# Janspiry/Image-Super-Resolution-via-Iterative-Refinement

Hardware: AMD Instinct MI355X
Metric: SR3 16->128 images/sec (2000-step sample) (higher is better)
Workload: dtype f32 via 3xbf16 split MFMA; 1 GPU; SR3 16->128 UNet (reference config/sr_sr3_16_128.json; BASELINE.json configs[1]), batch 16 per GPU, 2000-step p_sample_loop via hipGraph replay; step = one reverse step of the batch; images/s = n_gpus*batch/(2000*t_step); batch_per_gpu=16, global_batch=16, image_size=128, params=97807491, parallelism=independent batches per rank (no collective), weights=random init (PyTorch default, seed 0), output_finite=True

## Files before the change

image-super-resolution-via-iterative-refinement_amd/csrc/abi_ops.hip:

```cpp
#include "plan_internal.h"
#include "tile_code.h"

namespace {

enum Derive { DERIVE_IGEMM_WSPLIT, DERIVE_WINO, DERIVE_WINO_SPLIT };
size_t derive_bytes(const ConvParams& c, Derive kind) {
  const int Cin = c.C0 + c.C1;
  return (kind == DERIVE_IGEMM_WSPLIT ? igemm_wsplit_floats(c.Cout, c.ksize * c.ksize, Cin) : wino_weight_floats(c.Cout, Cin, kind == DERIVE_WINO_SPLIT)) * sizeof(float);
}
int derive_behind_slabs(const ConvParams& c, int tile, int ksplit, Derive kind, void* scratch, size_t* scratch_bytes, hipStream_t st, float** out) {
  const size_t slab = conv_splitk_bytes(c, tile, ksplit);
  const size_t need = derive_bytes(c, kind);
  if (!scratch || *scratch_bytes < slab + need) {
    set_error("conv: %s (%zu < %zu)", kind == DERIVE_IGEMM_WSPLIT ? "scratch too small for the pre-split weights" : "Winograd scratch too small", *scratch_bytes, slab + need);
    return SR3_E_NOMEM;
  }
  *out = reinterpret_cast<float*>(static_cast<char*>(scratch) + slab);
  *scratch_bytes = slab;
  const int Cin = c.C0 + c.C1;
  return kind == DERIVE_IGEMM_WSPLIT ? igemm_split_weights(c.w, c.Cout, c.ksize * c.ksize, Cin, *out, st)
                                     : wino_transform_weights(c.w, c.Cout, Cin, *out, st, kind == DERIVE_WINO_SPLIT);
}

}

extern "C" {

int sr3_p_sample_step(float* x, const float* eps, const float* z, const float* ta, const float* tb, const float* tc1,
                      const float* tc2, const float* tsig, const int* step_dev, const int64_t* t_per_sample,
                      int step_host, int batch, int elems_per_image, void* stream) {
  if (!x || !eps || !ta || !tb || !tc1 || !tc2 || !tsig) { set_error("null argument"); return SR3_E_BADARG; }
  StepTables t{ta, tb, tc1, tc2, tsig};
  return p_sample_update(x, eps, z, t, step_dev, t_per_sample, step_host, batch, elems_per_image,
                         static_cast<hipStream_t>(stream));
}
int sr3_p_sample_step_ex(float* x, const float* eps, const float* z, const float* ta, const float* tb, const float* tc1,
                         const float* tc2, const float* tsig, const int* step_dev, const int64_t* t_per_sample,
                         int step_host, int batch, int elems_per_image, int clip_denoised, void* stream) {
  if (!x || !eps || !ta || !tb || !tc1 || !tc2 || !tsig) { set_error("null argument"); return SR3_E_BADARG; }
  StepTables t{ta, tb, tc1, tc2, tsig};
  return p_sample_update(x, eps, z, t, step_dev, t_per_sample, step_host, batch, elems_per_image,
                         static_cast<hipStream_t>(stream), clip_denoised != 0);
}
int sr3_p_sample_step_hist(float* x, const float* eps, const float* z, const float* ta, const float* tb, const float* tc1,
                           const float* tc2, const float* tsig, const int* step_dev, const int64_t* t_per_sample,
                           int step_host, int batch, int elems_per_image, int clip_denoised, const float* tc3, float* hist,
                           void* stream) {
  if (!x || !eps || !ta || !tb || !tc1 || !tc2 || !tsig) { set_error("null argument"); return SR3_E_BADARG; }
  if (batch <= 0 || elems_per_image <= 0) { set_error("p_sample_step_hist: sizes must be positive"); return SR3_E_BADARG; }
  StepTables t{ta, tb, tc1, tc2, tsig};
  return p_sample_update(x, eps, z, t, step_dev, t_per_sample, step_host, batch, elems_per_image,
                         static_cast<hipStream_t>(stream), clip_denoised != 0, tc3, hist);
}
int sr3_step_decrement(int* step_dev, void* stream) { return step_decrement(step_dev, static_cast<hipStream_t>(stream)); }
int sr3_q_sample(const float* x0, const float* z, const float* ca, const float* cb, int batch, int elems_per_image,
                 float* out, void* stream) {
  if (!x0 || !z || !ca || !cb || !out) { set_error("null argument"); return SR3_E_BADARG; }
  return q_sample(x0, z, ca, cb, batch, elems_per_image, out, static_cast<hipStream_t>(stream));
}

int sr3_conv_f32(const float* src0, int C0, const float* src1, int C1, int B, int Hs, int Ws, int ups, int stride,
                 int ksize, int Cout, const float* w, const float* bias, const float* ss, int act, const float* film,
                 int film_stride, const float* res0, int RC0, const float* res1, int RC1, float* out, double* out_stats,
                 int tile_cfg, int ksplit, void* scratch, size_t scratch_bytes, void* stream) {
  if (!src0 || !w || !out) { set_error("null argument"); return SR3_E_BADARG; }
  hipStream_t st = static_cast<hipStream_t>(stream);
  ConvParams c = conv_shape(B, Hs, Ws, ups, stride, ksize, C0, src1 ? C1 : 0, Cout);
  c.src0 = src0; c.src1 = src1; c.w = w; c.bias = bias; c.ss = ss; c.act = act; c.film = film; c.film_stride = film_stride;
  c.res0 = res0; c.res1 = res1; c.RC0 = res0 ? RC0 : 0; c.RC1 = res1 ? RC1 : 0;
  c.out = out; c.ostat = out_stats;
  const TileCode t = tile_decode(tile_cfg);
  c.wino_split = t.wino_split; c.wino_full = t.wino_full; c.igemm_split = t.igemm_split; tile_cfg = t.tile;
  if (t.wpre) {
    if (tile_cfg == 22 && !gemm1x1_fits(c, 2)) { set_error("conv: the 1x1 GEMM kernel (tile 22) does not fit this problem"); return SR3_E_UNSUPPORTED; }
    float* q = nullptr;
    if (const int rc = derive_behind_slabs(c, tile_cfg, ksplit, DERIVE_IGEMM_WSPLIT, scratch, &scratch_bytes, st, &q)) return rc;
    c.w_split = q;
  }
  if (tile_cfg == 11 && (ksize != 3 || stride != 1)) { set_error("conv: the Winograd kernel does not fit this problem (3x3 stride 1 only)"); return SR3_E_UNSUPPORTED; }
  if (tile_cfg == 11) {
    const Derive kind = t.wino_split ? DERIVE_WINO_SPLIT : DERIVE_WINO;
#ifdef SR3_WINO_ABLATIONS
    const size_t total = scratch_bytes;
#endif
    float* u = nullptr;
    if (const int rc = derive_behind_slabs(c, tile_cfg, ksplit, kind, scratch, &scratch_bytes, st, &u)) return rc;
    c.wino_u = u;
#ifdef SR3_WINO_ABLATIONS
    if (total >= scratch_bytes + derive_bytes(c, kind) + (1u << 20)) c.partial = reinterpret_cast<float*>(reinterpret_cast<char*>(u) + derive_bytes(c, kind));
#endif
  }
  return conv_forward(c, tile_cfg, ksplit, static_cast<float*>(scratch), scratch_bytes, st);
}
int sr3_block_conv_f32(const float* src0, int C0, const float* src1, int C1, int B, int H, int W, int Cout,
                       const float* w, const float* bias, const float* ss, int act, const float* film, int film_stride,
                       const float* x2_src0, int x2_C0, const float* x2_src1, int x2_C1, const float* x2_w,
                       const float* x2_bias, float* out, double* out_stats, int tile_cfg, int ksplit, void* scratch,
                       size_t scratch_bytes, void* stream) {
  if (!src0 || !w || !out || !x2_src0 || !x2_w) { set_error("null argument"); return SR3_E_BADARG; }
  ConvParams c = conv_shape(B, H, W, 0, 1, 3, C0, src1 ? C1 : 0, Cout);
  c.src0 = src0; c.src1 = src1; c.w = w; c.bias = bias; c.ss = ss; c.act = act; c.film = film; c.film_stride = film_stride;
  c.out = out; c.ostat = out_stats;
  c.x2_src0 = x2_src0; c.x2_src1 = x2_src1; c.x2_C0 = x2_C0; c.x2_C1 = x2_src1 ? x2_C1 : 0; c.x2_w = x2_w; c.x2_bias = x2_bias;
  return conv_forward(c, tile_cfg, ksplit, static_cast<float*>(scratch), scratch_bytes, static_cast<hipStream_t>(stream));
}
int sr3_conv_dropout_f32(const float* src0, int C0, int B, int H, int W, int Cout, const float* w, const float* bias,
                         const float* ss, int act, const float* film, int film_stride, const float* res0, int RC0,
                         const float* x2_src0, int x2_C0, const float* x2_src1, int x2_C1, const float* x2_w,
                         const float* x2_bias, float* out, double* out_stats, int tile_cfg, int ksplit, void* scratch,
                         size_t scratch_bytes, unsigned drop_seed, float drop_p, void* stream) {
  if (!src0 || !w || !out || !ss) { set_error("null argument"); return SR3_E_BADARG; }
  if (drop_p < 0.f || drop_p >= 1.f) { set_error("drop_p out of range"); return SR3_E_BADARG; }
  hipStream_t st = static_cast<hipStream_t>(stream);
  ConvParams c = conv_shape(B, H, W, 0, 1, 3, C0, 0, Cout);
  c.src0 = src0; c.w = w; c.bias = bias; c.ss = ss; c.act = act; c.film = film; c.film_stride = film_stride;
  c.res0 = res0; c.RC0 = res0 ? RC0 : 0;
  c.out = out; c.ostat = out_stats;
  if (x2_src0) {
    if (!x2_w) { set_error("x2_src0 needs x2_w"); return SR3_E_BADARG; }
    c.x2_src0 = x2_src0; c.x2_src1 = x2_src1; c.x2_C0 = x2_C0; c.x2_C1 = x2_src1 ? x2_C1 : 0; c.x2_w = x2_w; c.x2_bias = x2_bias;
  }
  c.drop_seed = drop_seed;
  dropout_consts(drop_p, &c.drop_thresh, &c.drop_scale);
  TileCode t = tile_decode(tile_cfg);
  if (tile_cfg != 12) t = TileCode{tile_cfg, 0, 0, false};
  c.wino_split = t.wino_split; tile_cfg = t.tile;
  if (tile_cfg == 11) {
    if (c.x2_w) { set_error("conv: the Winograd kernel has no fused 1x1 segment"); return SR3_E_UNSUPPORTED; }
    float* u = nullptr;
    if (const int rc = derive_behind_slabs(c, tile_cfg, ksplit, t.wino_split ? DERIVE_WINO_SPLIT : DERIVE_WINO, scratch, &scratch_bytes, st, &u)) return rc;
    c.wino_u = u;
  }
  return conv_forward(c, tile_cfg, ksplit, static_cast<float*>(scratch), scratch_bytes, st);
}
unsigned sr3_dropout_threshold(float drop_p, float* scale_out) {
  unsigned t = 0;
  float s = 1.f;
  if (drop_p > 0.f && drop_p < 1.f) dropout_consts(drop_p, &t, &s);
  if (scale_out) *scale_out = s;
  return t;
}
size_t sr3_conv_scratch_bytes(int B, int Ho, int Wo, int Cin, int Cout, int ksize, int tile_cfg, int ksplit) {
  const TileCode t = tile_decode(tile_cfg);
  ConvParams c = conv_shape(B, Ho, Wo, 0, 1, ksize, Cin, 0, Cout);
  c.igemm_split = t.igemm_split;
  if (t.tile == 11) {
    c.wino_split = t.wino_split == 3 ? 3 : 0;
    return conv_splitk_bytes(c, 11, ksplit) + derive_bytes(c, t.wino_split ? DERIVE_WINO_SPLIT : DERIVE_WINO);
  }
  if (t.tile == 22) {
    if (ksize == 3) { c = conv_shape(B, 2 * Ho, 2 * Wo, 0, 2, 3, Cin, 0, Cout); c.igemm_split = 1; }
    return conv_splitk_bytes(c, 22, ksplit) + derive_bytes(c, DERIVE_IGEMM_WSPLIT);
  }
  const size_t extra = t.wpre ? derive_bytes(c, DERIVE_IGEMM_WSPLIT) : 0;
  const size_t b = conv_splitk_bytes(c, t.tile, ksplit);
  c.Hs = c.Ws = c.stride = 0;
  const size_t a = conv_splitk_bytes(c, t.tile, ksplit);
  return (a > b ? a : b) + extra;
}
int sr3_groupnorm_stats_f32(const float* x, int B, int HW, int C, double* stat, void* stream) {
  if (!x || !stat) { set_error("null argument"); return SR3_E_BADARG; }
  return chan_stats(x, B, HW, C, stat, static_cast<hipStream_t>(stream));
}
int sr3_groupnorm_stats_slices(int B, int HW, int C) { return chan_stats_slices(B, HW, C); }
int sr3_conv_stats_slices(int B, int Hs, int Ws, int ups, int Cin, int Cout, int tile_cfg, int ksplit) {
  ConvParams c = conv_shape(B, Hs, Ws, ups, 1, 3, Cin, 0, Cout);
  const TileCode t = tile_decode(tile_cfg);
  c.wino_split = t.wino_split; c.igemm_split = t.igemm_split; tile_cfg = t.tile;
  if (tile_cfg == 22) c.igemm_split = 0;
  conv_pick(c, tile_cfg, ksplit);
  if (ksplit > 1) {
    const int rpb = splitk_rows_per_block(c, true);
    return rpb > 0 ? (c.Ho * c.Wo) / rpb : 0;
  }
  if (tile_cfg == 11) {
    WinoGeom wg;
    return wino_geometry(c, &wg) ? wino_stats_slices(wg) : 0;
  }
  HaloGeom g;
  if (tile_cfg < 5 || !halo_geometry(c, tile_cfg, &g)) return 0;
  return halo_stats_slices(g);
}
int sr3_groupnorm_fold_f32(const double* stat0, int C0, int T0, const double* stat1, int C1, int T1, int B, int HW,
                           int groups, const float* gamma, const float* beta, float eps, float* ss, void* stream) {
  if (!stat0 || !gamma || !beta || !ss) { set_error("null argument"); return SR3_E_BADARG; }
  return gn_finalize(stat0, C0, T0, stat1, stat1 ? C1 : 0, stat1 ? T1 : 0, B, HW, groups, gamma, beta, eps, ss,
                     static_cast<hipStream_t>(stream));
}
int sr3_attention_f32(const float* qkv, int B, int N, int C, float* out, void* stream) {
  if (!qkv || !out) { set_error("null argument"); return SR3_E_BADARG; }
  return attention_forward(qkv, B, N, C, out, static_cast<hipStream_t>(stream));
}
int sr3_attention_ex_f32(const float* qkv, int B, int N, int C, float* out, int split, void* stream) {
  if (!qkv || !out) { set_error("null argument"); return SR3_E_BADARG; }
  return attention_forward(qkv, B, N, C, out, static_cast<hipStream_t>(stream), split);
}
int sr3_film_embed_f32(int variant, int B, int inner, const float* level, const int64_t* timestep, const float* freq,
                       const float* w1, const float* b1, const float* w2, const float* b2, const float* wf,
                       const float* bf, int F, float* temb_scratch, float* film_out, void* stream) {
  EmbedParams e;
  memset(&e, 0, sizeof(e));
  e.variant = variant; e.B = B; e.inner = inner; e.level = level; e.tstep = timestep; e.freq = freq;
  e.w1 = w1; e.b1 = b1; e.w2 = w2; e.b2 = b2; e.wf = wf; e.bf = bf; e.F = F; e.temb = temb_scratch; e.film = film_out;
  return embed_forward(e, static_cast<hipStream_t>(stream));
}
int sr3_conv_in_f32(const float* a, int Ca, const float* b, int Cb, int B, int H, int W, const float* w,
                    const float* bias, int Cout, float* out, void* stream) {
  return conv_in_nchw(a, Ca, b, b ? Cb : 0, B, H, W, w, bias, Cout, out, nullptr, static_cast<hipStream_t>(stream));
}
int sr3_conv_out_f32(const float* x, const float* ss, int B, int H, int W, int C, const float* w, const float* bias,
                     int Cout, float* out, void* stream) {
  return conv_out_nchw(x, ss, B, H, W, C, w, bias, Cout, out, static_cast<hipStream_t>(stream));
}

}
```

image-super-resolution-via-iterative-refinement_amd/csrc/conv_igemm.hip:

```cpp
#include <stdlib.h>

#include <type_traits>

#include "sr3_common.h"

namespace sr3 {

__device__ __forceinline__ float silu_f(float v) {
  return SR3_SILU(v);
}

template <int BM, int BN, int TAPS, int SPLITM>
__global__ __launch_bounds__(256, 2) void k_conv_igemm(const ConvParams p) {
  constexpr bool SPLIT = SPLITM != 0, WPRE = SPLITM == 2;
  constexpr int BK = 32, LDK = 36, LDB = 32;
  constexpr int NST = (SPLIT && !WPRE && BM + BN > 192) ? 1 : 2;
  constexpr int AR = BM / 32, BR = BN / 32;
  constexpr int WM = BM / 2, WN = BN / 2;
  constexpr int MI = WM / 32, NI = WN / 32;
  constexpr int STAGE = SPLIT ? (BM + (WPRE ? 0 : BN)) * LDB * 3 / 2 : (BM + BN) * LDK;
  auto swz = [](int row, int seg) { return row * LDB + (((seg ^ (row >> 2)) & 3) << 3); };
  extern __shared__ f32x4 smem_v[];
  float* smem = reinterpret_cast<float*>(smem_v);

// ... 369 lines not shown
  const int nchunks = (Cin + 31) / 32;
  const long nfrag = (long)((Cout + 31) / 32) * nchunks * taps * 2 * 64;
  int blocks = (int)((nfrag + 255) / 256);
  if (blocks > 4096) blocks = 4096;
  if (blocks < 1) blocks = 1;
  hipLaunchKernelGGL(k_split_weights, dim3(blocks), dim3(256), 0, st, w, Cout, taps, Cin, nchunks, nfrag, reinterpret_cast<__bf16*>(out));
  SR3_LAUNCH_CHECK("k_split_weights");
  return SR3_OK;
}

namespace {
struct TileCfg { int bm, bn; };
const TileCfg kCfgs[5] = {{0, 0}, {128, 128}, {128, 64}, {64, 64}, {64, 128}};

inline int cdiv(int a, int b) { return (a + b - 1) / b; }

template <int BM, int BN, int TAPS, int SPLIT = 0>
int launch_conv(const ConvParams& p, hipStream_t st) {
  static std::atomic<uint64_t> attr_done{0};
  constexpr int smem = SPLIT == 2 ? 2 * BM * 192 : SPLIT ? ((BM + BN > 192) ? 1 : 2) * (BM + BN) * 192 : 2 * (BM + BN) * 36 * 4;
  auto kern = k_conv_igemm<BM, BN, TAPS, SPLIT>;
  if (int rc = ensure_max_lds(reinterpret_cast<const void*>(kern), smem, attr_done)) return rc;
  const int M = p.B * p.Ho * p.Wo;
  dim3 grid(cdiv(M, BM) * cdiv(p.Cout, BN), p.ksplit);
  hipLaunchKernelGGL(kern, grid, dim3(256), smem, st, p);
  SR3_LAUNCH_CHECK("k_conv_igemm");
  return SR3_OK;
}
}

static thread_local hipEvent_t g_mid_event = nullptr;
void conv_set_mid_event(hipEvent_t ev) { g_mid_event = ev; }

void conv_pick(const ConvParams& p, int& tile_cfg, int& ksplit) {
  const int M = p.B * p.Ho * p.Wo;
  const int Cin = p.C0 + p.C1;
  const int taps = p.ksize * p.ksize;
  const int nchunks = cdiv(Cin, 32);
  static const bool no_wide = getenv("SR3_NO_WIDE") != nullptr;
  if (tile_cfg == 0) {
    HaloGeom g;
    if (p.ksize == 3 && p.stride == 1) {
      if (p.Cout <= 64 && halo_geometry(p, 6, &g)) tile_cfg = 6;
      else if (p.Cout > 64 && !no_wide && halo_geometry(p, 9, &g) &&
               (long)cdiv(p.Cout, 128) * g.tiles_w * g.tiles_h * cdiv(p.B, g.NB) >= 256)
        tile_cfg = 9;
      else if (halo_geometry(p, 5, &g)) tile_cfg = 5;
    }
  }
  if (tile_cfg == 0 && p.igemm_split && (p.ksize == 1 || p.stride == 2)) tile_cfg = 3;
  if (tile_cfg == 0 && p.ksize == 1) tile_cfg = 3;
  if (tile_cfg == 0) {
    const int order_wide[3] = {1, 2, 3};
    const int order_narrow[2] = {2, 3};
    const int* order = p.Cout > 64 ? order_wide : order_narrow;
    const int norder = p.Cout > 64 ? 3 : 2;
    tile_cfg = order[norder - 1];
    for (int k = 0; k < norder; ++k) {
      const TileCfg c = kCfgs[order[k]];
      if ((long)cdiv(M, c.bm) * cdiv(p.Cout, c.bn) >= 448) { tile_cfg = order[k]; break; }
    }
  }
  if (tile_cfg == 22) {
    if (ksplit == 0) {
      const long tiles = (long)(M / gemm1x1_rows(p)) * (p.Cout / gemm1x1_cols(p));
      int ks = 1;
#ifndef SR3_G1_SPLIT_BELOW
#define SR3_G1_SPLIT_BELOW 128
#endif
#ifndef SR3_G1_S2_SPLIT_BELOW
#define SR3_G1_S2_SPLIT_BELOW 512
#endif
      const int ksteps = nchunks * taps;
      const int below = taps == 9 ? SR3_G1_S2_SPLIT_BELOW : SR3_G1_SPLIT_BELOW;
      if (tiles < below && tiles > 0) {
        ks = (int)((512 + tiles - 1) / tiles);
        const int cap = taps == 9 ? (ksteps / 8 > 1 ? ksteps / 8 : 1) : (nchunks / 4 > 1 ? nchunks / 4 : 1);
        if (ks > cap) ks = cap;
        if (ks > 16) ks = 16;
      }
      while (ks > 1 && (long)(ks - 1) * cdiv(ksteps, ks) >= ksteps) --ks;
      ksplit = ks;
    }
    return;
  }
  if (ksplit == 0 && tile_cfg == 11) {
    WinoGeom wg;
    if (!wino_geometry(p, &wg)) { ksplit = 1; return; }
    const long tiles = wino_workgroups(p, wg);
    const int units = wino_chunks(p);
    const int maxck = wino_max_chunks_per_split(wg);
    const long round = p.wino_split >= 2 ? 512 : 256;
    int ks = 1;
    if (tiles < round) {
      ks = (int)((round + tiles - 1) / tiles);
      const int cap = units / 4 > 1 ? units / 4 : 1;
      if (ks > cap) ks = cap;
      if (ks > 16) ks = 16;
    }
    if (wg.NB != 1 && ks < 2 && units >= 2) ks = 2;
    if (cdiv(units, ks) > maxck) ks = cdiv(units, maxck);
    while (ks > 1 && (long)(ks - 1) * cdiv(units, ks) >= units) --ks;
    ksplit = ks;
    return;
  }
  if (ksplit == 0) {
    long tiles;
    int units, min_units;
    if (tile_cfg >= 5) {
      HaloGeom g;
      if (!halo_geometry(p, tile_cfg, &g)) { ksplit = 1; return; }
      const int bn = halo_cfg_bn(tile_cfg);
      tiles = (long)cdiv(p.Cout, bn) * g.tiles_w * g.tiles_h * cdiv(p.B, g.NB);
      units = nchunks; min_units = 2;
    } else {
      const TileCfg c = kCfgs[tile_cfg];
      tiles = (long)cdiv(M, c.bm) * cdiv(p.Cout, c.bn);
      units = nchunks * taps; min_units = 6;
    }
    int ks = 1;
    static const long split_below_env = getenv("SR3_KSPLIT_TILES") ? atol(getenv("SR3_KSPLIT_TILES")) : 384;
    const bool wide = halo_cfg_one_wg_per_cu(tile_cfg);
    const long split_below = wide ? 256 : split_below_env;
    if (tiles < split_below) {
      ks = (int)(((wide ? 256 : 512) + tiles - 1) / tiles);
      const int cap = units / min_units > 1 ? units / min_units : 1;
      if (ks > cap) ks = cap;
      if (ks > 16) ks = 16;
    }
    while (ks > 1 && (long)(ks - 1) * cdiv(units, ks) >= units) --ks;
    ksplit = ks;
  }
}

int splitk_rows_per_block(const ConvParams& p, bool stats) {
  const long M = (long)p.B * p.Ho * p.Wo;
  const int HoWo = p.Ho * p.Wo;
  int rpb = 64;
  while (rpb > 4 && M / rpb < 1024) rpb >>= 1;
  if (stats) {
    while (rpb > 1 && HoWo % rpb) rpb >>= 1;
    if (HoWo % rpb || HoWo / rpb > 256) return 0;
  }
  return rpb;
}

size_t conv_splitk_bytes(const ConvParams& p, int tile_cfg, int ksplit) {
  conv_pick(p, tile_cfg, ksplit);
  if (ksplit <= 1) return 0;
  return (size_t)ksplit * p.B * p.Ho * p.Wo * p.Cout * sizeof(float);
}

int conv_forward(const ConvParams& pin, int tile_cfg, int ksplit, float* scratch, size_t scratch_bytes,
                 hipStream_t st) {
  ConvParams p = pin;
  const int Cin = p.C0 + p.C1;
  if ((p.C0 & 3) || (p.C1 & 3) || (p.Cout & 3)) { set_error("conv: channel counts must be multiples of 4 (C0=%d C1=%d Cout=%d)", p.C0, p.C1, p.Cout); return SR3_E_UNSUPPORTED; }
  if (p.ksize != 1 && p.ksize != 3) { set_error("conv: ksize %d unsupported", p.ksize); return SR3_E_UNSUPPORTED; }
  if (p.stride != 1 && p.stride != 2) { set_error("conv: stride %d unsupported", p.stride); return SR3_E_UNSUPPORTED; }
  if (p.act != 0 && !p.ss) { set_error("conv: act needs ss"); return SR3_E_BADARG; }
  if (p.drop_thresh != 0 && (p.C1 != 0 || p.ups != 0 || p.act == 0)) { set_error("conv: dropout needs a single-source, non-upsampled, activated input"); return SR3_E_UNSUPPORTED; }
  if (p.C1 > 0 && !p.src1) { set_error("conv: C1 > 0 needs src1"); return SR3_E_BADARG; }
  if (p.res0 && p.RC0 + p.RC1 != p.Cout) { set_error("conv: residual channels %d+%d != Cout %d", p.RC0, p.RC1, p.Cout); return SR3_E_BADARG; }
  const int pad = p.ksize / 2;
  const int Hi = p.Hs << p.ups, Wi = p.Ws << p.ups;
  if ((Hi + 2 * pad - p.ksize) / p.stride + 1 != p.Ho || (Wi + 2 * pad - p.ksize) / p.stride + 1 != p.Wo) {
    set_error("conv: output dims %dx%d inconsistent with input %dx%d k%d s%d", p.Ho, p.Wo, Hi, Wi, p.ksize, p.stride);
    return SR3_E_BADARG;
  }
  {
    const double lim = 2147483647.0;
    const double e_in = (double)p.B * p.Hs * p.Ws * (double)(p.C0 > p.C1 ? p.C0 : p.C1);
    const double e_w = (double)p.Cout * p.ksize * p.ksize * (double)Cin;
    const double e_ss = (double)p.B * Cin * 2.0;
    if (e_in >= lim || e_w >= lim || e_ss >= lim) { set_error("conv: tensor exceeds 2^31 elements (32-bit offsets)"); return SR3_E_UNSUPPORTED; }
  }
  conv_pick(p, tile_cfg, ksplit);
  p.ksplit = ksplit;
  if (p.ostat && ksplit == 1 && (tile_cfg < 5 || tile_cfg >= 22)) { set_error("conv: fused output statistics need the halo kernel or split-K"); return SR3_E_UNSUPPORTED; }
  if (p.ostat && ksplit > 1 && splitk_rows_per_block(p, true) == 0) { set_error("conv: Ho*Wo does not allow fused split-K statistics"); return SR3_E_UNSUPPORTED; }
  { static const char* e = getenv("SR3_CONV_DBG"); p.dbg = e ? atoi(e) : 0; }
  if (ksplit > 1) {
    const size_t need = (size_t)ksplit * p.B * p.Ho * p.Wo * p.Cout * sizeof(float);
    if (!scratch || scratch_bytes < need) { set_error("conv: split-K scratch too small (%zu < %zu)", scratch_bytes, need); return SR3_E_NOMEM; }
    p.partial = scratch;
  }
  int rc;
  const bool k3 = p.ksize == 3;
  if (p.x2_w && (tile_cfg < 5 || tile_cfg == 11 || tile_cfg >= 22 || p.ups)) { set_error("conv: the fused 1x1 segment needs the halo kernel without upsampling"); return SR3_E_UNSUPPORTED; }
  if (p.x2_w && ((p.x2_C0 & 3) || (p.x2_C1 & 3) || !p.x2_src0 || (p.x2_C1 > 0 && !p.x2_src1))) { set_error("conv: bad x2 segment"); return SR3_E_BADARG; }
  if (tile_cfg == 22) {
    rc = gemm1x1_forward(p, 2, st);
  } else if (tile_cfg == 11) {
    rc = conv3x3_wino_forward(p, p.wino_u, st);
  } else if (tile_cfg >= 5) {
    HaloGeom g;
    if (tile_cfg > 10 || !halo_geometry(p, tile_cfg, &g)) { set_error("conv: halo tile_cfg %d does not fit this problem", tile_cfg); return SR3_E_UNSUPPORTED; }
    const int nchunks = cdiv(Cin, 32);
    if ((long)(ksplit - 1) * cdiv(nchunks, ksplit) >= nchunks && ksplit > 1) { set_error("conv: ksplit %d leaves an empty split over %d chunks", ksplit, nchunks); return SR3_E_BADARG; }
    rc = conv3x3_halo_forward(p, tile_cfg, g, st);
  } else
  if (p.igemm_split && p.w_split) switch (tile_cfg) {
    case 1: rc = k3 ? launch_conv<128, 128, 9, 2>(p, st) : launch_conv<128, 128, 1, 2>(p, st); break;
    case 2: rc = k3 ? launch_conv<128, 64, 9, 2>(p, st) : launch_conv<128, 64, 1, 2>(p, st); break;
    case 3: rc = k3 ? launch_conv<64, 64, 9, 2>(p, st) : launch_conv<64, 64, 1, 2>(p, st); break;
    case 4: rc = k3 ? launch_conv<64, 128, 9, 2>(p, st) : launch_conv<64, 128, 1, 2>(p, st); break;
    default: set_error("conv: bad tile_cfg %d", tile_cfg); return SR3_E_BADARG;
  } else
  if (p.igemm_split) switch (tile_cfg) {
    case 1: rc = k3 ? launch_conv<128, 128, 9, 1>(p, st) : launch_conv<128, 128, 1, 1>(p, st); break;
    case 2: rc = k3 ? launch_conv<128, 64, 9, 1>(p, st) : launch_conv<128, 64, 1, 1>(p, st); break;
    case 3: rc = k3 ? launch_conv<64, 64, 9, 1>(p, st) : launch_conv<64, 64, 1, 1>(p, st); break;
    case 4: rc = k3 ? launch_conv<64, 128, 9, 1>(p, st) : launch_conv<64, 128, 1, 1>(p, st); break;
    default: set_error("conv: bad tile_cfg %d", tile_cfg); return SR3_E_BADARG;
  } else
  switch (tile_cfg) {
    case 1: rc = k3 ? launch_conv<128, 128, 9>(p, st) : launch_conv<128, 128, 1>(p, st); break;
    case 2: rc = k3 ? launch_conv<128, 64, 9>(p, st) : launch_conv<128, 64, 1>(p, st); break;
    case 3: rc = k3 ? launch_conv<64, 64, 9>(p, st) : launch_conv<64, 64, 1>(p, st); break;
    case 4: rc = k3 ? launch_conv<64, 128, 9>(p, st) : launch_conv<64, 128, 1>(p, st); break;
    default: set_error("conv: bad tile_cfg %d", tile_cfg); return SR3_E_BADARG;
  }
  if (rc) return rc;
  if (ksplit > 1) {
    if (g_mid_event) { SR3_HIP(hipEventRecord(g_mid_event, st)); g_mid_event = nullptr; }
    if (p.fold) return splitk_reduce_fold(p, *p.fold, st);
    const int rpb = splitk_rows_per_block(p, p.ostat != nullptr);
    const long M = (long)p.B * p.Ho * p.Wo;
    hipLaunchKernelGGL(k_splitk_reduce, dim3((unsigned)((M + rpb - 1) / rpb)), dim3(256), 0, st, p, rpb);
    SR3_LAUNCH_CHECK("k_splitk_reduce");
  }
  return SR3_OK;
}

}
```

image-super-resolution-via-iterative-refinement_amd/csrc/gemm1x1.hip:

```cpp
#include <stdlib.h>

#include "sr3_common.h"

#pragma clang diagnostic ignored "-Wpass-failed"

namespace sr3 {

namespace {

__device__ __forceinline__ float opaque(float v) { asm("" : "+v"(v)); return v; }
__device__ __forceinline__ void split3_plain(float x0, float x1, unsigned& h, unsigned& m, unsigned& l) {
  bf16x2 hh;
  hh[0] = (__bf16)x0; hh[1] = (__bf16)x1;
  h = __builtin_bit_cast(unsigned, hh);
  const float r0 = opaque(x0 - __builtin_bit_cast(float, h << 16)), r1 = opaque(x1 - __builtin_bit_cast(float, h & 0xFFFF0000u));
  bf16x2 mm;
  mm[0] = (__bf16)r0; mm[1] = (__bf16)r1;
  m = __builtin_bit_cast(unsigned, mm);
  const float q0 = opaque(r0 - __builtin_bit_cast(float, m << 16)), q1 = opaque(r1 - __builtin_bit_cast(float, m & 0xFFFF0000u));
  bf16x2 ll;
  ll[0] = (__bf16)q0; ll[1] = (__bf16)q1;
  l = __builtin_bit_cast(unsigned, ll);
}

typedef unsigned u32x2 __attribute__((ext_vector_type(2)));

}

template <int MI, bool ACT, bool S2 = false, int WM = 1>
__global__ __launch_bounds__(256, 2) void k_gemm1x1_split(const ConvParams p) {
  static_assert(!(ACT && S2), "the stride-2 form has no GroupNorm affine");
  static_assert(WM == 1 || WM == 2, "waves along M");
  constexpr int NWN = 4 / WM;
  constexpr int MQ = MI * WM;
  constexpr int BM = 32 * MQ;
  constexpr int FRAG = 64 * 16;
  constexpr int STAGE = 2 * MQ * 3 * FRAG;
  extern __shared__ f32x4 smem_v[];
  char* smem = reinterpret_cast<char*>(smem_v);

  const int tid = threadIdx.x, lane = tid & 63, wave = tid >> 6;
  const int wn = wave % NWN, wm = wave / NWN;
  const int Cin = p.C0 + p.C1;
  const int HoWo = p.Ho * p.Wo;
  const int M = p.B * HoWo;
  const int total = (Cin >> 5) * (S2 ? 9 : 1);
  const int per = (total + p.ksplit - 1) / p.ksplit;
  const int it0 = blockIdx.y * per;
  const int it1 = min(total, it0 + per);
  const int nsteps = it1 - it0;
  const int tiles_n = p.Cout / (32 * NWN);
  int tile_m, tile_n;
  {
    const int nwg = gridDim.x, w = blockIdx.x;
    const int q = nwg >> 3, r = nwg & 7, xcd = w & 7;
    const int lin = (xcd < r ? xcd * (q + 1) : r * (q + 1) + (xcd - r) * q) + (w >> 3);
    tile_m = lin / tiles_n;
    tile_n = lin - tile_m * tiles_n;
  }

  const int kq = tid & 7, lrow = tid >> 3;
  int aoff0[MQ], aoff1[MQ], ssoff[MQ];
  int edge[MQ];
#pragma unroll
  for (int i = 0; i < MQ; ++i) {
    const int m = tile_m * BM + lrow + 32 * i;
    if constexpr (S2) {
      const int b = m / HoWo, r = m - b * HoWo;
      const int oh = r / p.Wo, ow = r - oh * p.Wo;
      aoff0[i] = ((b * p.Hs + 2 * oh) * p.Ws + 2 * ow) * p.C0 + kq * 4;
      aoff1[i] = 0;
      edge[i] = (oh == 0 ? 1 : 0) | (ow == 0 ? 2 : 0);
    } else {
      aoff0[i] = m * p.C0 + kq * 4;
      aoff1[i] = m * p.C1 + kq * 4 - p.C0;
      edge[i] = 0;
    }
    ssoff[i] = ((m / HoWo) * Cin + kq * 4) * 2;
  }
  const bf16x8* bq = reinterpret_cast<const bf16x8*>(p.w_split) + ((size_t)(tile_n * NWN + wn) * total + it0) * (6 * 64) + lane;

  f32x4 ra[3][MQ];
  bf16x8 rb[3][6];
  f32x4 ssa[MQ], ssb[MQ];
  int pad[3] = {0, 0, 0};
  auto load_a = [&](int s, int it) {
    if constexpr (S2) {
      const int chunk = it / 9, tap = it - chunk * 9;
      const int ky = tap / 3, kx = tap - ky * 3;
      const int off = ((ky - 1) * p.Ws + (kx - 1)) * p.C0 + (chunk << 5);
      const int tapedge = (ky == 0 ? 1 : 0) | (kx == 0 ? 2 : 0);
      int pm = 0;
#pragma unroll
      for (int i = 0; i < MQ; ++i) {
        const bool out = (edge[i] & tapedge) != 0;
        ra[s][i] = *reinterpret_cast<const f32x4*>(p.src0 + aoff0[i] + (out ? (chunk << 5) : off));
        pm |= out ? (1 << i) : 0;
      }
      pad[s] = pm;
      return;
    }
    const int c = it << 5;
    const bool second = c >= p.C0;
    const float* sp = second ? p.src1 : p.src0;
#pragma unroll
    for (int i = 0; i < MQ; ++i) ra[s][i] = *reinterpret_cast<const f32x4*>(sp + (second ? aoff1[i] : aoff0[i]) + c);
  };
  auto load_b = [&](int s, int rel) {
    const bf16x8* q = bq + (size_t)rel * (6 * 64);
#pragma unroll
    for (int j = 0; j < 6; ++j) rb[s][j] = q[j * 64];
  };
  auto load_ss = [&](int it) {
    if constexpr (ACT) {
      const int c2 = it << 6;
#pragma unroll
      for (int i = 0; i < MQ; ++i) {
        const float* q = p.ss + ssoff[i] + c2;
        ssa[i] = *reinterpret_cast<const f32x4*>(q);
        ssb[i] = *reinterpret_cast<const f32x4*>(q + 4);
      }
    }
  };
  const int wbase = (kq >> 2) * (MQ * 3 * FRAG) + (lrow + 32 * ((kq >> 1) & 1)) * 16 + (kq & 1) * 8;
  auto stage_a = [&](int s, int stage) {
    char* A = smem + stage * STAGE + wbase;
#pragma unroll
    for (int i = 0; i < MQ; ++i) {
      f32x4 v = ra[s][i];
      if constexpr (S2) { if (pad[s] & (1 << i)) v = f32x4{0.f, 0.f, 0.f, 0.f}; }
      if constexpr (ACT) {
        v.x = opaque(fmaf(v.x, ssa[i].x, ssa[i].y));
        v.y = opaque(fmaf(v.y, ssa[i].z, ssa[i].w));
        v.z = opaque(fmaf(v.z, ssb[i].x, ssb[i].y));
        v.w = opaque(fmaf(v.w, ssb[i].z, ssb[i].w));
      }
      unsigned h0, m0, l0, h1, m1, l1;
      split3_plain(v.x, v.y, h0, m0, l0);
      split3_plain(v.z, v.w, h1, m1, l1);
      const u32x2 h = {h0, h1}, m = {m0, m1}, l = {l0, l1};
      *reinterpret_cast<u32x2*>(A + (i * 3 + 0) * FRAG) = h;
      *reinterpret_cast<u32x2*>(A + (i * 3 + 1) * FRAG) = m;
      *reinterpret_cast<u32x2*>(A + (i * 3 + 2) * FRAG) = l;
    }
  };

  f32x16 acc[MI];
#pragma unroll
  for (int i = 0; i < MI; ++i)
#pragma unroll
    for (int r = 0; r < 16; ++r) acc[i][r] = 0.f;

  constexpr int NSQ = 10, NSL = NSQ * MQ, NMF = 12 * MI, NBAR = 8 * MI;
  constexpr int PA[6] = {2, 0, 1, 1, 0, 0}, PB[6] = {0, 2, 1, 0, 1, 0};
  bf16x8 a0[MI][3];
  auto read_a0 = [&](int stage) {
    const char* Ar = smem + stage * STAGE + lane * 16 + wm * (MI * 3 * FRAG);
#pragma unroll
    for (int m = 0; m < MI; ++m)
#pragma unroll
      for (int pl = 0; pl < 3; ++pl) a0[m][pl] = *reinterpret_cast<const bf16x8*>(Ar + (m * 3 + pl) * FRAG);
  };
  auto step = [&](int s0, int s1, int s2, int i) {
    const int stage = i & 1;
    const int i2 = min(i + 2, nsteps - 1);
    const char* Ar = smem + stage * STAGE + lane * 16 + wm * (MI * 3 * FRAG);
    char* Aw = smem + (stage ^ 1) * STAGE + wbase;
    bf16x8 a1[MI][3];
#ifdef SR3_G1_ABL
    load_a(s2, (SR3_G1_ABL & 4) ? it0 : it0 + i2); load_b(s2, (SR3_G1_ABL & 1) ? 0 : i2);
#else
    load_a(s2, it0 + i2); load_b(s2, i2);
#endif
    __builtin_amdgcn_sched_barrier(0);
    f32x4 v[MQ];
    float r[MQ][4];
    unsigned hh[MQ][2], mm[MQ][2], ll[MQ][2];
    auto slice = [&](int sl) {
#ifdef SR3_G1_ABL
      if (SR3_G1_ABL & 2) return;
#endif
      const int j = sl / NSQ, ph = sl % NSQ;
      if (ph == 0) {
        v[j] = ra[s1][j];
        if constexpr (S2) { if (pad[s1] & (1 << j)) v[j] = f32x4{0.f, 0.f, 0.f, 0.f}; }
        if constexpr (ACT) {
          v[j].x = opaque(fmaf(v[j].x, ssa[j].x, ssa[j].y));
          v[j].y = opaque(fmaf(v[j].y, ssa[j].z, ssa[j].w));
          v[j].z = opaque(fmaf(v[j].z, ssb[j].x, ssb[j].y));
          v[j].w = opaque(fmaf(v[j].w, ssb[j].z, ssb[j].w));
        }
      } else if (ph == 9) {
        const u32x2 h = {hh[j][0], hh[j][1]}, m = {mm[j][0], mm[j][1]}, l = {ll[j][0], ll[j][1]};
        *reinterpret_cast<u32x2*>(Aw + (j * 3 + 0) * FRAG) = h;
        *reinterpret_cast<u32x2*>(Aw + (j * 3 + 1) * FRAG) = m;
        *reinterpret_cast<u32x2*>(Aw + (j * 3 + 2) * FRAG) = l;
      } else {
        const int e = (ph - 1) >> 2, sub = (ph - 1) & 3;
        if (sub == 0) {
          bf16x2 t;
          t[0] = (__bf16)v[j][2 * e]; t[1] = (__bf16)v[j][2 * e + 1];
          hh[j][e] = __builtin_bit_cast(unsigned, t);
        } else if (sub == 1) {
          r[j][2 * e] = opaque(v[j][2 * e] - __builtin_bit_cast(float, hh[j][e] << 16));
          r[j][2 * e + 1] = opaque(v[j][2 * e + 1] - __builtin_bit_cast(float, hh[j][e] & 0xFFFF0000u));
        } else if (sub == 2) {
          bf16x2 t;
          t[0] = (__bf16)r[j][2 * e]; t[1] = (__bf16)r[j][2 * e + 1];
          mm[j][e] = __builtin_bit_cast(unsigned, t);
        } else {
          const float q0 = opaque(r[j][2 * e] - __builtin_bit_cast(float, mm[j][e] << 16));
          const float q1 = opaque(r[j][2 * e + 1] - __builtin_bit_cast(float, mm[j][e] & 0xFFFF0000u));
          bf16x2 t;
          t[0] = (__bf16)q0; t[1] = (__bf16)q1;
          ll[j][e] = __builtin_bit_cast(unsigned, t);
        }
      }
    };
#pragma unroll
    for (int n = 0; n < NMF; ++n) {
      const int ks = n / (6 * MI), q = (n % (6 * MI)) / MI, m = n % MI;
#ifdef SR3_G1_ABL
      if (SR3_G1_ABL & 8) { if (q == 0) { acc[m][0] += (float)a0[m][0][0] + (float)a1[m][0][0] + (float)rb[s0][0][0] + (float)rb[s0][3][0]; } } else
#endif
      if (ks == 0) acc[m] = __builtin_amdgcn_mfma_f32_32x32x16_bf16(a0[m][PA[q]], rb[s0][PB[q]], acc[m], 0, 0, 0);
      else acc[m] = __builtin_amdgcn_mfma_f32_32x32x16_bf16(a1[m][PA[q]], rb[s0][3 + PB[q]], acc[m], 0, 0, 0);
      if (n == 2 * MI) {
#pragma unroll
        for (int mb = 0; mb < MI; ++mb)
#pragma unroll
          for (int pl = 0; pl < 3; ++pl) a1[mb][pl] = *reinterpret_cast<const bf16x8*>(Ar + ((MQ + mb) * 3 + pl) * FRAG);
      }
      if (n < NBAR - 1) {
#pragma unroll
        for (int sl = (n * NSL) / (NBAR - 1); sl < ((n + 1) * NSL) / (NBAR - 1); ++sl) slice(sl);
      }
      if (n == NBAR - 1) {
        __builtin_amdgcn_sched_barrier(0);
        __syncthreads();
        read_a0(stage ^ 1);
        load_ss(it0 + i2);
      }
      __builtin_amdgcn_sched_barrier(0);
    }
  };
  if (nsteps > 0) {
    load_a(0, it0); load_b(0, 0); load_ss(it0);
    if (nsteps > 1) { load_a(1, it0 + 1); load_b(1, 1); }
    stage_a(0, 0);
    if (nsteps > 1) load_ss(it0 + 1);
    __syncthreads();
    read_a0(0);
    int i = 0;
    for (; i + 2 < nsteps; i += 3) {
      step(0, 1, 2, i);
      step(1, 2, 0, i + 1);
      step(2, 0, 1, i + 2);
    }
    if (i < nsteps) step(0, 1, 2, i);
    if (i + 1 < nsteps) step(1, 2, 0, i + 1);
  }

  const bool direct = p.ksplit == 1;
  float* dst = direct ? p.out : p.partial + (size_t)blockIdx.y * M * p.Cout;
  const int n = tile_n * (32 * NWN) + wn * 32 + (lane & 31);
  float bn = 0.f;
  if (direct && p.bias) bn = p.bias[n];
#pragma unroll
  for (int i = 0; i < MI; ++i) {
#pragma unroll
    for (int g = 0; g < 4; ++g) {
      const int mbase = tile_m * BM + 32 * (wm * MI + i) + 8 * g;
      float fb = bn;
      if (direct && p.film) fb += p.film[(size_t)(mbase / HoWo) * p.film_stride + n];
#pragma unroll
      for (int e = 0; e < 4; ++e) {
        const int m = mbase + e + 4 * (lane >> 5);
        float v = acc[i][g * 4 + e];
        if (direct) {
          v += fb;
          if (p.res0) v += (n < p.RC0) ? p.res0[(size_t)m * p.RC0 + n] : p.res1[(size_t)m * p.RC1 + (n - p.RC0)];
        }
        dst[(size_t)m * p.Cout + n] = v;
      }
    }
  }
}

bool gemm1x1_s2(const ConvParams& p) {
  return p.ksize == 3 && p.stride == 2 && p.C1 == 0 && p.act == 0 && !(p.Hs & 1) && !(p.Ws & 1) && p.Ho * 2 == p.Hs && p.Wo * 2 == p.Ws;
}
bool gemm1x1_fits(const ConvParams& p, int mi) {
  const long M = (long)p.B * p.Ho * p.Wo;
  return ((p.ksize == 1 && p.stride == 1) || gemm1x1_s2(p)) && p.ups == 0 && (p.Cout & 63) == 0 && p.C0 > 0 && (p.C0 & 31) == 0 && (p.C1 & 31) == 0 &&
         M % (32 * mi) == 0 && ((p.Ho * p.Wo) & 31) == 0 && (p.act == 0 || p.act == 1) && p.drop_thresh == 0 && !p.x2_w;
}

int gemm1x1_cols(const ConvParams& p) { return (p.Cout & 127) ? 64 : 128; }
int gemm1x1_rows(const ConvParams& p) {
  if (p.Cout & 127) return 64;
#ifdef SR3_G1_NO32
  return 64;
#elif defined(SR3_G1_ALL32)
  return 32;
#else
  const long M = (long)p.B * p.Ho * p.Wo;
  if ((M / 64) * (p.Cout / 128) >= 384) return 64;
  if (p.ksize == 3) return 32;
  return (M <= 1024 || p.C0 + p.C1 <= 512) ? 32 : 64;
#endif
}

int gemm1x1_forward(const ConvParams& p, int mi, hipStream_t st) {
  if (!gemm1x1_fits(p, mi) || !p.w_split) { set_error("conv: the 1x1 GEMM kernel (tile 22) does not fit this problem"); return SR3_E_UNSUPPORTED; }
  if (p.act == 1 && !p.ss) { set_error("conv: act needs ss"); return SR3_E_BADARG; }
  const int M = p.B * p.Ho * p.Wo;
  const int rows = gemm1x1_rows(p), cols = gemm1x1_cols(p);
  mi = rows / 32;
  dim3 grid((M / rows) * (p.Cout / cols), p.ksplit);
  const int smem = 2 * 2 * mi * 3 * 1024;
  static std::atomic<uint64_t> done[9];
  auto go = [&](auto kern, std::atomic<uint64_t>& d) -> int {
    if (int rc = ensure_max_lds(reinterpret_cast<const void*>(kern), smem, d)) return rc;
    hipLaunchKernelGGL(kern, grid, dim3(256), smem, st, p);
    SR3_LAUNCH_CHECK("k_gemm1x1_split");
    return SR3_OK;
  };
  if (p.ksize == 3 && p.act) { set_error("conv: the stride-2 form of the GEMM kernel takes no activation"); return SR3_E_UNSUPPORTED; }
  if (cols == 64) {
    if (p.ksize == 3) return go(k_gemm1x1_split<1, false, true, 2>, done[6]);
    return p.act ? go(k_gemm1x1_split<1, true, false, 2>, done[7]) : go(k_gemm1x1_split<1, false, false, 2>, done[8]);
  }
  if (p.ksize == 3) {
    return mi == 2 ? go(k_gemm1x1_split<2, false, true>, done[4]) : go(k_gemm1x1_split<1, false, true>, done[5]);
  }
  if (mi == 2) return p.act ? go(k_gemm1x1_split<2, true>, done[0]) : go(k_gemm1x1_split<2, false>, done[1]);
  if (mi == 1) return p.act ? go(k_gemm1x1_split<1, true>, done[2]) : go(k_gemm1x1_split<1, false>, done[3]);
  set_error("conv: bad 1x1 GEMM tile");
  return SR3_E_BADARG;
}

}
```

image-super-resolution-via-iterative-refinement_amd/csrc/plan.hip:

```cpp
#include <stdarg.h>
#include <stdlib.h>
#include <stdio.h>
#include <string.h>

#include <algorithm>
#include <map>
#include <string>
#include <vector>

#include "plan_internal.h"
#include "tile_code.h"
#include "train.h"

namespace sr3 {

static thread_local char g_err[512] = "";
void set_error(const char* fmt, ...) {
  va_list ap;
  va_start(ap, fmt);
  vsnprintf(g_err, sizeof(g_err), fmt, ap);
  va_end(ap);
}
int hip_fail(hipError_t e, const char* what) {
  set_error("HIP error %d (%s) at %s", (int)e, hipGetErrorString(e), what);
  (void)hipGetLastError();
  return (int)e > 0 ? (int)e : 1;
}
const char* last_error() { return g_err; }

static size_t add_param(sr3_plan* P, const std::string& name, int ndim, const int* shape, int pack, size_t* cursor) {
  sr3_param_info pi;
  memset(&pi, 0, sizeof(pi));
  snprintf(pi.name, sizeof(pi.name), "%s", name.c_str());
  pi.ndim = ndim;
  size_t n = 1;
  for (int i = 0; i < ndim; ++i) { pi.shape[i] = shape[i]; n *= (size_t)shape[i]; }
  pi.pack = pack;
  pi.numel = n;
  *cursor = (*cursor + 3) & ~(size_t)3;
  pi.offset = *cursor;
  *cursor += n;
  P->pindex[name] = (int)P->params.size();
  P->params.push_back(pi);
  return pi.offset;
}
static size_t add_vec(sr3_plan* P, const std::string& name, int n, size_t* cur) {
  int s[1] = {n};
  return add_param(P, name, 1, s, 0, cur);
}
static size_t add_mat(sr3_plan* P, const std::string& name, int o, int i, size_t* cur) {
  int s[2] = {o, i};
  return add_param(P, name, 2, s, 0, cur);
}
static size_t add_conv(sr3_plan* P, const std::string& name, int o, int i, int k, size_t* cur) {
  int s[4] = {o, i, k, k};
  return add_param(P, name, 4, s, k == 1 ? 0 : 1, cur);
}

static bool in_list(const int* v, int n, int x) {
  for (int i = 0; i < n; ++i) if (v[i] == x) return true;
  return false;
}

static int build_structure(sr3_plan* P) {
  const sr3_unet_desc& d = P->d;
  const int inner = d.inner_channel;
  const bool ddpm = d.variant == SR3_VARIANT_DDPM;
  if (inner <= 0 || (inner & 3)) { set_error("inner_channel must be a positive multiple of 4 (got %d)", inner); return SR3_E_UNSUPPORTED; }
  if (d.n_mults < 1 || d.n_mults > 8 || d.n_attn_res < 0 || d.n_attn_res > 8) { set_error("bad n_mults/n_attn_res"); return SR3_E_BADARG; }
  if (d.norm_groups <= 0) { set_error("norm_groups must be > 0"); return SR3_E_BADARG; }
  if (d.in_channel <= 0 || d.in_channel > 16) { set_error("in_channel %d unsupported", d.in_channel); return SR3_E_UNSUPPORTED; }
  const int out_ch = d.out_channel > 0 ? d.out_channel : d.in_channel;
  if (out_ch > 4) { set_error("out_channel %d > 4 unsupported", out_ch); return SR3_E_UNSUPPORTED; }
  if ((d.image_size >> (d.n_mults - 1)) < 1 || (d.image_size & ((1 << (d.n_mults - 1)) - 1))) {
    set_error("image_size %d not divisible by 2^%d", d.image_size, d.n_mults - 1);
    return SR3_E_BADARG;
  }
  P->out_ch = out_ch;

  struct Proto { LayerKind kind; int cin, cout, skip; bool attn; };
  std::vector<Proto> pd, pm, pu;
  std::vector<int> feat;
  int pre = inner, now_res = d.image_size;
  feat.push_back(pre);
  pd.push_back({L_CONV_IN, d.in_channel, inner, 0, false});
  for (int ind = 0; ind < d.n_mults; ++ind) {
    const bool is_last = ind == d.n_mults - 1;
    const bool use_attn = in_list(d.attn_res, d.n_attn_res, now_res);
    const int cm = inner * d.channel_mults[ind];
    for (int r = 0; r < d.res_blocks; ++r) {
      pd.push_back({L_RES, pre, cm, 0, use_attn});
      feat.push_back(cm);
      pre = cm;
    }
    if (!is_last) {
      pd.push_back({L_DOWN, pre, pre, 0, false});
      feat.push_back(pre);
      now_res /= 2;
    }
  }
  pm.push_back({L_RES, pre, pre, 0, true});
  pm.push_back({L_RES, pre, pre, 0, false});
  for (int ind = d.n_mults - 1; ind >= 0; --ind) {
    const bool is_last = ind < 1;
    const bool use_attn = in_list(d.attn_res, d.n_attn_res, now_res);
    const int cm = inner * d.channel_mults[ind];
    for (int r = 0; r < d.res_blocks + 1; ++r) {
      const int skip = feat.back();
      feat.pop_back();
      pu.push_back({L_RES, pre + skip, cm, skip, use_attn});
      pre = cm;
    }
    if (!is_last) {
      pu.push_back({L_UP, pre, pre, 0, false});
      now_res *= 2;
    }
  }
  P->fin_cin = pre;

  size_t cur = 0;
  int F = 0;
  auto count_f = [&](const std::vector<Proto>& v) { for (auto& p : v) if (p.kind == L_RES) F += p.cout; };
  count_f(pd); count_f(pm); count_f(pu);
  P->F = F;
  P->film_w = cur; cur += (size_t)F * inner;
  cur = (cur + 3) & ~(size_t)3;
  P->film_b = cur; cur += (size_t)F;
  int frow = 0;

  const char* emb = ddpm ? "time_mlp" : "noise_level_mlp";
  P->emb_w1 = add_mat(P, std::string(emb) + ".1.weight", 4 * inner, inner, &cur);
  P->emb_b1 = add_vec(P, std::string(emb) + ".1.bias", 4 * inner, &cur);
  P->emb_w2 = add_mat(P, std::string(emb) + ".3.weight", inner, 4 * inner, &cur);
  P->emb_b2 = add_vec(P, std::string(emb) + ".3.bias", inner, &cur);

  auto emit = [&](const std::vector<Proto>& protos, const char* grp, std::vector<Layer>& out) {
    for (size_t i = 0; i < protos.size(); ++i) {
      const Proto& pr = protos[i];
      Layer L;
      L.kind = pr.kind;
      L.cin = pr.cin;
      L.cout = pr.cout;
      char nm[64];
      snprintf(nm, sizeof(nm), "%s.%zu", grp, i);
      L.name = nm;
      L.w = L.b = 0;
      std::string n = nm;
      if (pr.kind == L_CONV_IN) {
        L.w = add_conv(P, n + ".weight", pr.cout, pr.cin, 3, &cur);
        L.b = add_vec(P, n + ".bias", pr.cout, &cur);
      } else if (pr.kind == L_DOWN || pr.kind == L_UP) {
        L.w = add_conv(P, n + ".conv.weight", pr.cout, pr.cin, 3, &cur);
        L.b = add_vec(P, n + ".conv.bias", pr.cout, &cur);
      } else {
        ResLayer& R = L.res;
        R.name = n;
        R.cin = pr.cin; R.cout = pr.cout; R.skip = pr.skip; R.attn = pr.attn;
        R.film_off = frow;
        std::string rb = n + ".res_block";
        {
          sr3_param_info pi;
          memset(&pi, 0, sizeof(pi));
          std::string wn = rb + (ddpm ? ".mlp.1.weight" : ".noise_func.noise_func.0.weight");
// ... 375 lines not shown
  for (auto& L : P->downs) {
    if (L.kind == L_CONV_IN) {
      cur = bld.make(L.cout, IH, IW);
      Op o; o.kind = OP_CONV_IN;
      Op::ConvIn& v = o.conv_in;
      v.x_channels = d.in_channel - cond_channels; v.cond_channels = cond_channels; v.Cout = L.cout; v.H = IH; v.W = IW;
      v.w = L.w; v.bias = L.b; v.out = bld.T[cur].off;
      if (const int slices = P->fuse_stats ? conv_in_stat_slices(d.in_channel, IH, IW, L.cout) : 0) {
        bld.stat_slot(cur, slices);
        v.ostat = bld.T[cur].stat_off;
      }
      ops.push_back(o);
      if (bld.train) { Rec r; r.kind = R_CONV_IN; r.out = cur; r.s.w = L.w; r.s.bias = L.b; P->recs.push_back(r); }
      bld.flops += 2.0 * B * IH * IW * (double)L.cout * L.cin * 9;
    } else if (L.kind == L_RES) {
      cur = bld.res_block(cur, -1, L.res);
    } else {
      cur = bld.conv({.x0 = cur, .Cout = L.cout, .stride = 2, .w = L.w, .bias = L.b, .want_stats = true});
    }
    feats.push_back(cur);
    tap(L.name, cur);
  }
  bool cur_is_skip = true;
  for (auto& L : P->mid) {
    const int nxt = bld.res_block(cur, -1, L.res);
    if (!cur_is_skip) bld.drop(cur);
    cur = nxt;
    cur_is_skip = false;
    tap(L.name, cur);
  }
  for (auto& L : P->ups) {
    int nxt;
    if (L.kind == L_RES) {
      const int skip = feats.back();
      feats.pop_back();
      nxt = bld.res_block(cur, skip, L.res);
      bld.drop(cur);
      bld.drop(skip);
    } else {
      nxt = bld.conv({.x0 = cur, .Cout = L.cout, .ups = 1, .w = L.w, .bias = L.b, .want_stats = true});
      bld.drop(cur);
    }
    cur = nxt;
    tap(L.name, cur);
  }
  bld.fold(cur, -1, P->fin_gn_w, P->fin_gn_b);
  {
    Op o; o.kind = OP_CONV_OUT;
    o.conv_out = {bld.T[cur].off, P->fin_w, P->fin_b, bld.T[cur].C, P->out_ch, IH, IW};
    o.ss_rel = bld.cur_ss;
    ops.push_back(o);
    if (bld.train) {
      Rec r; r.kind = R_CONV_OUT; r.s.x0 = cur; r.s.w = P->fin_w; r.s.bias = P->fin_b; r.s.act = 2; r.gamma = P->fin_gn_w; r.beta = P->fin_gn_b;
      r.ss_off = bld.cur_ss; r.mr_off = bld.cur_mr;
      P->recs.push_back(r);
    }
    bld.flops += 2.0 * B * IH * IW * (double)P->out_ch * bld.T[cur].C * 9;
  }
}

void layout_derived(sr3_plan* P) {
  P->derived.clear();
  P->derived_of.clear();
  size_t dcur = 0;
  auto reg = [&](size_t w, int Cout, int Cin) {
    if (Cin & 3) return;
    P->derived.push_back({w, Cout, Cin, dcur});
    P->derived_of[w] = dcur;
    dcur += wino_weight_floats(Cout, Cin) + (P->wino_split ? wino_weight_floats(Cout, Cin, true) : 0);
  };
  for (auto* v : {&P->downs, &P->mid, &P->ups})
    for (auto& L : *v) {
      if (L.kind == L_RES) { reg(L.res.c1_w, L.res.cout, L.res.cin); reg(L.res.c2_w, L.res.cout, L.res.cout); }
      else if (L.kind == L_UP) reg(L.w, L.cout, L.cin);
    }
  P->wsplits.clear();
  P->wsplit_of.clear();
  if (P->gemm_split && (P->gemm_wpre || P->gemm2)) {
    auto regw = [&](size_t w, int Cout, int taps, int Cin) {
      if (Cin & 3) return;
      if (!P->gemm_wpre && ((taps != 1 && !(taps == 9 && P->gemm_s2)) || (Cout & (P->gemm_n64 ? 63 : 127)) || (Cin & 31))) return;
      P->wsplits.push_back({w, Cout, taps, Cin, dcur});
      P->wsplit_of[w] = dcur;
      dcur += igemm_wsplit_floats(Cout, taps, Cin);
    };
    for (auto* v : {&P->downs, &P->mid, &P->ups})
      for (auto& L : *v) {
        if (L.kind == L_RES) {
          if (L.res.has_rc) regw(L.res.rc_w, L.res.cout, 1, L.res.cin);
          if (L.res.attn) { regw(L.res.qkv_w, 3 * L.res.cout, 1, L.res.cout); regw(L.res.ao_w, L.res.cout, 1, L.res.cout); }
        } else if (L.kind == L_DOWN && (L.cout > 64 || (P->gemm2 && P->gemm_s2 && P->gemm_n64 && L.cout == 64))) {
          regw(L.w, L.cout, 9, L.cin);
        }
      }
  }
  P->derived_floats = dcur;
  P->derived_from = nullptr;
  if (P->derived_bound_bytes < dcur * sizeof(float)) { P->derived_ptr = nullptr; P->derived_bound_bytes = 0; }
}

static int build_forward(sr3_plan* P, int B, int cond_channels) {
  if (P->built_batch == B && P->built_cond == cond_channels && P->built_h == plan_height(P) && P->built_w == plan_width(P)) return SR3_OK;
  const sr3_unet_desc& d = P->d;
  if (B <= 0) { set_error("batch must be > 0"); return SR3_E_BADARG; }
  if (cond_channels < 0 || cond_channels >= d.in_channel) { set_error("cond_channels %d out of range (in_channel %d)", cond_channels, d.in_channel); return SR3_E_BADARG; }
  P->ops.clear();
  P->taps.clear();
  P->built_batch = -1;
  Builder bld(P, B);
  const int inner = d.inner_channel;
  walk_forward(P, bld, cond_channels);
  if (!bld.refused.empty()) {
    set_error("geometry %d x %d unsupported: %s", plan_height(P), plan_width(P), bld.refused.c_str());
    P->ops.clear();
    P->taps.clear();
    return SR3_E_UNSUPPORTED;
  }
  if (P->fork_side && !P->ops.empty() && P->ops[0].kind == OP_EMBED) {
    for (Op& o : P->ops)
      if (o.kind == OP_CONV && o.conv.film_row >= 0) {
        if (o.wait_id < 0) { o.wait_id = bld.n_side; P->ops[0].side_id = bld.n_side++; }
        break;
      }
  }
  size_t off = (bld.act.high + 255) & ~(size_t)255;
  Regions& R = P->regions;
  R.stats_off = off; off += (bld.stats_cursor + 255) & ~(size_t)255;
  R.ss_off = off; off += ((size_t)B * std::max(bld.max_cin, 4) * 2 * sizeof(float) + 255) & ~(size_t)255;
  R.temb_off = off; off += ((size_t)B * inner * sizeof(float) + 255) & ~(size_t)255;
  R.film_off = off; off += ((size_t)B * P->F * sizeof(float) + 255) & ~(size_t)255;
  R.scratch_off = off; R.scratch_bytes = bld.max_scratch; off += (bld.max_scratch + 255) & ~(size_t)255;
  P->ws_bytes = off;
  P->flops = bld.flops;
  P->built_batch = B;
  P->built_cond = cond_channels;
  P->built_h = plan_height(P); P->built_w = plan_width(P);
  return SR3_OK;
}

template <typename T> static T* bind(char* base, size_t off) { return off == NO_OFF ? nullptr : reinterpret_cast<T*>(base + off); }
static const float* bind(const float* params, size_t off) { return off == NO_OFF ? nullptr : params + off; }

static FoldTail make_fold_tail(const FoldSpec& s, int groups, const float* params, char* ws, const Regions& R) {
  FoldTail f;
  memset(&f, 0, sizeof(f));
  f.groups = groups; f.Ctot = s.Ctot; f.c_off = s.c_off;
  f.ostat = bind<const double>(ws + R.stats_off, s.ostat); f.oC = s.oC; f.oT = s.oT; f.o_off = s.o_off;
  f.gamma = params + s.gamma; f.beta = params + s.beta; f.eps = 1e-5f;
  f.ss = reinterpret_cast<float*>(ws + R.ss_off + s.ss_rel);
  f.mr = s.has_mr ? reinterpret_cast<float*>(ws + R.mr_off + s.mr_rel) : nullptr;
  return f;
}

int run_forward(sr3_plan* P, bool train, const float* x, const float* cond, int cond_channels, const float* level,
                const int64_t* tstep, const float* freq, const float* level_table, const int* step_dev,
                const float* params, char* ws, float* eps_out, int B, hipStream_t st,
                hipEvent_t* ev, hipEvent_t* mid, const DropCfg* drop, const StepFuse* fuse, const int* t_map) {
  const sr3_unet_desc& d = P->d;
  const Regions& R = train ? P->t_regions : P->regions;
  size_t op_index = 0;
  float* film = reinterpret_cast<float*>(ws + R.film_off);
  char* const stats = ws + R.stats_off;
  const bool forking = !ev && !train;
  hipStream_t const main_st = st;
  for (const Op& o : train ? P->tops : P->ops) {
    int rc = SR3_OK;
    st = main_st;
    if (ev) SR3_HIP(hipEventRecord(ev[op_index], st));
    ++op_index;
    if (forking && o.wait_id >= 0 && o.wait_id < (int)P->join_ev.size())
      SR3_HIP(hipStreamWaitEvent(main_st, P->join_ev[o.wait_id], 0));
    if (forking && o.side_id >= 0) {
      if (!P->side_stream) SR3_HIP(hipStreamCreateWithFlags(&P->side_stream, hipStreamNonBlocking));
      while ((int)P->fork_ev.size() <= o.side_id) {
        hipEvent_t a, b;
        SR3_HIP(hipEventCreateWithFlags(&a, hipEventDisableTiming));
        SR3_HIP(hipEventCreateWithFlags(&b, hipEventDisableTiming));
        P->fork_ev.push_back(a); P->join_ev.push_back(b);
      }
      SR3_HIP(hipEventRecord(P->fork_ev[o.side_id], main_st));
      SR3_HIP(hipStreamWaitEvent(P->side_stream, P->fork_ev[o.side_id], 0));
      st = P->side_stream;
    }
    switch (o.kind) {
      case OP_RESERVED:
        break;
      case OP_EMBED: {
        EmbedParams e;
        memset(&e, 0, sizeof(e));
        e.variant = d.variant; e.B = B; e.inner = d.inner_channel;
        e.level = level; e.tstep = tstep; e.level_table = level_table; e.step_dev = step_dev; e.t_map = t_map; e.freq = freq;
        e.step_out = fuse ? const_cast<int*>(fuse->step_cur) : nullptr;
        e.w1 = params + P->emb_w1; e.b1 = params + P->emb_b1; e.w2 = params + P->emb_w2; e.b2 = params + P->emb_b2;
        e.wf = params + P->film_w; e.bf = params + P->film_b; e.F = P->F;
        e.temb = reinterpret_cast<float*>(ws + R.temb_off); e.film = film;
        rc = embed_forward(e, st);
        break;
      }
      case OP_CONV_IN: {
        const Op::ConvIn& v = o.conv_in;
        const float* a = cond_channels > 0 ? cond : x;
        const int Ca = cond_channels > 0 ? cond_channels : v.x_channels;
        const float* b = cond_channels > 0 ? x : nullptr;
        const int Cb = cond_channels > 0 ? v.x_channels : 0;
        rc = conv_in_nchw(a, Ca, b, Cb, B, v.H, v.W, params + v.w, params + v.bias, v.Cout, bind<float>(ws, v.out),
                          bind<double>(stats, v.ostat), st);
        break;
      }
      case OP_STATS: {
        const Op::Stats& v = o.stats;
        if (o.fold_fused) {
          FoldTail ft = make_fold_tail(o.tail, d.norm_groups, params, ws, R);
          rc = chan_stats_fold(bind<const float>(ws, v.src), B, v.pixels, v.channels, bind<double>(stats, v.stat), ft, st);
          break;
        }
        rc = chan_stats(bind<const float>(ws, v.src), B, v.pixels, v.channels, bind<double>(stats, v.stat), st);
        break;
      }
      case OP_FOLD: {
        const Op::Fold& v = o.fold;
        rc = gn_finalize(bind<const double>(stats, v.stat0), v.C0, v.T0, bind<const double>(stats, v.stat1), v.C1, v.T1, B, v.pixels,
                         d.norm_groups, params + v.gamma, params + v.beta, 1e-5f, bind<float>(ws, R.ss_off + o.ss_rel), st,
                         v.has_mr ? bind<float>(ws, R.mr_off + o.mr_rel) : nullptr);
        break;
      }
      case OP_CONV: {
        const Op::Conv& v = o.conv;
        const ConvChoice& ch = v.ch;
        ConvParams c = v.cp;
        c.src0 = bind<const float>(ws, v.src0);
        c.src1 = bind<const float>(ws, v.src1);
        c.w = params + v.w;
        c.bias = bind(params, v.bias);
        c.ss = c.act ? bind<const float>(ws, R.ss_off + o.ss_rel) : nullptr;
        c.film = v.film_row >= 0 ? film + v.film_row : nullptr;
        c.res0 = bind<const float>(ws, v.res0);
        c.res1 = bind<const float>(ws, v.res1);
        c.out = bind<float>(ws, v.out);
        c.ostat = bind<double>(stats, v.ostat);
        if (drop && v.has_drop && drop->thresh != 0) {
          c.drop_seed = drop_layer_seed(drop->seed, v.drop_key); c.drop_thresh = drop->thresh; c.drop_scale = drop->scale;
        }
        if (v.x2_src0 != NO_OFF) {
          c.x2_src0 = bind<const float>(ws, v.x2_src0);
          c.x2_src1 = bind<const float>(ws, v.x2_src1);
          c.x2_w = params + v.x2_w;
          c.x2_bias = params + v.x2_bias;
        }
        if (ch.tile_cfg == 11) {
          if (!P->derived_ptr) { set_error("the plan's derived (Winograd) weights are not bound: call sr3_plan_bind_derived + sr3_plan_prepare_derived"); return SR3_E_BADARG; }
          if (P->derived_from != params) {
            set_error("the plan's derived (Winograd) weights are stale or were prepared from another arena: call sr3_plan_prepare_derived");
            return SR3_E_BADARG;
          }
          c.wino_u = P->derived_ptr + ch.wino_off;
        }
        if (ch.has_wsplit && ((ch.tile_cfg >= 1 && ch.tile_cfg <= 4) || ch.tile_cfg == 22) && c.igemm_split) {
          if (!P->derived_ptr || P->derived_from != params) {
            set_error("the plan's derived (pre-split 1x1 / stride-2) weights are not bound or stale: call sr3_plan_bind_derived + sr3_plan_prepare_derived");
            return SR3_E_BADARG;
          }
          c.w_split = P->derived_ptr + ch.wsplit_off;
        }
        if (mid && ch.ksplit > 1) conv_set_mid_event(mid[op_index - 1]);
        FoldTail ft;
        if (o.fold_fused) { ft = make_fold_tail(o.tail, d.norm_groups, params, ws, R); c.fold = &ft; }
        rc = conv_forward(c, ch.tile_cfg, ch.ksplit, bind<float>(ws, R.scratch_off), R.scratch_bytes, st);
        break;
      }
      case OP_ATTN: {
        const Op::Attn& v = o.attn;
        rc = attention_forward(bind<const float>(ws, v.qkv), B, v.tokens, v.channels, bind<float>(ws, v.out), st,
                               (P->attn_split ? 1 : 0) | (v.tile_cfg == 24 ? 2 : 0));
        break;
      }
      case OP_CONV_OUT: {
        const Op::ConvOut& v = o.conv_out;
        rc = conv_out_nchw(bind<const float>(ws, v.src), bind<const float>(ws, R.ss_off + o.ss_rel), B, v.H, v.W, v.channels,
                           params + v.w, params + v.bias, v.out_ch, eps_out, st, fuse);
        break;
      }
    }
    if (rc) return rc;
    if (forking && o.side_id >= 0) SR3_HIP(hipEventRecord(P->join_ev[o.side_id], st));
  }
  st = main_st;
  if (ev) SR3_HIP(hipEventRecord(ev[op_index], st));
  return SR3_OK;
}

TrainWalk walk_train(sr3_plan* P, int B, int cond_channels) {
  P->tops.clear();
  P->recs.clear();
  Builder bld(P, B, true);
  walk_forward(P, bld, cond_channels);
  P->ttens = bld.T;
  TrainWalk w;
  w.act_high = bld.act.high; w.stats_bytes = bld.stats_cursor; w.gn_bytes = bld.gn_cursor; w.mr_bytes = bld.mr_cursor;
  w.max_scratch = bld.max_scratch; w.refused = bld.refused;
  return w;
}

}

extern "C" {

int sr3_version(void) { return SR3_ABI_VERSION; }
const char* sr3_last_error(void) { return sr3::last_error(); }
int sr3_selftest_split3(int* scratch_dev, int* mismatches, void* stream) {
  if (!scratch_dev || !mismatches) { sr3::set_error("null argument"); return SR3_E_BADARG; }
  hipStream_t st = static_cast<hipStream_t>(stream);
  const int rc = sr3::split3_selftest(scratch_dev, st);
  if (rc) return rc;
  SR3_HIP(hipMemcpyAsync(mismatches, scratch_dev, sizeof(int), hipMemcpyDeviceToHost, st));
  SR3_HIP(hipStreamSynchronize(st));
  if (*mismatches != 0) { sr3::set_error("split3 self-test: %d of 2097152 elements do not satisfy x == h + m + l exactly (compiler / ISA change?)", *mismatches); return SR3_E_UNSUPPORTED; }
  return SR3_OK;
}

int sr3_plan_create(const sr3_unet_desc* desc, sr3_plan** out) {
  if (!desc || !out) { set_error("null argument"); return SR3_E_BADARG; }
  sr3_plan* P = new (std::nothrow) sr3_plan();
  if (!P) { set_error("out of host memory"); return SR3_E_NOMEM; }
#ifdef SR3_EXPERIMENTS
  { const char* e = getenv("SR3_WGRAD_SPLIT"); if (e) P->wgrad_split = atoi(e); }
  { const char* e = getenv("SR3_WINO2"); if (e) P->wino2 = atoi(e); }
#endif
  P->d = *desc;
  const int rc = build_structure(P);
  if (rc) { delete P; *out = nullptr; return rc; }
  *out = P;
  return SR3_OK;
}
void sr3_plan_destroy(sr3_plan* plan) { delete plan; }
int sr3_plan_num_params(const sr3_plan* plan) { return plan ? (int)plan->params.size() : 0; }
int sr3_plan_param_info(const sr3_plan* plan, int index, sr3_param_info* out) {
  if (!plan || !out || index < 0 || index >= (int)plan->params.size()) { set_error("bad param index"); return SR3_E_BADARG; }
  *out = plan->params[index];
  return SR3_OK;
}
size_t sr3_plan_param_floats(const sr3_plan* plan) { return plan ? plan->param_floats : 0; }
int sr3_plan_num_ops(sr3_plan* plan, int batch) {
  if (!plan) return 0;
  const int cond = plan->built_cond >= 0 ? plan->built_cond : 0;
  if (build_forward(plan, batch, cond)) return -1;
  return (int)plan->ops.size();
}
int sr3_plan_op_info(sr3_plan* plan, int batch, int index, sr3_op_info* out) {
  if (!plan || !out) { set_error("null argument"); return SR3_E_BADARG; }
  const int cond = plan->built_cond >= 0 ? plan->built_cond : 0;
  const int rc = build_forward(plan, batch, cond);
  if (rc) return rc;
  if (index < 0 || index >= (int)plan->ops.size()) { set_error("op index out of range"); return SR3_E_BADARG; }
  const Op& o = plan->ops[index];
  memset(out, 0, sizeof(*out));
  out->kind = (int)o.kind * 10;
  if (o.kind == OP_CONV) {
    const ConvParams& c = o.conv.cp;
    const ConvChoice& ch = o.conv.ch;
    out->tile_cfg = tile_encode(ch.tile_cfg, c.wino_split, c.igemm_split, ch.has_wsplit, c.wino_full);
    out->ksplit = ch.ksplit;
    out->ksize = c.ksize; out->stride = c.stride; out->upsample = c.ups;
    out->cin = c.C0 + c.C1; out->cout = c.Cout; out->h_out = c.Ho; out->w_out = c.Wo;
    out->fused_res_conv_cin = c.x2_C0 + c.x2_C1;
    out->fused_output_stats = o.conv.ostat != NO_OFF ? 1 : 0;
    out->flops = conv_flops(c);
  } else if (o.kind == OP_CONV_IN) {
    const Op::ConvIn& v = o.conv_in;
    out->ksize = 3; out->stride = 1; out->cin = v.x_channels + v.cond_channels; out->cout = v.Cout; out->h_out = v.H; out->w_out = v.W;
    out->fused_output_stats = v.ostat != NO_OFF ? 1 : 0;
  } else if (o.kind == OP_ATTN) {
    out->h_out = o.attn.tokens; out->cin = out->cout = o.attn.channels;
    out->tile_cfg = o.attn.tile_cfg;
    out->flops = attn_flops(batch, o.attn.tokens, o.attn.channels);
  }
  return SR3_OK;
}
int sr3_plan_op_side(sr3_plan* plan, int batch, int index, int* side_id, int* wait_id) {
  if (!plan) { set_error("null argument"); return SR3_E_BADARG; }
  const int cond = plan->built_cond >= 0 ? plan->built_cond : 0;
  const int rc = build_forward(plan, batch, cond);
  if (rc) return rc;
  if (index < 0 || index >= (int)plan->ops.size()) { set_error("op index out of range"); return SR3_E_BADARG; }
  if (side_id) *side_id = plan->ops[index].side_id;
  if (wait_id) *wait_id = plan->ops[index].wait_id;
  return SR3_OK;
}
double sr3_plan_forward_flops(sr3_plan* plan, int batch) {
  if (!plan) return 0;
  const int cond = plan->built_cond >= 0 ? plan->built_cond : 0;
  if (build_forward(plan, batch, cond)) return -1;
  return plan->flops;
}
int sr3_plan_set_option(sr3_plan* plan, const char* key, int value) {
  if (!plan || !key) return SR3_E_BADARG;
  int* slot = nullptr;
  if (!strcmp(key, "fuse_stats")) slot = &plan->fuse_stats;
  else if (!strcmp(key, "tile_cfg")) slot = &plan->tile_cfg;
  else if (!strcmp(key, "ksplit")) slot = &plan->ksplit;
  else if (!strcmp(key, "keep_all")) slot = &plan->keep_all;
  else if (!strcmp(key, "fuse_res")) slot = &plan->fuse_res;
  else if (!strcmp(key, "split_bf16")) slot = &plan->split_bf16;
  else if (!strcmp(key, "winograd")) slot = &plan->winograd;
  else if (!strcmp(key, "wino_split")) slot = &plan->wino_split;
  else if (!strcmp(key, "wino_split8")) slot = &plan->wino_split8;
  else if (!strcmp(key, "wgrad_split")) { const int prev = plan->wgrad_split; plan->wgrad_split = value; return prev; }
  else if (!strcmp(key, "attn_split")) { const int prev = plan->attn_split; plan->attn_split = value; return prev; }
  else if (!strcmp(key, "attn_long")) slot = &plan->attn_long;
  else if (!strcmp(key, "gemm_split")) slot = &plan->gemm_split;
  else if (!strcmp(key, "gemm_wpre")) slot = &plan->gemm_wpre;
  else if (!strcmp(key, "gemm2")) slot = &plan->gemm2;
  else if (!strcmp(key, "gemm_s2")) slot = &plan->gemm_s2;
  else if (!strcmp(key, "fork_side")) slot = &plan->fork_side;
  else if (!strcmp(key, "gemm_n64")) slot = &plan->gemm_n64;
  else if (!strcmp(key, "fold_fuse")) slot = &plan->fold_fuse;
  else if (!strcmp(key, "gemm_tile")) slot = &plan->gemm_tile;
  else if (!strcmp(key, "wino2")) slot = &plan->wino2;
  else if (!strcmp(key, "wino_ragged")) slot = &plan->wino_ragged;
  else if (!strcmp(key, "wino_up")) slot = &plan->wino_up;
  else if (!strcmp(key, "train_geom")) slot = &plan->train_geom;
  else if (!strcmp(key, "loss_l2")) { const int prev = plan->loss_l2; plan->loss_l2 = value; return prev; }
  if (!slot) { set_error("unknown option %s", key); return SR3_E_BADARG; }
#ifndef SR3_EXPERIMENTS
  if (slot == &plan->split_bf16 && value != 0) {
    set_error("option %s selects an experiment kernel that this library was built without (csrc/build.sh -DSR3_EXPERIMENTS)", key);
    return SR3_E_UNSUPPORTED;
  }
#endif
  const int prev = *slot;
  *slot = value;
  plan->built_batch = -1;
  plan->train_batch = -1;
  if (slot == &plan->winograd || slot == &plan->tile_cfg || slot == &plan->split_bf16) plan->derived_from = nullptr;
  if ((slot == &plan->wino_split || slot == &plan->gemm_split || slot == &plan->gemm_wpre || slot == &plan->gemm2 || slot == &plan->gemm_s2 || slot == &plan->gemm_n64) && prev != value) layout_derived(plan);
  return prev;
}
int sr3_plan_num_taps(sr3_plan* plan) { return plan ? (int)plan->taps.size() : 0; }
int sr3_plan_tap_info(sr3_plan* plan, int index, char* name, int name_len, size_t* offset, int* C, int* H, int* W) {
  if (!plan || index < 0 || index >= (int)plan->taps.size()) { set_error("bad tap index"); return SR3_E_BADARG; }
  const Tap& t = plan->taps[index];
  if (name && name_len > 0) snprintf(name, name_len, "%s", t.name.c_str());
  if (offset) *offset = t.off;
  if (C) *C = t.C;
  if (H) *H = t.H;
  if (W) *W = t.W;
  return SR3_OK;
}

size_t sr3_plan_derived_bytes(const sr3_plan* plan) { return plan ? plan->derived_floats * sizeof(float) : 0; }
int sr3_plan_bind_derived(sr3_plan* plan, void* buffer, size_t bytes) {
  if (!plan) { set_error("null plan"); return SR3_E_BADARG; }
  if (buffer && (bytes < plan->derived_floats * sizeof(float) || ((uintptr_t)buffer & 15))) {
    set_error("derived buffer too small or misaligned (%zu < %zu)", bytes, plan->derived_floats * sizeof(float));
    return SR3_E_NOMEM;
  }
  plan->derived_ptr = static_cast<float*>(buffer);
  plan->derived_bound_bytes = buffer ? bytes : 0;
  plan->derived_from = nullptr;
  return SR3_OK;
}
int sr3_plan_invalidate_derived(sr3_plan* plan) {
  if (!plan) { set_error("null plan"); return SR3_E_BADARG; }
  plan->derived_from = nullptr;
  return SR3_OK;
}
int sr3_plan_prepare_derived(sr3_plan* plan, const float* params, void* stream) {
  if (!plan || !params) { set_error("null argument"); return SR3_E_BADARG; }
  if (!plan->derived_ptr) { set_error("no derived buffer bound"); return SR3_E_BADARG; }
  for (const auto& d : plan->derived) {
    int rc = wino_transform_weights(params + d.w, d.Cout, d.Cin, plan->derived_ptr + d.off, static_cast<hipStream_t>(stream));
    if (rc) return rc;
    if (plan->wino_split) {
      rc = wino_transform_weights(params + d.w, d.Cout, d.Cin, plan->derived_ptr + d.off + wino_weight_floats(d.Cout, d.Cin),
                                  static_cast<hipStream_t>(stream), true);
      if (rc) return rc;
    }
  }
  for (const auto& d : plan->wsplits) {
    const int rc = igemm_split_weights(params + d.w, d.Cout, d.taps, d.Cin, plan->derived_ptr + d.off, static_cast<hipStream_t>(stream));
    if (rc) return rc;
  }
  plan->derived_from = params;
  return SR3_OK;
}

int sr3_plan_set_geometry(sr3_plan* plan, int height, int width) {
  if (!plan) { set_error("null plan"); return SR3_E_BADARG; }
  const int div = 1 << (plan->d.n_mults - 1);
  if (height == 0 && width == 0) {
    height = width = plan->d.image_size;
  } else if (height <= 0 || width <= 0 || (height % div) || (width % div)) {
    set_error("geometry %d x %d: height and width must be positive multiples of %d (2^(n_mults-1): the UNet halves the image %d times)",
              height, width, div, plan->d.n_mults - 1);
    return SR3_E_BADARG;
  }
  const bool native = height == plan->d.image_size && width == plan->d.image_size;
  const int h = native ? 0 : height, w = native ? 0 : width;
  if (h == plan->geo_h && w == plan->geo_w) return SR3_OK;
  plan->geo_h = h; plan->geo_w = w;
  plan->built_batch = -1;
  return SR3_OK;
}
int sr3_plan_get_geometry(const sr3_plan* plan, int* height, int* width) {
  if (!plan) { set_error("null plan"); return SR3_E_BADARG; }
  if (height) *height = plan_height(plan);
  if (width) *width = plan_width(plan);
  return SR3_OK;
}

size_t sr3_workspace_bytes(sr3_plan* plan, int batch) {
  if (!plan) return 0;
  const int cond = plan->built_cond >= 0 ? plan->built_cond : 0;
  if (build_forward(plan, batch, cond)) return 0;
  return plan->ws_bytes;
}

int sr3_unet_forward(sr3_plan* plan, const float* x_nchw, const float* cond_nchw, int cond_channels,
                     const float* noise_level, const int64_t* timestep, const float* freq, const float* level_table,
                     const int* step_dev, const float* params, void* workspace, size_t workspace_bytes,
                     float* eps_out_nchw, int batch, void* stream) {
  if (!plan || !x_nchw || !params || !workspace || !eps_out_nchw || !freq) { set_error("null argument"); return SR3_E_BADARG; }
  if (!cond_nchw) cond_channels = 0;
  const int rc = build_forward(plan, batch, cond_channels);
  if (rc) return rc;
  if (workspace_bytes < plan->ws_bytes) { set_error("workspace too small: %zu < %zu", workspace_bytes, plan->ws_bytes); return SR3_E_NOMEM; }
  if (((uintptr_t)workspace & 255) || ((uintptr_t)params & 15) || ((uintptr_t)x_nchw & 15) || ((uintptr_t)eps_out_nchw & 15)) {
    set_error("misaligned pointer (workspace 256 B, tensors 16 B)");
    return SR3_E_ALIGN;
  }
  if (plan->d.variant == SR3_VARIANT_SR3 && !noise_level && !step_dev) { set_error("SR3 variant needs noise_level or step_dev"); return SR3_E_BADARG; }
  if (plan->d.variant == SR3_VARIANT_DDPM && !timestep && !step_dev) { set_error("DDPM variant needs timestep or step_dev"); return SR3_E_BADARG; }
  return run_forward(plan, false, x_nchw, cond_nchw, cond_channels, noise_level, timestep, freq, level_table,
                     step_dev, params, static_cast<char*>(workspace), eps_out_nchw, batch, static_cast<hipStream_t>(stream),
                     nullptr, nullptr);
}

int sr3_reverse_step_hist(sr3_plan* plan, float* x_nchw, const float* cond_nchw, int cond_channels, const float* freq,
                          const float* level_table, int* step2_dev, const float* params, void* workspace, size_t workspace_bytes,
                          const float* z_nchw, const float* ta, const float* tb, const float* tc1, const float* tc2, const float* tsig,
                          int clip_denoised, float* eps_out_nchw, int batch, void* stream, const int* t_map, const float* tc3,
                          float* hist_nchw) {
  if (!plan || !x_nchw || !params || !workspace || !freq || !step2_dev || !ta || !tb || !tc1 || !tc2 || !tsig) { set_error("null argument"); return SR3_E_BADARG; }
  if (!cond_nchw) cond_channels = 0;
  const int rc = build_forward(plan, batch, cond_channels);
  if (rc) return rc;
  if (workspace_bytes < plan->ws_bytes) { set_error("workspace too small: %zu < %zu", workspace_bytes, plan->ws_bytes); return SR3_E_NOMEM; }
  if (((uintptr_t)workspace & 255) || ((uintptr_t)params & 15) || ((uintptr_t)x_nchw & 15) || ((uintptr_t)eps_out_nchw & 15) || ((uintptr_t)z_nchw & 15)) {
    set_error("misaligned pointer (workspace 256 B, tensors 16 B)");
    return SR3_E_ALIGN;
  }
  if (plan->d.variant == SR3_VARIANT_SR3 && !level_table) { set_error("SR3 variant needs level_table"); return SR3_E_BADARG; }
  const size_t image_bytes = (size_t)batch * plan->d.out_channel * plan_height(plan) * plan_width(plan) * sizeof(float);
  if (const int rc = check_step_history("reverse_step", tc3, hist_nchw, x_nchw, eps_out_nchw, image_bytes, true)) return rc;
  StepFuse f;
  f.x = x_nchw; f.z = z_nchw; f.tb = StepTables{ta, tb, tc1, tc2, tsig};
  f.step_cur = step2_dev; f.step_next = step2_dev + 1; f.clip = clip_denoised; f.c3 = tc3; f.hist = hist_nchw;
  return run_forward(plan, false, x_nchw, cond_nchw, cond_channels, nullptr, nullptr, freq, level_table,
                     step2_dev + 1, params, static_cast<char*>(workspace), eps_out_nchw, batch, static_cast<hipStream_t>(stream),
                     nullptr, nullptr, nullptr, &f, t_map);
}

int sr3_reverse_step_ex(sr3_plan* plan, float* x_nchw, const float* cond_nchw, int cond_channels, const float* freq,
                        const float* level_table, int* step2_dev, const float* params, void* workspace, size_t workspace_bytes,
                        const float* z_nchw, const float* ta, const float* tb, const float* tc1, const float* tc2, const float* tsig,
                        int clip_denoised, float* eps_out_nchw, int batch, void* stream, const int* t_map) {
  return sr3_reverse_step_hist(plan, x_nchw, cond_nchw, cond_channels, freq, level_table, step2_dev, params, workspace, workspace_bytes,
                               z_nchw, ta, tb, tc1, tc2, tsig, clip_denoised, eps_out_nchw, batch, stream, t_map, nullptr, nullptr);
}

int sr3_reverse_step(sr3_plan* plan, float* x_nchw, const float* cond_nchw, int cond_channels, const float* freq,
                     const float* level_table, int* step2_dev, const float* params, void* workspace, size_t workspace_bytes,
                     const float* z_nchw, const float* ta, const float* tb, const float* tc1, const float* tc2, const float* tsig,
// ... 73 lines not shown
```

image-super-resolution-via-iterative-refinement_amd/csrc/plan_internal.h:

```cpp
#pragma once
#include <map>
#include <string>
#include <vector>

#include "../../include/sr3_mi355x.h"
#include "sr3_common.h"

namespace sr3 {

struct Tensor {
  size_t off = 0;
  size_t bytes = 0;
  int C = 0, H = 0, W = 0;
  size_t stat_off = 0;
  int stat_T = 0;
  bool stats_done = false;
  bool valid = false;
};

struct ResLayer {
  std::string name;
  int cin, cout, skip;
  bool attn;
  int film_off;
  size_t gn1_w, gn1_b, c1_w, c1_b, gn2_w, gn2_b, c2_w, c2_b, rc_w, rc_b;
  bool has_rc;
  size_t an_w, an_b, qkv_w, ao_w, ao_b;
};

enum LayerKind { L_CONV_IN, L_RES, L_DOWN, L_UP };
struct Layer {
  LayerKind kind;
  std::string name;
  int cin, cout;
  size_t w, b;
  ResLayer res;
};

static constexpr size_t NO_OFF = ~(size_t)0;

struct ConvChoice {
  int tile_cfg, ksplit;
  int wino_split, igemm_split;
  int wino_mode;
  size_t wino_off;
  bool has_wsplit;
  size_t wsplit_off;
  int wino_full = 0;
};

struct FoldSpec {
  int Ctot = 0, c_off = 0;
  size_t ostat = NO_OFF;
  int oC = 0, oT = 0, o_off = 0;
  size_t gamma = 0, beta = 0;
  size_t ss_rel = 0, mr_rel = 0;
  bool has_mr = false;
};

enum OpKind { OP_RESERVED, OP_EMBED, OP_CONV_IN, OP_STATS, OP_FOLD, OP_CONV, OP_ATTN, OP_CONV_OUT };

struct Op {
  OpKind kind;
  struct ConvIn {
    int x_channels = 0, cond_channels = 0, Cout = 0, H = 0, W = 0;
    size_t w = 0, bias = 0, out = 0, ostat = NO_OFF;
  } conv_in;
  struct Stats { size_t src = 0, stat = 0; int pixels = 0, channels = 0; } stats;
  struct Fold {
    size_t stat0 = 0, stat1 = NO_OFF;
    int C0 = 0, C1 = 0, T0 = 0, T1 = 0, pixels = 0;
    size_t gamma = 0, beta = 0;
    bool has_mr = false;
  } fold;
  struct Conv {
    ConvParams cp = {};
    ConvChoice ch = {};
    size_t src0 = 0, src1 = NO_OFF, res0 = NO_OFF, res1 = NO_OFF, out = 0, ostat = NO_OFF;
    size_t w = 0, bias = NO_OFF;
    int film_row = -1;
    size_t x2_src0 = NO_OFF, x2_src1 = NO_OFF, x2_w = 0, x2_bias = 0;
    bool has_drop = false;
    unsigned drop_key = 0;
  } conv;
  struct Attn { size_t qkv = 0, out = 0; int tokens = 0, channels = 0, tile_cfg = 0; } attn;
  struct ConvOut { size_t src = 0, w = 0, bias = 0; int channels = 0, out_ch = 0, H = 0, W = 0; } conv_out;
  size_t ss_rel = 0, mr_rel = 0;
  bool fold_fused = false;
  FoldSpec tail;
  int side_id = -1, wait_id = -1;
};

inline double conv_flops(const ConvParams& c) {
  return 2.0 * c.B * c.Ho * c.Wo * (double)c.Cout * ((double)(c.C0 + c.C1) * c.ksize * c.ksize + (c.x2_C0 + c.x2_C1));
}
inline double attn_flops(int B, int tokens, int channels) { return 4.0 * B * (double)tokens * (double)tokens * channels; }

struct Tap { std::string name; size_t off; int C, H, W; };

struct Regions {
  size_t stats_off = 0, ss_off = 0, mr_off = 0, temb_off = 0, film_off = 0, scratch_off = 0, scratch_bytes = 0;
};

struct ConvSpec {
  int x0 = -1, x1 = -1;
  int Cout = 0, ksize = 3, stride = 1, ups = 0;
  int act = 0;
  size_t w = 0, bias = NO_OFF;
  int film_row = -1;
  int r0 = -1, r1 = -1;
  bool want_stats = false;
  int q0 = -1, q1 = -1; size_t qw = 0, qb = 0;
  int drop_key = -1;
};

enum WuKind { WU_NONE, WU_WINO, WU_WINO_SPLIT, WU_GEMM };
struct Dgrad {
  ConvParams c = {};
  int tile = 0, ksplit = 0;
  int wu = WU_NONE;
};

enum RecKind { R_CONV_IN, R_CONV, R_ATTN, R_CONV_OUT };
struct Rec {
  int kind = R_CONV;
  ConvSpec s;
  int out = -1;
  size_t gamma = 0, beta = 0;
  size_t ss_off = 0, mr_off = 0;
  int qkv = -1, o = -1;
  ConvParams dw = {}, dqw = {};
  Dgrad dx, dq;
  bool acc_x0 = true, acc_x1 = true, acc_r0 = true, acc_r1 = true, acc_q0 = true, acc_q1 = true;
  size_t param_end = 0;
};

struct DropCfg { unsigned seed, thresh; float scale; };
inline unsigned drop_layer_seed(unsigned seed, unsigned key) { return seed + (key + 1u) * 0x632BE5ABu; }

}

using namespace sr3;

struct sr3_plan {
  sr3_unet_desc d;
  std::vector<sr3_param_info> params;
  std::map<std::string, int> pindex;
  size_t param_floats = 0;
  int F = 0;
  size_t film_w = 0, film_b = 0;
  size_t emb_w1 = 0, emb_b1 = 0, emb_w2 = 0, emb_b2 = 0;
  std::vector<Layer> downs, mid, ups;
  size_t fin_gn_w = 0, fin_gn_b = 0, fin_w = 0, fin_b = 0;
  int fin_cin = 0, out_ch = 0;
  int fuse_stats = 1, fuse_res = 1, tile_cfg = 0, ksplit = 0, keep_all = 0, split_bf16 = 0;
  int winograd = 1;
  int wino2 = 1;
  int wino_split = 1;
  int wino_split8 = 1;
  int wgrad_split = 1;
  int attn_split = 1;
  int attn_long = 0;
  int gemm_tile = 0;
  int gemm_split = 1;
  int gemm_wpre = 0;
  int fold_fuse = 1;
  int gemm2 = 1;
  int gemm_s2 = 1;
  int gemm_n64 = 1;
  int wino_ragged = 1;
  int wino_up = 1;
  int train_geom = 0;
  int geo_h = 0, geo_w = 0;
  int fork_side = 0;
  hipStream_t side_stream = nullptr;
  std::vector<hipEvent_t> fork_ev, join_ev;
  ~sr3_plan() {
    for (hipEvent_t e : fork_ev) (void)hipEventDestroy(e);
    for (hipEvent_t e : join_ev) (void)hipEventDestroy(e);
    if (side_stream) (void)hipStreamDestroy(side_stream);
  }
  struct Derived { size_t w; int Cout, Cin; size_t off; };
  std::vector<Derived> derived;
  std::map<size_t, size_t> derived_of;
  struct WSplit { size_t w; int Cout, taps, Cin; size_t off; };
  std::vector<WSplit> wsplits;
  std::map<size_t, size_t> wsplit_of;
  size_t derived_floats = 0;
  float* derived_ptr = nullptr;
  size_t derived_bound_bytes = 0;
  const float* derived_from = nullptr;
  int loss_l2 = 0;
  int built_batch = -1;
  int built_cond = -1;
  int built_h = 0, built_w = 0;
  std::vector<Op> ops;
  std::vector<Tap> taps;
  size_t ws_bytes = 0;
  Regions regions;
  double flops = 0;
  int train_batch = -1, train_cond = -1;
  int train_h = 0, train_w = 0;
  std::vector<Op> tops;
  std::vector<sr3::Tensor> ttens;
  std::vector<sr3::Rec> recs;
  size_t t_act_bytes = 0;
  Regions t_regions;
  size_t t_dA_off = 0, t_z_off = 0, t_dq_off = 0, t_wt_off = 0, t_slab_off = 0, t_part_off = 0, t_gs_off = 0;
  size_t t_dfilm_off = 0, t_xnoisy_off = 0, t_eps_off = 0, t_geps_off = 0, t_inpad_off = 0, t_dwtmp_off = 0;
  size_t t_ws_bytes = 0, t_embscr_off = 0, t_a_off = 0;
  size_t t_wu_off = 0, t_wu_bytes = 0;
  std::vector<size_t> t_unproc_max;
  int t_final_x = -1;
  size_t t_final_ss = 0, t_final_mr = 0;
  int t_conv_in_out = -1;
};


namespace sr3 {
struct Builder;
inline int plan_height(const sr3_plan* P) { return P->geo_h > 0 ? P->geo_h : P->d.image_size; }
inline int plan_width(const sr3_plan* P) { return P->geo_w > 0 ? P->geo_w : P->d.image_size; }
inline bool plan_native_geometry(const sr3_plan* P) { return plan_height(P) == P->d.image_size && plan_width(P) == P->d.image_size; }
int run_forward(sr3_plan* P, bool train, const float* x, const float* cond, int cond_channels, const float* level,
                const int64_t* tstep, const float* freq, const float* level_table, const int* step_dev,
                const float* params, char* ws, float* eps_out, int B, hipStream_t st, hipEvent_t* ev, hipEvent_t* mid,
                const DropCfg* drop = nullptr, const StepFuse* fuse = nullptr, const int* t_map = nullptr);
struct TrainWalk {
  size_t act_high = 0;
  size_t stats_bytes = 0, gn_bytes = 0, mr_bytes = 0;
  size_t max_scratch = 0;
  std::string refused;
};
TrainWalk walk_train(sr3_plan* P, int B, int cond_channels);
int build_train(sr3_plan* P, int B, int cond_channels);
bool wino_ragged_wins(const ConvParams& c);
inline int igemm_split_rule(const sr3_plan* P, const ConvParams& c) { return (P->gemm_split && !(c.ksize == 3 && c.Cout <= 64)) ? 1 : 0; }
void layout_derived(sr3_plan* P);
}
```

image-super-resolution-via-iterative-refinement_amd/csrc/small_kernels.hip:

```cpp
#include <string.h>

#include "sr3_common.h"

namespace sr3 {

__device__ __forceinline__ float silu_s(float v) { return SR3_SILU(v); }

__global__ __launch_bounds__(256) void k_chan_stats(const float* __restrict__ x, int HW, int C, int LQ,
                                                     int pix_per_block, double* __restrict__ stat) {
  __shared__ double red[256 * 8];
  const int tid = threadIdx.x;
  const int nq = C >> 2;
  const int ql = tid % LQ, pl = tid / LQ, PP = 256 / LQ;
  const int q = blockIdx.y * LQ + ql;
  const int b = blockIdx.z;
  const int T = gridDim.x;
  const int p0 = blockIdx.x * pix_per_block;
  const int p1 = min(HW, p0 + pix_per_block);
  double s[4] = {0, 0, 0, 0}, s2[4] = {0, 0, 0, 0};
  if (q < nq) {
    const float* base = x + (size_t)b * HW * C + q * 4;
    for (int p = p0 + pl; p < p1; p += PP) {
      const f32x4 v = *reinterpret_cast<const f32x4*>(base + (size_t)p * C);
#pragma unroll
      for (int e = 0; e < 4; ++e) { const double d = (double)v[e]; s[e] += d; s2[e] += d * d; }
    }
  }
#pragma unroll
  for (int e = 0; e < 4; ++e) { red[tid * 8 + e] = s[e]; red[tid * 8 + 4 + e] = s2[e]; }
  __syncthreads();
  if (pl == 0 && q < nq) {
    for (int k = 1; k < PP; ++k) {
#pragma unroll
      for (int e = 0; e < 4; ++e) { s[e] += red[(k * LQ + ql) * 8 + e]; s2[e] += red[(k * LQ + ql) * 8 + 4 + e]; }
    }
    double* o = stat + (((size_t)b * T + blockIdx.x) * C + q * 4) * 2;
#pragma unroll
    for (int e = 0; e < 4; ++e) { o[2 * e] = s[e]; o[2 * e + 1] = s2[e]; }
  }
}

static void chan_stats_geometry(int B, int HW, int C, int* LQ_, int* cblocks_, int* ppb_, int* slices_) {
  const int nq = C >> 2;
  int LQ = 1;
  while (LQ < nq && LQ < 64) LQ <<= 1;
  const int cblocks = (nq + LQ - 1) / LQ;
  const int PP = 256 / LQ;
  long base_blocks = (long)cblocks * B;
  long want = 2048 / (base_blocks > 0 ? base_blocks : 1);
  if (want < 1) want = 1;
  if (want > 64) want = 64;
  long max_slices = (HW + PP - 1) / PP;
  if (want > max_slices) want = max_slices;
  int ppb = (int)((HW + want - 1) / want);
  ppb = ((ppb + PP - 1) / PP) * PP;
  *LQ_ = LQ; *cblocks_ = cblocks; *ppb_ = ppb; *slices_ = (HW + ppb - 1) / ppb;
}

int chan_stats_slices(int B, int HW, int C) {
  int LQ, cb, ppb, sl;
  chan_stats_geometry(B, HW, C, &LQ, &cb, &ppb, &sl);
  return sl;
}

int chan_stats(const float* x, int B, int HW, int C, double* stat, hipStream_t st) {
  if (C & 3) { set_error("chan_stats: C %% 4 != 0 (%d)", C); return SR3_E_UNSUPPORTED; }
  int LQ, cblocks, ppb, slices;
  chan_stats_geometry(B, HW, C, &LQ, &cblocks, &ppb, &slices);
  hipLaunchKernelGGL(k_chan_stats, dim3(slices, cblocks, B), dim3(256), 0, st, x, HW, C, LQ, ppb, stat);
  SR3_LAUNCH_CHECK("k_chan_stats");
  return SR3_OK;
}

__global__ __launch_bounds__(64) void k_gn_finalize(const double* __restrict__ st0, int C0, int T0,
                                                     const double* __restrict__ st1, int C1, int T1, int HW,
                                                     int groups, const float* __restrict__ gamma,
                                                     const float* __restrict__ beta, float eps,
                                                     float* __restrict__ ss, float* __restrict__ mr) {
  const int C = C0 + C1;
  const int b = blockIdx.x / groups, g = blockIdx.x - b * groups;
  const int cpg = C / groups;
  const int lane = threadIdx.x;
  double s = 0.0, s2 = 0.0;
  const int c_lo = g * cpg, c_hi = c_lo + cpg;
  const int n0 = max(0, min(c_hi, C0) - c_lo);
  typedef double d2 __attribute__((ext_vector_type(2)));
  auto walk = [&](const double* st, int Cs, int T, int c_first, int n) {
    const int total = n * T;
    auto at = [&](int idx) {
      const int k = idx / T, t = idx - k * T;
      return *reinterpret_cast<const d2*>(st + (((size_t)b * T + t) * Cs + (c_first + k)) * 2);
    };
    int idx = lane;
    for (; idx + 192 < total; idx += 256) {
      const d2 q0 = at(idx), q1 = at(idx + 64), q2 = at(idx + 128), q3 = at(idx + 192);
      s += q0[0]; s2 += q0[1]; s += q1[0]; s2 += q1[1]; s += q2[0]; s2 += q2[1]; s += q3[0]; s2 += q3[1];
    }
    for (; idx < total; idx += 64) { const d2 q = at(idx); s += q[0]; s2 += q[1]; }
  };
  walk(st0, C0, T0, c_lo, n0);
  const int n1 = cpg - n0;
  const int c1_lo = max(c_lo, C0) - C0;
  if (n1 > 0) walk(st1, C1, T1, c1_lo, n1);
#pragma unroll
  for (int m = 32; m >= 1; m >>= 1) { s += __shfl_xor(s, m); s2 += __shfl_xor(s2, m); }
  const double cnt = (double)HW * cpg;
  const double mean = s / cnt;
  double var = s2 / cnt - mean * mean;
  if (var < 0.0) var = 0.0;
  const float rstd = (float)(1.0 / sqrt(var + (double)eps));
  if (mr && lane == 0) { mr[((size_t)b * groups + g) * 2] = (float)mean; mr[((size_t)b * groups + g) * 2 + 1] = rstd; }
  for (int k = lane; k < cpg; k += 64) {
    const int c = g * cpg + k;
    const float sc = rstd * gamma[c];
    float* o = ss + ((size_t)b * C + c) * 2;
    o[0] = sc;
    o[1] = beta[c] - (float)mean * sc;
  }
}

int gn_finalize(const double* stat0, int C0, int T0, const double* stat1, int C1, int T1, int B, int HW, int groups,
                const float* gamma, const float* beta, float eps, float* ss, hipStream_t st, float* mr) {
  const int C = C0 + C1;
  if (groups <= 0 || C % groups) { set_error("gn_finalize: C=%d not divisible by groups=%d", C, groups); return SR3_E_BADARG; }
  hipLaunchKernelGGL(k_gn_finalize, dim3(B * groups), dim3(64), 0, st, stat0, C0, T0, stat1, C1, T1, HW, groups,
                     gamma, beta, eps, ss, mr);
  SR3_LAUNCH_CHECK("k_gn_finalize");
  return SR3_OK;
}

template <bool REDUCE>
__global__ __launch_bounds__(256) void k_rows_fold(const ConvParams p, const FoldTail f, const float* __restrict__ x, int C, int HW,
                                                    double* __restrict__ stat) {
  __shared__ double red[256 * 8];
  __shared__ double chs[2 * 128];
  __shared__ float mrs[2];
  const int tid = threadIdx.x;
#ifdef SR3_FOLD_NO_XCD
  const int lin = blockIdx.x;
#else
  int lin;
  {
    const int nwg = gridDim.x, w = blockIdx.x;
    const int q = nwg >> 3, r = nwg & 7, xcd = w & 7;
    lin = (xcd < r ? xcd * (q + 1) : r * (q + 1) + (xcd - r) * q) + (w >> 3);
  }
#endif
  const int b = lin / f.groups, g = lin - b * f.groups;
  const int cpg = f.Ctot / f.groups;
  const int glo = g * cpg, ghi = glo + cpg;
  const int a_lo = max(glo, f.c_off) - f.c_off, a_hi = min(ghi, f.c_off + C) - f.c_off;
  const int na = a_hi > a_lo ? a_hi - a_lo : 0;
  const int nq = na >> 2;
  int nqp = 1;
  while (nqp < nq) nqp <<= 1;
  const int R = 256 / nqp, tq = tid % nqp, tr = tid / nqp;
  double s1[4] = {0, 0, 0, 0}, s2[4] = {0, 0, 0, 0};
  if (tq < nq) {
    const int n = a_lo + 4 * tq;
    const size_t M = (size_t)p.B * HW;
    f32x4 cb = {0.f, 0.f, 0.f, 0.f};
    if constexpr (REDUCE) {
      if (p.bias) cb += *reinterpret_cast<const f32x4*>(p.bias + n);
      if (p.x2_w && p.x2_bias) cb += *reinterpret_cast<const f32x4*>(p.x2_bias + n);
    }
    for (int r = tr; r < HW; r += R) {
      const size_t m = (size_t)b * HW + r;
      f32x4 v;
      if constexpr (REDUCE) {
        v = cb;
        auto slab = [&](int s) { return *reinterpret_cast<const f32x4*>(p.partial + ((size_t)s * M + m) * p.Cout + n); };
        int s = 0;
        for (; s + 4 <= p.ksplit; s += 4) {
          const f32x4 q0 = slab(s), q1 = slab(s + 1), q2 = slab(s + 2), q3 = slab(s + 3);
          v += q0; v += q1; v += q2; v += q3;
        }
        for (; s < p.ksplit; ++s) v += slab(s);
        if (p.film) v += *reinterpret_cast<const f32x4*>(p.film + (size_t)b * p.film_stride + n);
        if (p.res0) {
          if (n < p.RC0) v += *reinterpret_cast<const f32x4*>(p.res0 + m * p.RC0 + n);
          else v += *reinterpret_cast<const f32x4*>(p.res1 + m * p.RC1 + (n - p.RC0));
        }
        *reinterpret_cast<f32x4*>(p.out + m * p.Cout + n) = v;
      } else {
        v = *reinterpret_cast<const f32x4*>(x + m * C + n);
      }
#pragma unroll
      for (int e = 0; e < 4; ++e) { const double dv = (double)v[e]; s1[e] += dv; s2[e] += dv * dv; }
    }
  }
#pragma unroll
  for (int e = 0; e < 4; ++e) { red[tid * 8 + e] = s1[e]; red[tid * 8 + 4 + e] = s2[e]; }
  __syncthreads();
  if (tid < na) {
    const int q = tid >> 2, e = tid & 3;
    double a1 = 0.0, a2 = 0.0;
    for (int k = 0; k < R; ++k) { a1 += red[(k * nqp + q) * 8 + e]; a2 += red[(k * nqp + q) * 8 + 4 + e]; }
    double* o = stat + ((size_t)b * C + a_lo + tid) * 2;
    o[0] = a1; o[1] = a2;
    const int cc = f.c_off + a_lo + tid - glo;
    chs[2 * cc] = a1; chs[2 * cc + 1] = a2;
  }
  if (f.ostat) {
    const int o_lo = max(glo, f.o_off) - f.o_off, o_hi = min(ghi, f.o_off + f.oC) - f.o_off;
    const int no = o_hi > o_lo ? o_hi - o_lo : 0;
    const int t2 = tid - 128;
    if (t2 >= 0 && t2 < no) {
      typedef double d2 __attribute__((ext_vector_type(2)));
      double a1 = 0.0, a2 = 0.0;
      const double* q = f.ostat + ((size_t)b * f.oT * f.oC + o_lo + t2) * 2;
      int t = 0;
      for (; t + 4 <= f.oT; t += 4) {
        const d2 q0 = *reinterpret_cast<const d2*>(q + (size_t)t * f.oC * 2), q1 = *reinterpret_cast<const d2*>(q + (size_t)(t + 1) * f.oC * 2),
                 q2 = *reinterpret_cast<const d2*>(q + (size_t)(t + 2) * f.oC * 2), q3 = *reinterpret_cast<const d2*>(q + (size_t)(t + 3) * f.oC * 2);
        a1 += q0[0]; a2 += q0[1]; a1 += q1[0]; a2 += q1[1]; a1 += q2[0]; a2 += q2[1]; a1 += q3[0]; a2 += q3[1];
      }
      for (; t < f.oT; ++t) { const d2 q0 = *reinterpret_cast<const d2*>(q + (size_t)t * f.oC * 2); a1 += q0[0]; a2 += q0[1]; }
      const int cc = f.o_off + o_lo + t2 - glo;
      chs[2 * cc] = a1; chs[2 * cc + 1] = a2;
    }
  }
  __syncthreads();
  if (tid == 0) {
    double s = 0.0, sq = 0.0;
    for (int k = 0; k < cpg; ++k) { s += chs[2 * k]; sq += chs[2 * k + 1]; }
    const double cnt = (double)HW * cpg;
    const double mean = s / cnt;
    double var = sq / cnt - mean * mean;
    if (var < 0.0) var = 0.0;
    const float rstd = (float)(1.0 / sqrt(var + (double)f.eps));
    mrs[0] = (float)mean; mrs[1] = rstd;
    if (f.mr) { f.mr[((size_t)b * f.groups + g) * 2] = (float)mean; f.mr[((size_t)b * f.groups + g) * 2 + 1] = rstd; }
  }
  __syncthreads();
  if (tid < cpg) {
    const int c = glo + tid;
    const float sc = mrs[1] * f.gamma[c];
    float* o = f.ss + ((size_t)b * f.Ctot + c) * 2;
    o[0] = sc;
    o[1] = f.beta[c] - mrs[0] * sc;
  }
}

bool fold_tail_fits(int C, int Ctot, int c_off, int groups) {
  if (groups <= 0 || Ctot % groups) return false;
  const int cpg = Ctot / groups;
  return (cpg & 3) == 0 && cpg <= 64 && (c_off & 3) == 0 && (C & 3) == 0;
}

int chan_stats_fold(const float* x, int B, int HW, int C, double* stat, const FoldTail& f, hipStream_t st) {
  if (!fold_tail_fits(C, f.Ctot, f.c_off, f.groups)) { set_error("chan_stats_fold: grouping does not fit"); return SR3_E_UNSUPPORTED; }
  ConvParams p;
  memset(&p, 0, sizeof(p));
  p.B = B;
  hipLaunchKernelGGL(k_rows_fold<false>, dim3(B * f.groups), dim3(256), 0, st, p, f, x, C, HW, stat);
  SR3_LAUNCH_CHECK("k_rows_fold");
  return SR3_OK;
}

int splitk_reduce_fold(const ConvParams& p, const FoldTail& f, hipStream_t st) {
  if (!fold_tail_fits(p.Cout, f.Ctot, f.c_off, f.groups) || !p.ostat) { set_error("splitk_reduce_fold: grouping does not fit"); return SR3_E_UNSUPPORTED; }
  hipLaunchKernelGGL(k_rows_fold<true>, dim3(p.B * f.groups), dim3(256), 0, st, p, f, static_cast<const float*>(nullptr), p.Cout,
                     p.Ho * p.Wo, p.ostat);
  SR3_LAUNCH_CHECK("k_rows_fold");
  return SR3_OK;
}

__global__ __launch_bounds__(256) void k_split3_selftest(int n, unsigned seed, int* __restrict__ bad) {
  int nbad = 0;
  for (int i = blockIdx.x * blockDim.x + threadIdx.x; i < n; i += gridDim.x * blockDim.x) {
    float x[2];
#pragma unroll
    for (int e = 0; e < 2; ++e) {
      const unsigned r = hash32((unsigned)(2 * i + e) * 0x9E3779B9u + seed);
      unsigned bits;
      switch (i & 7) {
        case 0: bits = (r & 0x807fffffu) | (((r >> 23) % 200u + 27u) << 23); break;
        case 1: bits = ((r >> 23) % 200u + 27u) << 23; break;
        case 2: bits = (r & 0xffff0000u & 0x807fffffu) | (100u << 23) | 0x00007fffu; break;
        case 3: bits = (r & 0xffff0000u & 0x807fffffu) | (140u << 23) | 0x00008001u; break;
        case 4: bits = (r & 0x80000000u) | (127u << 23) | 0x007fffffu; break;
        case 5: bits = r & 0x80000000u; break;
        case 6: bits = (r & 0x807fffffu) | (127u << 23); break;
        default: bits = (r & 0xffff8000u & 0x807fffffu) | (90u << 23) | 0x00008000u; break;
      }
      x[e] = __builtin_bit_cast(float, bits);
    }
    bf16x2 h, m, l;
    split3_pair(x[0], x[1], h, m, l);
#pragma unroll
    for (int e = 0; e < 2; ++e) {
      const float back = ((float)h[e] + (float)m[e]) + (float)l[e];
      if (__builtin_bit_cast(unsigned, back) != __builtin_bit_cast(unsigned, x[e]) && !(back == 0.f && x[e] == 0.f)) ++nbad;
    }
  }
  if (nbad) atomicAdd(bad, nbad);
}

int split3_selftest(int* bad_dev, hipStream_t st) {
  SR3_HIP(hipMemsetAsync(bad_dev, 0, sizeof(int), st));
  hipLaunchKernelGGL(k_split3_selftest, dim3(64), dim3(256), 0, st, 1 << 20, 0x5eedu, bad_dev);
  SR3_LAUNCH_CHECK("k_split3_selftest");
  return SR3_OK;
}

__global__ __launch_bounds__(256) void k_conv_in_nchw(const float* __restrict__ a, int Ca,
                                                       const float* __restrict__ bsrc, int Cb, int B, int H,
                                                       int W, const float* __restrict__ w,
                                                       const float* __restrict__ bias, int Cout,
                                                       float* __restrict__ out) {
  extern __shared__ f32x4 smem_v[];
  float* wl = reinterpret_cast<float*>(smem_v);
  const int Cin = Ca + Cb;
  const int K = 9 * Cin;
  const int CoutP = (Cout + 63) & ~63;
  const int tid = threadIdx.x;
  for (int i = tid; i < K * CoutP; i += 256) {
    const int k = i / CoutP, n = i - k * CoutP;
    const int tap = k / Cin, c = k - tap * Cin;
    wl[i] = (n < Cout) ? w[((size_t)n * 9 + tap) * Cin + c] : 0.f;
  }
  __syncthreads();
  const int HWp = H * W;
  const long M = (long)B * HWp;
  const long m = (long)blockIdx.x * 64 + (tid & 63);
  const int cog = tid >> 6;
  if (m >= M) return;
  const int b = (int)(m / HWp);
  const int rem = (int)(m - (long)b * HWp);
  const int oh = rem / W, ow = rem - oh * W;
  for (int cobase = 0; cobase < Cout; cobase += 64) {
    float acc[16];
#pragma unroll
    for (int e = 0; e < 16; ++e) acc[e] = 0.f;
    for (int tap = 0; tap < 9; ++tap) {
      const int ih = oh + tap / 3 - 1, iw = ow + tap % 3 - 1;
      const bool ok = (unsigned)ih < (unsigned)H && (unsigned)iw < (unsigned)W;
      for (int c = 0; c < Cin; ++c) {
        float v = 0.f;
        if (ok) {
          v = (c < Ca) ? a[((size_t)b * Ca + c) * HWp + (size_t)ih * W + iw]
                       : bsrc[((size_t)b * Cb + (c - Ca)) * HWp + (size_t)ih * W + iw];
        }
        const float* wr = wl + (size_t)(tap * Cin + c) * CoutP + cobase + cog * 16;
#pragma unroll
        for (int e4 = 0; e4 < 4; ++e4) {
          const f32x4 ww = *reinterpret_cast<const f32x4*>(wr + e4 * 4);
#pragma unroll
          for (int e = 0; e < 4; ++e) acc[e4 * 4 + e] = fmaf(v, ww[e], acc[e4 * 4 + e]);
        }
      }
    }
    const int co0 = cobase + cog * 16;
#pragma unroll
    for (int e4 = 0; e4 < 4; ++e4) {
      const int co = co0 + e4 * 4;
      if (co < Cout) {
        f32x4 o;
#pragma unroll
        for (int e = 0; e < 4; ++e) o[e] = acc[e4 * 4 + e] + (bias ? bias[co + e] : 0.f);
        *reinterpret_cast<f32x4*>(out + (size_t)m * Cout + co) = o;
      }
    }
  }
}

template <int CIN, int NB>
__global__ __launch_bounds__(256) void k_conv_in_mfma(const float* __restrict__ a, int Ca, const float* __restrict__ bsrc,
                                                       int Cb, int B, int H, int W, const float* __restrict__ w,
                                                       const float* __restrict__ bias, float* __restrict__ out,
                                                       double* __restrict__ ostat, int bpw, int T) {
  constexpr int K = 9 * CIN, KS = (K + 1) / 2, Cout = 32 * NB;
  const int lane = threadIdx.x & 63, wave = threadIdx.x >> 6;
  const int ln = lane & 31, h = lane >> 5;
  const int HW = H * W, bpi = HW >> 5;
  const int task = blockIdx.x * 4 + wave;
  if (task >= B * (bpi / bpw)) return;
  const int blk0 = task * bpw;
  const int b = blk0 / bpi;
  const int slice = (blk0 - b * bpi) / bpw;

  float bw[KS][NB], bn[NB];
#pragma unroll
  for (int s = 0; s < KS; ++s)
#pragma unroll
    for (int nb = 0; nb < NB; ++nb) {
      const int k = 2 * s + h;
      bw[s][nb] = k < K ? w[(size_t)(nb * 32 + ln) * K + k] : 0.f;
    }
#pragma unroll
  for (int nb = 0; nb < NB; ++nb) bn[nb] = bias ? bias[nb * 32 + ln] : 0.f;

  const float* plane[CIN];
#pragma unroll
  for (int c = 0; c < CIN; ++c)
    plane[c] = c < Ca ? a + ((size_t)b * Ca + c) * HW : bsrc + ((size_t)b * Cb + (c - Ca)) * HW;

  auto load_block = [&](int blk, float (&av)[KS]) {
    const int p0 = (blk - b * bpi) * 32;
    const int oh = p0 / W, ow = p0 - oh * W + ln;
    const int pixoff = oh * W + ow;
    const bool up = oh > 0, down = oh < H - 1, left = ow > 0, right = ow < W - 1;
#pragma unroll
    for (int s = 0; s < KS; ++s) {
      constexpr int dummy = 0; (void)dummy;
      const int k0 = 2 * s, k1 = 2 * s + 1;
      const int t0 = k0 / CIN, c0 = k0 - t0 * CIN, t1 = k1 / CIN, c1 = (k1 < K) ? k1 - t1 * CIN : 0;
      const int dy0 = t0 / 3 - 1, dx0 = t0 % 3 - 1, dy1 = (k1 < K) ? t1 / 3 - 1 : 0, dx1 = (k1 < K) ? t1 % 3 - 1 : 0;
      const bool v0 = (dy0 < 0 ? up : (dy0 > 0 ? down : true)) && (dx0 < 0 ? left : (dx0 > 0 ? right : true));
      const bool v1 = (k1 < K) && (dy1 < 0 ? up : (dy1 > 0 ? down : true)) && (dx1 < 0 ? left : (dx1 > 0 ? right : true));
      const bool valid = h ? v1 : v0;
      const float* pl = h ? plane[c1] : plane[c0];
      const int d = h ? dy1 * W + dx1 : dy0 * W + dx0;
      const float v = pl[pixoff + (valid ? d : 0)];
      av[s] = valid ? v : 0.f;
    }
  };

// ... 352 lines not shown
```

image-super-resolution-via-iterative-refinement_amd/csrc/sr3_common.h:

```cpp
#pragma once
#include <hip/hip_runtime.h>
#include <stdint.h>
#include <stddef.h>

#include <atomic>

#include "../../include/sr3_mi355x.h"

namespace sr3 {

typedef float f32x4 __attribute__((ext_vector_type(4)));
typedef float f32x16 __attribute__((ext_vector_type(16)));

typedef __bf16 bf16x8 __attribute__((ext_vector_type(8)));
typedef __bf16 bf16x4 __attribute__((ext_vector_type(4)));

typedef __bf16 bf16x2 __attribute__((ext_vector_type(2)));

__device__ __forceinline__ void split3_pair(float x0, float x1, bf16x2& h, bf16x2& m, bf16x2& l) {
#ifdef SR3_SPLIT_NO_DOT2
  h[0] = (__bf16)x0; h[1] = (__bf16)x1;
  const float r0 = x0 - (float)h[0], r1 = x1 - (float)h[1];
  m[0] = (__bf16)r0; m[1] = (__bf16)r1;
  const float q0 = r0 - (float)m[0], q1 = r1 - (float)m[1];
  l[0] = (__bf16)q0; l[1] = (__bf16)q1;
#else
  unsigned s_lo = 0x0000BF80u, s_hi = 0xBF800000u;
  asm("" : "+v"(s_lo), "+v"(s_hi));
  const bf16x2 sel_lo = __builtin_bit_cast(bf16x2, s_lo), sel_hi = __builtin_bit_cast(bf16x2, s_hi);
  h[0] = (__bf16)x0; h[1] = (__bf16)x1;
  const float r0 = __builtin_amdgcn_fdot2_f32_bf16(h, sel_lo, x0, false);
  const float r1 = __builtin_amdgcn_fdot2_f32_bf16(h, sel_hi, x1, false);
  m[0] = (__bf16)r0; m[1] = (__bf16)r1;
  const float q0 = __builtin_amdgcn_fdot2_f32_bf16(m, sel_lo, r0, false);
  const float q1 = __builtin_amdgcn_fdot2_f32_bf16(m, sel_hi, r1, false);
  l[0] = (__bf16)q0; l[1] = (__bf16)q1;
#endif
}
__device__ __forceinline__ void split3(const f32x4 v, bf16x4& h, bf16x4& m, bf16x4& l) {
#pragma unroll
  for (int e = 0; e < 4; e += 2) {
    bf16x2 hh, mm, ll;
    split3_pair(v[e], v[e + 1], hh, mm, ll);
    h[e] = hh[0]; h[e + 1] = hh[1]; m[e] = mm[0]; m[e + 1] = mm[1]; l[e] = ll[0]; l[e + 1] = ll[1];
  }
}

__device__ __forceinline__ void split3x8(const f32x4& lo, const f32x4& hi, bf16x8& h, bf16x8& m, bf16x8& l) {
#pragma unroll
  for (int e = 0; e < 8; e += 2) {
    bf16x2 hh, mm, ll;
    split3_pair(e < 4 ? lo[e] : hi[e - 4], e < 4 ? lo[e + 1] : hi[e - 3], hh, mm, ll);
    h[e] = hh[0]; h[e + 1] = hh[1]; m[e] = mm[0]; m[e + 1] = mm[1]; l[e] = ll[0]; l[e + 1] = ll[1];
  }
}
__device__ __forceinline__ void mfma_split6(const bf16x8 (&a)[3], const bf16x8 (&b)[3], f32x16& acc) {
  constexpr int PA[6] = {2, 0, 1, 1, 0, 0}, PB[6] = {0, 2, 1, 0, 1, 0};
#pragma unroll
  for (int q = 0; q < 6; ++q) acc = __builtin_amdgcn_mfma_f32_32x32x16_bf16(a[PA[q]], b[PB[q]], acc, 0, 0, 0);
}

#ifdef SR3_EXACT_ACT
#define SR3_SIGMOID(v) (1.0f / (1.0f + expf(-(v))))
#define SR3_SILU(v) ((v) / (1.0f + expf(-(v))))
#else
#define SR3_SIGMOID(v) __builtin_amdgcn_rcpf(1.0f + expf(-(v)))
#define SR3_SILU(v) ((v) * __builtin_amdgcn_rcpf(1.0f + expf(-(v))))
#endif

enum { SR3_OK = 0 };
void set_error(const char* fmt, ...);
int hip_fail(hipError_t e, const char* what);
#define SR3_HIP(call)                                   \
  do {                                                  \
    hipError_t _e = (call);                             \
    if (_e != hipSuccess) return sr3::hip_fail(_e, #call); \
  } while (0)
#define SR3_LAUNCH_CHECK(name)                          \
  do {                                                  \
    hipError_t _e = hipGetLastError();                  \
    if (_e != hipSuccess) return sr3::hip_fail(_e, name); \
  } while (0)

inline int ensure_max_lds(const void* kern, int bytes, std::atomic<uint64_t>& done) {
  int dev = 0;
  SR3_HIP(hipGetDevice(&dev));
  const uint64_t bit = 1ull << (dev & 63);
  if (done.load(std::memory_order_acquire) & bit) return SR3_OK;
  SR3_HIP(hipFuncSetAttribute(kern, hipFuncAttributeMaxDynamicSharedMemorySize, bytes));
  done.fetch_or(bit, std::memory_order_release);
  return SR3_OK;
}

double meant_double(float f);
inline void dropout_consts(float p, unsigned* thresh, float* scale) {
  const double pd = meant_double(p);
  *thresh = p > 0.f ? (unsigned)(pd * 4294967296.0) : 0u;
  *scale = p > 0.f ? (float)(1.0 / (1.0 - pd)) : 1.0f;
}

struct FoldTail {
  int groups, Ctot, c_off;
  const double* ostat;
  int oC, oT, o_off;
  const float* gamma;
  const float* beta;
  float eps;
  float* ss;
  float* mr;
};
bool fold_tail_fits(int C, int Ctot, int c_off, int groups);
int chan_stats_fold(const float* x, int B, int HW, int C, double* stat, const FoldTail& f, hipStream_t st);
struct ConvParams;
int splitk_reduce_fold(const ConvParams& p, const FoldTail& f, hipStream_t st);

struct ConvParams {
  const float* src0;
  const float* src1;
  int C0, C1;
  int B, Hs, Ws;
  int ups;
  int stride;
  int ksize;
  int Ho, Wo;
  int Cout;
  const float* w;
  const float* bias;
  const float* ss;
  int act;
  const float* film;
  int film_stride;
  const float* res0;
  const float* res1;
  int RC0, RC1;
  float* out;
  float* partial;
  int ksplit;
  double* ostat;
  int dbg;
  const float* x2_src0;
  const float* x2_src1;
  int x2_C0, x2_C1;
  const float* x2_w;
  const float* x2_bias;
  unsigned drop_seed, drop_thresh;
  float drop_scale;
  const float* wino_u;
  int wino_split;
  int igemm_split;
  int wgrad_split;
  const FoldTail* fold;
  const void* w_split;
  int wino_full;
};

__device__ __forceinline__ unsigned hash32(unsigned x) {
  x ^= x >> 16; x *= 0x7feb352dU; x ^= x >> 15; x *= 0x846ca68bU; x ^= x >> 16;
  return x;
}
__device__ __forceinline__ float drop_mask(unsigned seed, unsigned idx, unsigned thresh, float scale) {
  return hash32(idx * 0x9E3779B9U + seed) >= thresh ? scale : 0.f;
}

int conv_forward(const ConvParams& p, int tile_cfg, int ksplit, float* splitk_scratch,
                 size_t splitk_scratch_bytes, hipStream_t st);
size_t conv_splitk_bytes(const ConvParams& p, int tile_cfg, int ksplit);
void conv_pick(const ConvParams& p, int& tile_cfg, int& ksplit);
int splitk_rows_per_block(const ConvParams& p, bool stats);
size_t igemm_wsplit_floats(int Cout, int taps, int Cin);
int igemm_split_weights(const float* w, int Cout, int taps, int Cin, float* out, hipStream_t st);
bool gemm1x1_fits(const ConvParams& p, int mi);
int gemm1x1_cols(const ConvParams& p);
int gemm1x1_forward(const ConvParams& p, int mi, hipStream_t st);
int gemm1x1_rows(const ConvParams& p);
void conv_set_mid_event(hipEvent_t ev);
struct HaloGeom {
  int TH, TW, NB;
  int log_tw, log_thw;
  int tiles_w, tiles_h;
  int HPI, HP;
};
inline bool halo_cfg_one_wg_per_cu(int cfg) { return cfg >= 8; }
inline int halo_cfg_bm(int cfg) { return (cfg == 5 || cfg == 7) ? 128 : 256; }
inline int halo_cfg_bn(int cfg) { return (cfg == 6 || cfg == 8) ? 64 : 128; }
inline bool halo_cfg_split(int cfg) { return cfg == 7 || cfg == 8 || cfg == 10; }
bool halo_geometry(const ConvParams& p, int cfg, HaloGeom* g);
int conv3x3_halo_forward(const ConvParams& p, int cfg, const HaloGeom& g, hipStream_t st);

struct WinoGeom {
  int TH, TW, NB;
  int twt, log_twt;
  int tpi, log_tpi;
  int tiles_w, tiles_h;
  int nbt;
  int HPI, HP;
  int log_tw, log_th, pow2;
  unsigned sp_magic;
};
bool wino_geometry(const ConvParams& p, WinoGeom* g);
int wino_stats_slices(const WinoGeom& g);
int wino_max_chunks_per_split(const WinoGeom& g);
long wino_workgroups(const ConvParams& p, const WinoGeom& g);
int wino_chunks(const ConvParams& p);
size_t wino_weight_floats(int Cout, int Cin, bool split = false);
int wino_transform_weights(const float* w_ohwi, int Cout, int Cin, float* ufrag, hipStream_t st, bool split = false);
int conv3x3_wino_forward(const ConvParams& p, const float* ufrag, hipStream_t st);
bool wino2_fits(const ConvParams& p);
bool wino2_ragged_fits(const ConvParams& p);
int conv3x3_wino2_forward(const ConvParams& p, const WinoGeom& g, const float* ufrag, hipStream_t st);

int chan_stats_slices(int B, int HW, int C);
int chan_stats(const float* x, int B, int HW, int C, double* stat, hipStream_t st);
int gn_finalize(const double* stat0, int C0, int T0, const double* stat1, int C1, int T1, int B, int HW, int groups,
                const float* gamma, const float* beta, float eps, float* ss, hipStream_t st, float* mr = nullptr);
int halo_stats_slices(const HaloGeom& g);
int conv_in_stat_slices(int Cin, int H, int W, int Cout);
int conv_in_nchw(const float* a, int Ca, const float* b, int Cb, int B, int H, int W, const float* w,
                 const float* bias, int Cout, float* out, double* ostat, hipStream_t st);
struct StepTables { const float* a; const float* b; const float* c1; const float* c2; const float* sigma; };

__device__ __forceinline__ float mul_rn(float a, float b) { float r = a * b; asm volatile("" : "+v"(r)); return r; }
__device__ __forceinline__ float add_rn(float a, float b) { float r = a + b; asm volatile("" : "+v"(r)); return r; }
__device__ __forceinline__ float sub_rn(float a, float b) { float r = a - b; asm volatile("" : "+v"(r)); return r; }
struct StepCoef { float a, b, c1, c2, c3, sigma; };
template <bool HIST>
__device__ __forceinline__ StepCoef load_step_coef(const StepTables& tb, const float* c3, int t) {
  return StepCoef{tb.a[t], tb.b[t], tb.c1[t], tb.c2[t], HIST ? c3[t] : 0.f, tb.sigma[t]};
}
__device__ __forceinline__ float step_x0(const StepCoef& k, bool clip, float x, float eps) {
  float x0 = sub_rn(mul_rn(k.a, x), mul_rn(k.b, eps));
  if (clip) x0 = fminf(fmaxf(x0, -1.f), 1.f);
  return x0;
}
template <bool HIST>
__device__ __forceinline__ float step_mix(const StepCoef& k, float x0, float x, float z, float& hist) {
  float mean = add_rn(mul_rn(k.c1, x0), mul_rn(k.c2, x));
  if (HIST) { mean = add_rn(mean, mul_rn(k.c3, hist)); hist = x0; }
  return add_rn(mean, mul_rn(z, k.sigma));
}
template <bool HIST>
__device__ __forceinline__ float step_tail(const StepCoef& k, bool clip, float x, float eps, float z, float& hist) {
  return step_mix<HIST>(k, step_x0(k, clip, x, eps), x, z, hist);
}
inline bool overlaps(const void* a, size_t abytes, const void* b, size_t bbytes) {
  const uintptr_t a0 = (uintptr_t)a, b0 = (uintptr_t)b;
  return a0 < b0 + bbytes && b0 < a0 + abytes;
}
inline int check_step_history(const char* who, const float* c3, const float* hist, const float* x, const float* eps, size_t bytes,
                              bool align16 = false) {
  if ((c3 != nullptr) != (hist != nullptr)) { set_error("%s: the c3 table and the history go together (both or neither)", who); return SR3_E_BADARG; }
  if (!hist) return SR3_OK;
  const uintptr_t h0 = (uintptr_t)hist;
  if (align16 && (h0 & 15)) { set_error("misaligned pointer (hist: 16 B)"); return SR3_E_ALIGN; }
  for (const float* p : {x, eps}) {
    const uintptr_t p0 = (uintptr_t)p;
    if (p && p0 < h0 + bytes && h0 < p0 + bytes) { set_error("%s: the history overlaps x or eps", who); return SR3_E_BADARG; }
  }
  return SR3_OK;
}

struct StepFuse {
  float* x;
  const float* z;
  StepTables tb;
  const int* step_cur;
  int* step_next;
  int clip;
  const float* c3;
  float* hist;
};
int conv_out_nchw(const float* x, const float* ss, int B, int H, int W, int C, const float* w,
                  const float* bias, int Cout, float* out_nchw, hipStream_t st, const StepFuse* fuse = nullptr);
struct EmbedParams {
  int variant;
  int B, inner;
  const float* level;
  const int64_t* tstep;
  const float* level_table;
  const int* step_dev;
  const int* t_map;
  int* step_out;
  const float* freq;
  const float* w1; const float* b1;
  const float* w2; const float* b2;
  const float* wf; const float* bf;
  int F;
  float* temb;
  float* film;
};
int embed_forward(const EmbedParams& p, hipStream_t st);
int attention_forward(const float* qkv, int B, int N, int C, float* out, hipStream_t st, int mode = 0);
bool attention_fits(int N, int C);
int attention_long_forward(const float* qkv, int B, int N, int C, float* out, hipStream_t st, bool split);
int p_sample_update(float* x, const float* eps, const float* z, StepTables tb, const int* step_dev,
                    const int64_t* t_per_sample, int step_host, int B, int per_image, hipStream_t st, bool clip = true,
                    const float* c3 = nullptr, float* hist = nullptr);
int step_decrement(int* step_dev, hipStream_t st);
int step_copy(int* step2, hipStream_t st);
int split3_selftest(int* bad_dev, hipStream_t st);
int q_sample(const float* x0, const float* z, const float* ca, const float* cb, int B, int per_image,
             float* out, hipStream_t st);

}
```

image-super-resolution-via-iterative-refinement_amd/sr3_hip/engine.py:

```python
import ctypes as C
import math

import torch

from . import lib as L


def make_desc(variant, in_channel, out_channel, inner_channel, norm_groups, channel_mults, attn_res,
              res_blocks, image_size):
    d = L.UnetDesc()
    d.variant = {'sr3': 0, 'ddpm': 1}[variant]
    d.in_channel = int(in_channel)
    d.out_channel = int(out_channel if out_channel is not None else in_channel)
    d.inner_channel = int(inner_channel)
    d.norm_groups = int(norm_groups)
    mults = list(channel_mults)
    attn = [attn_res] if isinstance(attn_res, int) else list(attn_res)
    if len(mults) > 8 or len(attn) > 8:
        raise L.Sr3Error('at most 8 channel multipliers / attention resolutions')
    d.n_mults = len(mults)
    for i, m in enumerate(mults):
        d.channel_mults[i] = int(m)
    d.n_attn_res = len(attn)
    for i, a in enumerate(attn):
        d.attn_res[i] = int(a)
    d.res_blocks = int(res_blocks)
    d.image_size = int(image_size)
    return d


class Plan(object):

    def __init__(self, variant, in_channel, out_channel, inner_channel, norm_groups, channel_mults, attn_res,
                 res_blocks, image_size):
        self.lib = L.load()
        self.variant = variant
        self.inner = int(inner_channel)
        self.in_channel = int(in_channel)
        self.out_channel = int(out_channel if out_channel is not None else in_channel)
        self.image_size = int(image_size)
        self.desc = make_desc(variant, in_channel, out_channel, inner_channel, norm_groups, channel_mults,
                              attn_res, res_blocks, image_size)
        h = C.c_void_p()
        L.check(self.lib.sr3_plan_create(C.byref(self.desc), C.byref(h)))
        self.handle = h
        self.options = {}
        self.generation = 0
        self.options_epoch = 0
        self.divisor = 1 << (len(list(channel_mults)) - 1)
        self.geometry = (self.image_size, self.image_size)
        self._next_generation = 1
        self._geometry_generation = {self.geometry: 0}
        self.param_floats = int(self.lib.sr3_plan_param_floats(h))
        self.table = []
        pi = L.ParamInfo()
        for i in range(self.lib.sr3_plan_num_params(h)):
            L.check(self.lib.sr3_plan_param_info(h, i, C.byref(pi)))
            self.table.append(dict(name=pi.name.decode(), shape=tuple(pi.shape[:pi.ndim]), pack=int(pi.pack),
                                   offset=int(pi.offset), numel=int(pi.numel)))

    def __del__(self):
        try:
            if getattr(self, 'handle', None):
                self.lib.sr3_plan_destroy(self.handle)
                self.handle = None
        except Exception:
            pass

    def set_option(self, key, value):
        rc = self.lib.sr3_plan_set_option(self.handle, key.encode(), int(value))
        if rc < 0:
            L.check(rc)
        self.options[key] = int(value)
        self.generation = self._next_generation
        self._next_generation += 1
        self._geometry_generation = {self.geometry: self.generation}
        self.options_epoch += 1
        return rc

    def set_geometry(self, height, width):
        height, width = int(height), int(width)
        if (height, width) == (0, 0):
            height = width = self.image_size
        if (height, width) == self.geometry:
            return
        if height <= 0 or width <= 0 or height % self.divisor or width % self.divisor:
            raise L.Sr3Error('image size %d x %d: height and width must be positive multiples of %d (the UNet halves the image %d times)'
                             % (height, width, self.divisor, self.desc.n_mults - 1))
        L.check(self.lib.sr3_plan_set_geometry(self.handle, height, width))
        self.geometry = (height, width)
        gen = self._geometry_generation.get(self.geometry)
        if gen is None:
            gen = self._geometry_generation[self.geometry] = self._next_generation
            self._next_generation += 1
        self.generation = gen

    def workspace_bytes(self, batch):
        n = int(self.lib.sr3_workspace_bytes(self.handle, int(batch)))
        if n == 0:
            raise L.Sr3Error('sr3_workspace_bytes failed: %s' % L.hint((self.lib.sr3_last_error() or b'').decode()))
        return n

    def forward_flops(self, batch):
        return float(self.lib.sr3_plan_forward_flops(self.handle, int(batch)))

    def num_ops(self, batch):
        return int(self.lib.sr3_plan_num_ops(self.handle, int(batch)))

    def op_list(self, batch):
        info = L.OpInfo()
        side, wait = C.c_int(), C.c_int()
        out = []
        for i in range(self.num_ops(batch)):
            L.check(self.lib.sr3_plan_op_info(self.handle, int(batch), i, C.byref(info)))
            o = {k: getattr(info, k) for k, _ in L.OpInfo._fields_}
            L.check(self.lib.sr3_plan_op_side(self.handle, int(batch), i, C.byref(side), C.byref(wait)))
            if side.value >= 0 or wait.value >= 0:
                o['side_id'], o['wait_id'] = side.value, wait.value
            out.append(o)
        return out

    def taps(self):
        out = []
        name = C.create_string_buffer(64)
        off = C.c_size_t()
        c, h, w = C.c_int(), C.c_int(), C.c_int()
        for i in range(self.lib.sr3_plan_num_taps(self.handle)):
            L.check(self.lib.sr3_plan_tap_info(self.handle, i, name, 64, C.byref(off), C.byref(c), C.byref(h), C.byref(w)))
            out.append((name.value.decode(), int(off.value), c.value, h.value, w.value))
        return out

    def view(self, arena, entry):
        flat = arena[entry['offset']:entry['offset'] + entry['numel']]
        shape = entry['shape']
        if entry['pack'] == 1:
            o, i, kh, kw = shape
            return flat.view(o, kh, kw, i).permute(0, 3, 1, 2)
        return flat.view(*shape)

    def default_freq(self):
        dim = self.inner
        if self.variant == 'sr3':
            count = dim // 2
            step = torch.arange(count, dtype=torch.float32) / count
            return torch.exp(-math.log(1e4) * step)
        return torch.exp(torch.arange(0, dim, 2, dtype=torch.float32) * (-math.log(10000) / dim))


class Workspace(object):

    def __init__(self):
        self.buf = None
        self.batch = None

    def get(self, plan, batch, device):
        need = plan.workspace_bytes(batch)
        if self.buf is None or self.buf.numel() < need or self.buf.device != device:
            self.buf = torch.empty(need + 256, dtype=torch.uint8, device=device)
        self.batch = batch
        off = (-self.buf.data_ptr()) % 256
        return self.buf[off:off + need], need


def _check_same_size(x, cond):
    if cond is not None and (cond.dim() != 4 or cond.shape[0] != x.shape[0] or tuple(cond.shape[2:]) != tuple(x.shape[2:])):
        raise L.Sr3Error('conditioning image %s and input %s differ in batch or size' % (tuple(cond.shape), tuple(x.shape)))


def reverse_step(plan, arena, freq, ws, x, z, tables, step2, cond=None, level_table=None, clip_denoised=True, eps_out=None,
                 t_map=None, c3=None, hist=None):
    if not x.is_cuda or not x.is_contiguous() or x.dtype != torch.float32:
        raise L.Sr3Error('reverse_step needs a contiguous fp32 GPU tensor (got %s, %s); there is no CPU fallback' % (x.device, x.dtype))
    B = x.shape[0]
    cc = 0
    if cond is not None:
        cond = cond.contiguous()
        cc = cond.shape[1]
    if x.dim() != 4 or x.shape[1] + cc != plan.in_channel or x.shape[1] != plan.out_channel:
        raise L.Sr3Error('input shape %s (+%d cond channels) does not match the plan (in_channel %d, out_channel %d)'
                         % (tuple(x.shape), cc, plan.in_channel, plan.out_channel))
    _check_same_size(x, cond)
    plan.set_geometry(x.shape[2], x.shape[3])
    if step2.dtype != torch.int32 or step2.numel() != 2 or step2.device != x.device:
        raise L.Sr3Error('step2 must be two int32 on the device of x')
    wsbuf, need = ws.get(plan, B, x.device)
    stream = torch.cuda.current_stream(x.device).cuda_stream
    a, b, c1, c2, sg = tables
    if t_map is not None and (t_map.dtype != torch.int32 or not t_map.is_contiguous() or t_map.device != x.device):
        raise L.Sr3Error('t_map must be a contiguous int32 tensor on the device of x')
    if hist is not None and (hist.dtype != torch.float32 or not hist.is_contiguous() or hist.device != x.device or hist.shape != x.shape):
        raise L.Sr3Error('hist must be a contiguous fp32 tensor of the shape and on the device of x')
    L.check(plan.lib.sr3_reverse_step_hist(plan.handle, L.ptr(x), L.ptr(cond), cc, L.ptr(freq), L.ptr(level_table), L.ptr(step2),
                                           L.ptr(arena), L.ptr(wsbuf), need, L.ptr(z), L.ptr(a), L.ptr(b), L.ptr(c1), L.ptr(c2), L.ptr(sg),
                                           1 if clip_denoised else 0, L.ptr(eps_out), B, C.c_void_p(stream), L.ptr(t_map), L.ptr(c3),
                                           L.ptr(hist)))
    return x


def unet_forward(plan, arena, freq, ws, x, cond=None, noise_level=None, timestep=None, level_table=None,
                 step_dev=None, out=None):
    if not x.is_cuda:
        raise L.Sr3Error('the MI355X engine only runs on a GPU tensor (got %s); there is no CPU fallback' % x.device)
    B = x.shape[0]
    x = x.contiguous()
    cc = 0
    if cond is not None:
        cond = cond.contiguous()
        cc = cond.shape[1]
    if x.dtype != torch.float32 or (cond is not None and cond.dtype != torch.float32):
        raise L.Sr3Error('fp32 tensors expected')
    if x.dim() != 4 or x.shape[1] + cc != plan.in_channel:
        raise L.Sr3Error('input shape %s (+%d cond channels) does not match the plan (in_channel %d)'
                         % (tuple(x.shape), cc, plan.in_channel))
    _check_same_size(x, cond)
    plan.set_geometry(x.shape[2], x.shape[3])
    if noise_level is not None:
        noise_level = noise_level.reshape(-1).contiguous().float()
        if noise_level.numel() != B:
            raise L.Sr3Error('noise_level must have one value per sample')
    if timestep is not None:
        timestep = timestep.reshape(-1).contiguous().long()
        if timestep.numel() != B:
            raise L.Sr3Error('timestep must have one value per sample')
    wsbuf, need = ws.get(plan, B, x.device)
    if out is None:
        out = torch.empty(B, plan.out_channel, x.shape[2], x.shape[3], device=x.device, dtype=torch.float32)
    elif tuple(out.shape) != (B, plan.out_channel, x.shape[2], x.shape[3]) or not out.is_contiguous():
        raise L.Sr3Error('out must be a contiguous %s tensor (got %s)' % ((B, plan.out_channel, x.shape[2], x.shape[3]), tuple(out.shape)))
    stream = torch.cuda.current_stream(x.device).cuda_stream
    L.check(plan.lib.sr3_unet_forward(plan.handle, L.ptr(x), L.ptr(cond), cc, L.ptr(noise_level), L.ptr(timestep),
                                      L.ptr(freq), L.ptr(level_table), L.ptr(step_dev), L.ptr(arena), L.ptr(wsbuf),
                                      need, L.ptr(out), B, C.c_void_p(stream)))
    return out
```

image-super-resolution-via-iterative-refinement_amd/sr3_hip/lib.py:

```python
import ctypes as C
import os

_HERE = os.path.dirname(os.path.abspath(__file__))
LIB_PATH = os.environ.get('SR3_LIBRARY') or os.path.join(_HERE, 'libsr3_mi355x.so')


class Sr3Error(RuntimeError):
    pass


class UnetDesc(C.Structure):
    _fields_ = [('variant', C.c_int), ('in_channel', C.c_int), ('out_channel', C.c_int),
                ('inner_channel', C.c_int), ('norm_groups', C.c_int), ('n_mults', C.c_int),
                ('channel_mults', C.c_int * 8), ('n_attn_res', C.c_int), ('attn_res', C.c_int * 8),
                ('res_blocks', C.c_int), ('image_size', C.c_int)]


class ParamInfo(C.Structure):
    _fields_ = [('name', C.c_char * 128), ('ndim', C.c_int), ('shape', C.c_int * 4), ('pack', C.c_int),
                ('offset', C.c_size_t), ('numel', C.c_size_t)]


class OpInfo(C.Structure):
    _fields_ = [('kind', C.c_int), ('tile_cfg', C.c_int), ('ksplit', C.c_int), ('ksize', C.c_int), ('stride', C.c_int),
                ('upsample', C.c_int), ('cin', C.c_int), ('cout', C.c_int), ('h_out', C.c_int), ('w_out', C.c_int),
                ('fused_res_conv_cin', C.c_int), ('fused_output_stats', C.c_int), ('flops', C.c_double)]


_P = C.c_void_p
_I = C.c_int
_Z = C.c_size_t

_F = C.c_float
_PI = C.POINTER(C.c_int)
SIGNATURES = {
    'sr3_tensor2img': (_I, [_P, _I, _I, _I, _I, _F, _F, _I, _I, _I, _P, _PI, _PI, _PI, _P]),
    'sr3_sse_u8': (_I, [_P, _P, _I, _Z, _P, _P]),
    'sr3_ssim_scratch_bytes': (_Z, [_I, _I, _I, _I]),
    'sr3_ssim_u8': (_I, [_P, _P, _I, _I, _I, _I, _P, _Z, _P, _P]),
    'sr3_eval_scratch_bytes': (_Z, [_I, _I, _I, _I]),
    'sr3_eval_psnr_ssim_f32': (_I, [_P, _P, _I, _I, _I, _I, _F, _F, _P, _Z, _P, _P, _P]),
    'sr3_attention_bwd_f32': (_I, [_P, _P, _P, _I, _I, _I, _P, _P]),
    'sr3_conv_wgrad_scratch_bytes': (_Z, [_I, _I, _I, _I, _I, _I, _I, _I, _I, _I]),
    'sr3_conv_wgrad_f32': (_I, [_P, _I, _P, _I, _I, _I, _I, _I, _I, _I, _I, _P, _I, _P, _P, _I, _P, _Z, _P]),
    'sr3_attention_bwd_scratch_bytes': (_Z, [_I, _I, _I]),
    'sr3_attention_bwd_ex_f32': (_I, [_P, _P, _P, _I, _I, _I, _P, _P, _Z, _P]),
    'sr3_resize_scratch_bytes': (_Z, [_I, _I, _I, _I, _I, _I]),
    'sr3_resize_u8': (_I, [_P, _I, _I, _I, _I, _I, _I, _I, _P, _Z, _P, _P]),
    'sr3_images_u8_to_f32': (_I, [_P, _I, _I, _I, _I, _P, _F, _F, _P, _P]),
    'sr3_blur_u8': (_I, [_P, _I, _I, _I, _I, _P, _I, _P, _P]),
    'sr3_noise_u8': (_I, [_P, _I, _Z, _P, _P, _P, _P]),
    'sr3_version': (_I, []),
    'sr3_selftest_split3': (_I, [_P, C.POINTER(C.c_int), _P]),
    'sr3_last_error': (C.c_char_p, []),
    'sr3_plan_create': (_I, [C.POINTER(UnetDesc), C.POINTER(_P)]),
    'sr3_plan_destroy': (None, [_P]),
    'sr3_plan_num_params': (_I, [_P]),
    'sr3_plan_param_info': (_I, [_P, _I, C.POINTER(ParamInfo)]),
    'sr3_plan_param_floats': (_Z, [_P]),
    'sr3_plan_op_info': (C.c_int, [C.c_void_p, C.c_int, C.c_int, C.POINTER(OpInfo)]),
    'sr3_plan_op_side': (C.c_int, [C.c_void_p, C.c_int, C.c_int, C.POINTER(C.c_int), C.POINTER(C.c_int)]),
    'sr3_plan_num_ops': (_I, [_P, _I]),
    'sr3_plan_forward_flops': (C.c_double, [_P, _I]),
    'sr3_plan_set_option': (_I, [_P, C.c_char_p, _I]),
    'sr3_plan_num_taps': (_I, [_P]),
    'sr3_plan_tap_info': (_I, [_P, _I, C.c_char_p, _I, C.POINTER(_Z), C.POINTER(_I), C.POINTER(_I), C.POINTER(_I)]),
    'sr3_workspace_bytes': (_Z, [_P, _I]),
    'sr3_plan_set_geometry': (_I, [_P, _I, _I]),
    'sr3_plan_get_geometry': (_I, [_P, _PI, _PI]),
    'sr3_plan_derived_bytes': (_Z, [_P]),
    'sr3_plan_bind_derived': (_I, [_P, _P, _Z]),
    'sr3_plan_prepare_derived': (_I, [_P, _P, _P]),
    'sr3_plan_invalidate_derived': (_I, [_P]),
    'sr3_unet_forward': (_I, [_P, _P, _P, _I, _P, _P, _P, _P, _P, _P, _P, _Z, _P, _I, _P]),
    'sr3_unet_forward_profile': (_I, [_P, _P, _P, _I, _P, _P, _P, _P, _P, _Z, _P, _I, _P, _I, _P, _P, _P, _P]),
    'sr3_p_sample_step': (_I, [_P, _P, _P, _P, _P, _P, _P, _P, _P, _P, _I, _I, _I, _P]),
    'sr3_p_sample_step_ex': (_I, [_P, _P, _P, _P, _P, _P, _P, _P, _P, _P, _I, _I, _I, _I, _P]),
    'sr3_p_sample_step_hist': (_I, [_P, _P, _P, _P, _P, _P, _P, _P, _P, _P, _I, _I, _I, _I, _P, _P, _P]),
    'sr3_step_decrement': (_I, [_P, _P]),
    'sr3_reverse_step': (_I, [_P, _P, _P, _I, _P, _P, _P, _P, _P, _Z, _P, _P, _P, _P, _P, _P, _I, _P, _I, _P]),
    'sr3_reverse_step_ex': (_I, [_P, _P, _P, _I, _P, _P, _P, _P, _P, _Z, _P, _P, _P, _P, _P, _P, _I, _P, _I, _P, _P]),
    'sr3_reverse_step_hist': (_I, [_P, _P, _P, _I, _P, _P, _P, _P, _P, _Z, _P, _P, _P, _P, _P, _P, _I, _P, _I, _P, _P, _P, _P]),
    'sr3_tile_gather': (_I, [_P, _I, _I, _I, _I, _P, _I, _P, _I, _I, _I, _I, _I, _P, _P]),
    'sr3_tiled_step': (_I, [_P, _P, _I, _I, _I, _I, _P, _I, _P, _I, _P, _P, _I, _I, _P, _P, _P, _P, _P, _P, _P, _P, _P, _I, _P, _P]),
    'sr3_tiled_step_hist': (_I, [_P, _P, _I, _I, _I, _I, _P, _I, _P, _I, _P, _P, _I, _I, _P, _P, _P, _P, _P, _P, _P, _P, _P, _I, _P, _P, _P, _P]),
    'sr3_block_mean_f32': (_I, [_P, _I, _I, _I, _I, _I, _P, _P]),
    'sr3_consistent_step': (_I, [_P, _P, _P, _P, _I, _I, _I, _I, _I, _F, _P, _P, _P, _P, _P, _P, _I, _P, _P, _P]),
    'sr3_resample_f32': (_I, [_P, _I, _I, _I, _P, _I, _I, _P, _P, _I, _P, _P, _I, _P, _P, _P, _P]),
    'sr3_backproject_scratch_bytes': (_Z, [_I, _I, _I, _I, _I]),
    'sr3_backproject_step': (_I, [_P, _P, _P, _P, _I, _I, _I, _I, _I, _I, _F, _P, _P, _I, _P, _P, _I, _P, _P, _I, _P, _P, _I,
                                  _P, _P, _P, _P, _P, _P, _I, _P, _P, _P, _Z, _P]),
    'sr3_cond_drop_f32': (_I, [_P, _P, _I, _I, _P, _P]),
    'sr3_abs_quantile_scratch_bytes': (_Z, [_I, _I]),
    'sr3_abs_quantile_f32': (_I, [_P, _I, _I, _I, C.c_double, _P, _P, _Z, _P]),
    'sr3_guided_step': (_I, [_P, _P, _P, _F, _P, _I, _I, _I, _I, _P, _P, _P, _P, _P, _P, _P, _P, _I, _I, C.c_double, _P, _P, _Z, _P, _P]),
    'sr3_teacher_step_f32': (_I, [_P, _P, _P, _F, _P, _P, _P, _P, _I, _I, _I, _P, _P, _P]),
    'sr3_distill_target_f32': (_I, [_P, _P, _P, _P, _F, _P, _P, _P, _P, _P, _P, _P, _I, _I, _I, _P, _P, _P]),
    'sr3_q_sample': (_I, [_P, _P, _P, _P, _I, _I, _P, _P]),
    'sr3_train_workspace_bytes': (_Z, [_P, _I, _I]),
    'sr3_train_step': (_I, [_P, _P, _P, _I, _P, _P, _P, _P, _P, _P, _P, _P, _P, _Z, _P, C.c_float, C.c_float, C.c_uint,
                            _I, _P, _P, _I, _P]),
    'sr3_train_step_ex': (_I, [_P, _P, _P, _I, _P, _P, _P, _P, _P, _P, _P, _P, _P, _Z, _P, C.c_float, C.c_float, C.c_uint,
                               _I, _P, _P, _I, _P, _P, _P, _I, C.c_float, _P]),
    'sr3_loss_grad_scratch_bytes': (_Z, []),
    'sr3_loss_grad_f32': (_I, [_P, _P, _P, _P, _P, _P, _I, _I, _I, _I, C.c_float, C.c_float, _P, _P, _P, _P]),
    'sr3_adam_step': (_I, [_P, _P, _P, _P, _Z, C.c_float, C.c_float, C.c_float, C.c_float, _I, _P]),
    'sr3_adam_ema_step': (_I, [_P, _P, _P, _P, _P, _Z, C.c_float, C.c_float, C.c_float, C.c_float, _I, C.c_float, _I, _P]),
    'sr3_adam_ema_step_scaled': (_I, [_P, _P, _P, _P, _P, _Z, C.c_float, C.c_float, C.c_float, C.c_float, _I, C.c_float, _I, _P, _P]),
    'sr3_grad_norm_scratch_bytes': (_Z, [_Z]),
    'sr3_grad_norm': (_I, [_P, _Z, C.c_float, _P, _Z, _P, _P]),
    'sr3_grad_accumulate': (_I, [_P, _P, _Z, _I, C.c_float, _P, _Z, _P, _P]),
    'sr3_conv_f32': (_I, [_P, _I, _P, _I, _I, _I, _I, _I, _I, _I, _I, _P, _P, _P, _I, _P, _I, _P, _I, _P, _I, _P, _P,
                          _I, _I, _P, _Z, _P]),
    'sr3_block_conv_f32': (_I, [_P, _I, _P, _I, _I, _I, _I, _I, _P, _P, _P, _I, _P, _I, _P, _I, _P, _I, _P, _P, _P, _P, _I,
                                _I, _P, _Z, _P]),
    'sr3_conv_dropout_f32': (_I, [_P, _I, _I, _I, _I, _I, _P, _P, _P, _I, _P, _I, _P, _I, _P, _I, _P, _I, _P, _P, _P, _P,
                                  _I, _I, _P, _Z, C.c_uint, C.c_float, _P]),
    'sr3_dropout_threshold': (C.c_uint, [C.c_float, C.POINTER(C.c_float)]),
    'sr3_conv_scratch_bytes': (_Z, [_I, _I, _I, _I, _I, _I, _I, _I]),
    'sr3_groupnorm_stats_f32': (_I, [_P, _I, _I, _I, _P, _P]),
    'sr3_groupnorm_stats_slices': (_I, [_I, _I, _I]),
    'sr3_conv_stats_slices': (_I, [_I, _I, _I, _I, _I, _I, _I, _I]),
    'sr3_groupnorm_fold_f32': (_I, [_P, _I, _I, _P, _I, _I, _I, _I, _I, _P, _P, C.c_float, _P, _P]),
    'sr3_attention_f32': (_I, [_P, _I, _I, _I, _P, _P]),
    'sr3_attention_ex_f32': (_I, [_P, _I, _I, _I, _P, _I, _P]),
    'sr3_film_embed_f32': (_I, [_I, _I, _I, _P, _P, _P, _P, _P, _P, _P, _P, _P, _I, _P, _P, _P]),
    'sr3_conv_in_f32': (_I, [_P, _I, _P, _I, _I, _I, _I, _P, _P, _I, _P, _P]),
    'sr3_conv_out_f32': (_I, [_P, _P, _I, _I, _I, _I, _P, _P, _I, _P, _P]),
}

_lib = None


def load():
    global _lib
    if _lib is not None:
        return _lib
    if not os.path.exists(LIB_PATH):
        raise Sr3Error('libsr3_mi355x.so is not built (%s); run `python __graft_entry__.py build` '
                       'or csrc/build.sh -- there is no CPU / eager fallback' % LIB_PATH)
    lib = C.CDLL(LIB_PATH)
    for name, (res, args) in SIGNATURES.items():
        fn = getattr(lib, name)
        fn.restype = res
        fn.argtypes = args
    if lib.sr3_version() != 1:
        raise Sr3Error('ABI version mismatch: %d' % lib.sr3_version())
    _lib = lib
    return lib


def hint(msg):
    if 'more than the attention kernel holds in LDS' in msg:
        msg += ('; set "long_attention": true in the config\'s model.unet section (EngineUNet(long_attention=True), plan option '
                'attn_long) to run such levels on the key-blocked attention kernel')
    return msg


def check(rc):
    if rc != 0:
        msg = load().sr3_last_error()
        raise Sr3Error('libsr3_mi355x error %d: %s' % (rc, hint((msg or b'').decode())))


def ptr(t):
    return None if t is None else C.c_void_p(t.data_ptr())
```

include/sr3_mi355x.h:

```cpp
#ifndef SR3_MI355X_H
#define SR3_MI355X_H

#include <stddef.h>
#include <stdint.h>

#ifdef __cplusplus
extern "C" {
#endif

#define SR3_ABI_VERSION 1

#define SR3_E_BADARG (-1)
#define SR3_E_UNSUPPORTED (-2)
#define SR3_E_ALIGN (-3)
#define SR3_E_NOMEM (-4)
#define SR3_E_STATE (-5)

#define SR3_VARIANT_SR3 0
#define SR3_VARIANT_DDPM 1

typedef struct sr3_unet_desc {
  int variant;
  int in_channel, out_channel, inner_channel, norm_groups;
  int n_mults;
  int channel_mults[8];
  int n_attn_res;
  int attn_res[8];
  int res_blocks;
  int image_size;
} sr3_unet_desc;

typedef struct sr3_param_info {
  char name[128];
  int ndim;
  int shape[4];
  int pack;
  size_t offset;
  size_t numel;
} sr3_param_info;

typedef struct sr3_plan sr3_plan;

int sr3_version(void);
const char* sr3_last_error(void);
int sr3_selftest_split3(int* scratch_dev, int* mismatches, void* stream);

int sr3_plan_create(const sr3_unet_desc* desc, sr3_plan** out);
void sr3_plan_destroy(sr3_plan* plan);
int sr3_plan_num_params(const sr3_plan* plan);
int sr3_plan_param_info(const sr3_plan* plan, int index, sr3_param_info* out);
size_t sr3_plan_param_floats(const sr3_plan* plan);
int sr3_plan_num_ops(sr3_plan* plan, int batch);
typedef struct sr3_op_info {
  int kind, tile_cfg, ksplit;
  int ksize, stride, upsample;
  int cin, cout, h_out, w_out;
  int fused_res_conv_cin;
  int fused_output_stats;
  double flops;
} sr3_op_info;
int sr3_plan_op_info(sr3_plan* plan, int batch, int index, sr3_op_info* out);
int sr3_plan_op_side(sr3_plan* plan, int batch, int index, int* side_id, int* wait_id);
double sr3_plan_forward_flops(sr3_plan* plan, int batch);
int sr3_plan_set_option(sr3_plan* plan, const char* key, int value);

int sr3_plan_num_taps(sr3_plan* plan);
int sr3_plan_tap_info(sr3_plan* plan, int index, char* name, int name_len, size_t* offset, int* C, int* H, int* W);

int sr3_plan_set_geometry(sr3_plan* plan, int height, int width);
int sr3_plan_get_geometry(const sr3_plan* plan, int* height, int* width);

size_t sr3_plan_derived_bytes(const sr3_plan* plan);
int sr3_plan_bind_derived(sr3_plan* plan, void* buffer, size_t bytes);
int sr3_plan_prepare_derived(sr3_plan* plan, const float* params, void* stream);
int sr3_plan_invalidate_derived(sr3_plan* plan);
size_t sr3_workspace_bytes(sr3_plan* plan, int batch);

int sr3_unet_forward(sr3_plan* plan, const float* x_nchw, const float* cond_nchw, int cond_channels,
                     const float* noise_level, const int64_t* timestep, const float* freq,
                     const float* level_table, const int* step_dev, const float* params,
                     void* workspace, size_t workspace_bytes, float* eps_out_nchw, int batch,
                     void* stream);

int sr3_unet_forward_profile(sr3_plan* plan, const float* x_nchw, const float* cond_nchw, int cond_channels,
                             const float* noise_level, const int64_t* timestep, const float* freq,
                             const float* params, void* workspace, size_t workspace_bytes, float* eps_out_nchw,
                             int batch, void* stream, int max_ops, float* op_ms, int* op_kind, double* op_flops,
                             int* n_ops);

int sr3_p_sample_step(float* x_nchw, const float* eps_nchw, const float* z_nchw, const float* tab_a,
                      const float* tab_b, const float* tab_c1, const float* tab_c2, const float* tab_sigma,
                      const int* step_dev, const int64_t* t_per_sample, int step_host, int batch,
                      int elems_per_image, void* stream);
int sr3_p_sample_step_ex(float* x_nchw, const float* eps_nchw, const float* z_nchw, const float* tab_a,
                         const float* tab_b, const float* tab_c1, const float* tab_c2, const float* tab_sigma,
                         const int* step_dev, const int64_t* t_per_sample, int step_host, int batch,
                         int elems_per_image, int clip_denoised, void* stream);
int sr3_p_sample_step_hist(float* x_nchw, const float* eps_nchw, const float* z_nchw, const float* tab_a,
                           const float* tab_b, const float* tab_c1, const float* tab_c2, const float* tab_sigma,
                           const int* step_dev, const int64_t* t_per_sample, int step_host, int batch,
                           int elems_per_image, int clip_denoised, const float* tab_c3, float* hist_nchw, void* stream);
int sr3_step_decrement(int* step_dev, void* stream);

int sr3_reverse_step(sr3_plan* plan, float* x_nchw, const float* cond_nchw, int cond_channels, const float* freq,
                     const float* level_table, int* step2_dev, const float* params, void* workspace, size_t workspace_bytes,
                     const float* z_nchw, const float* tab_a, const float* tab_b, const float* tab_c1, const float* tab_c2,
                     const float* tab_sigma, int clip_denoised, float* eps_out_nchw, int batch, void* stream);
int sr3_reverse_step_ex(sr3_plan* plan, float* x_nchw, const float* cond_nchw, int cond_channels, const float* freq,
                        const float* level_table, int* step2_dev, const float* params, void* workspace, size_t workspace_bytes,
                        const float* z_nchw, const float* tab_a, const float* tab_b, const float* tab_c1, const float* tab_c2,
                        const float* tab_sigma, int clip_denoised, float* eps_out_nchw, int batch, void* stream, const int* t_map);
int sr3_reverse_step_hist(sr3_plan* plan, float* x_nchw, const float* cond_nchw, int cond_channels, const float* freq,
                          const float* level_table, int* step2_dev, const float* params, void* workspace, size_t workspace_bytes,
                          const float* z_nchw, const float* tab_a, const float* tab_b, const float* tab_c1, const float* tab_c2,
                          const float* tab_sigma, int clip_denoised, float* eps_out_nchw, int batch, void* stream, const int* t_map,
                          const float* tab_c3, float* hist_nchw);


int sr3_tile_gather(const float* src_nchw, int batch, int channels, int height, int width, const int* oy_dev, int ny,
                    const int* ox_dev, int nx, int first_tile, int n_tiles, int th, int tw, float* dst_tiles, void* stream);

int sr3_tiled_step(float* x_nchw, const float* eps_tiles, int batch, int channels, int height, int width, const int* oy_dev, int ny,
                   const int* ox_dev, int nx, const float* wy_dev, const float* wx_dev, int th, int tw, const int* oy_host,
                   const int* ox_host, const float* z_nchw, const float* tab_a, const float* tab_b, const float* tab_c1,
                   const float* tab_c2, const float* tab_sigma, int* step2_dev, int clip_denoised, float* eps_out_nchw, void* stream);
int sr3_tiled_step_hist(float* x_nchw, const float* eps_tiles, int batch, int channels, int height, int width, const int* oy_dev, int ny,
                        const int* ox_dev, int nx, const float* wy_dev, const float* wx_dev, int th, int tw, const int* oy_host,
                        const int* ox_host, const float* z_nchw, const float* tab_a, const float* tab_b, const float* tab_c1,
                        const float* tab_c2, const float* tab_sigma, int* step2_dev, int clip_denoised, float* eps_out_nchw, void* stream,
                        const float* tab_c3, float* hist_nchw);


int sr3_block_mean_f32(const float* src_nchw, int batch, int channels, int height, int width, int block, float* dst_means, void* stream);

int sr3_consistent_step(float* x_nchw, const float* eps_nchw, const float* z_nchw, const float* target_means, int batch, int channels,
                        int height, int width, int block, float strength, const float* tab_a, const float* tab_b, const float* tab_c1,
                        const float* tab_c2, const float* tab_sigma, int* step2_dev, int clip_denoised, const float* tab_c3,
                        float* hist_nchw, void* stream);


int sr3_resample_f32(const float* src, int planes, int height, int width, float* dst, int out_height, int out_width,
                     const int* bounds_h_dev, const float* weights_h_dev, int ksize_h, const int* bounds_v_dev,
                     const float* weights_v_dev, int ksize_v, float* tmp, const int* bounds_h_host, const int* bounds_v_host,
                     void* stream);

size_t sr3_backproject_scratch_bytes(int batch, int channels, int height, int width, int scale);

int sr3_backproject_step(float* x_nchw, const float* eps_nchw, const float* z_nchw, const float* y_lr, int batch, int channels, int height,
                         int width, int scale, int iterations, float strength, const int* down_bounds_h, const float* down_weights_h,
                         int down_ksize_h, const int* down_bounds_v, const float* down_weights_v, int down_ksize_v,
                         const int* up_bounds_h, const float* up_weights_h, int up_ksize_h, const int* up_bounds_v,
                         const float* up_weights_v, int up_ksize_v, const float* tab_a, const float* tab_b, const float* tab_c1,
                         const float* tab_c2, const float* tab_sigma, int* step2_dev, int clip_denoised, const float* tab_c3,
                         float* hist_nchw, void* scratch, size_t scratch_bytes, void* stream);


int sr3_cond_drop_f32(const float* src, const int* keep_dev, int batch, int elems_per_image, float* dst, void* stream);

size_t sr3_abs_quantile_scratch_bytes(int batch, int n);
int sr3_abs_quantile_f32(const float* src, int batch, int n, int rank_lo, double frac, float* out_dev, void* scratch, size_t scratch_bytes,
                         void* stream);

int sr3_guided_step(float* x_nchw, const float* out_c, const float* out_u, float scale, const float* z_nchw, int batch, int channels,
                    int height, int width, const float* tab_a, const float* tab_b, const float* tab_c1, const float* tab_c2,
                    const float* tab_sigma, const float* tab_c3, float* hist_nchw, int* step2_dev, int mode, int rank_lo, double frac,
                    float* x0_scratch, void* q_scratch, size_t q_scratch_bytes, float* thr_out_dev, void* stream);


int sr3_teacher_step_f32(const float* x, const float* out_c, const float* out_u, float scale, const float* a, const float* b,
                         const float* c1, const float* c2, int batch, int elems_per_image, int clip_denoised, float* x_next,
                         float* x0_out, void* stream);

int sr3_distill_target_f32(const float* z_t, const float* x_mid, const float* out_c, const float* out_u, float scale,
                           const float* x0_first, const float* a, const float* b, const float* w1, const float* w2, const float* s1,
                           const float* s2, int batch, int elems_per_image, int clip_denoised, float* x_tgt, float* eps_tgt,
                           void* stream);

int sr3_q_sample(const float* x0, const float* z, const float* ca, const float* cb, int batch,
                 int elems_per_image, float* out, void* stream);


size_t sr3_train_workspace_bytes(sr3_plan* plan, int batch, int cond_channels);

int sr3_train_step(sr3_plan* plan, const float* hr_nchw, const float* cond_nchw, int cond_channels,
                   const float* z_nchw, const float* q_ca, const float* q_cb, const float* noise_level,
                   const int64_t* timestep, const float* freq, const float* params, float* grads,
                   void* workspace, size_t workspace_bytes, float* loss_sum_out, float grad_scale, float dropout_p,
                   unsigned dropout_seed, int n_marks, const size_t* mark_offsets, void* const* mark_events,
                   int batch, void* stream);

int sr3_train_step_ex(sr3_plan* plan, const float* hr_nchw, const float* cond_nchw, int cond_channels,
                      const float* z_nchw, const float* q_ca, const float* q_cb, const float* noise_level,
                      const int64_t* timestep, const float* freq, const float* params, float* grads,
                      void* workspace, size_t workspace_bytes, float* loss_sum_out, float grad_scale, float dropout_p,
                      unsigned dropout_seed, int n_marks, const size_t* mark_offsets, void* const* mark_events,
                      int batch, const float* tgt_z, const float* tgt_x0, const float* weight, int loss_kind,
                      float huber_delta, void* stream);

size_t sr3_loss_grad_scratch_bytes(void);
int sr3_loss_grad_f32(const float* z_nchw, const float* out_nchw, const float* hr_nchw, const float* tgt_z,
                      const float* tgt_x0, const float* weight, int batch, int channels , int pixels,
                      int loss_kind, float huber_delta, float scale, float* g_nhwc4, float* loss_sum_out,
                      void* scratch , void* stream);

int sr3_adam_step(float* params, const float* grads, float* exp_avg, float* exp_avg_sq, size_t n, float lr,
                  float beta1, float beta2, float eps, int step, void* stream);

int sr3_adam_ema_step(float* params, const float* grads, float* exp_avg, float* exp_avg_sq, float* ema, size_t n,
                      float lr, float beta1, float beta2, float eps, int step, float ema_decay, int ema_mode,
                      void* stream);

size_t sr3_grad_norm_scratch_bytes(size_t n);
int sr3_grad_norm(const float* grads, size_t n, float max_norm, void* scratch, size_t scratch_bytes, float* out4_dev,
                  void* stream);

int sr3_grad_accumulate(float* acc, const float* g, size_t n, int first, float max_norm, void* scratch,
                        size_t scratch_bytes, float* out4_dev, void* stream);

int sr3_adam_ema_step_scaled(float* params, const float* grads, float* exp_avg, float* exp_avg_sq, float* ema, size_t n,
                             float lr, float beta1, float beta2, float eps, int step, float ema_decay, int ema_mode,
                             const float* scale4_dev, void* stream);


int sr3_conv_f32(const float* src0, int C0, const float* src1, int C1, int B, int Hs, int Ws, int ups,
                 int stride, int ksize, int Cout, const float* w_ohwi, const float* bias, const float* ss,
                 int act, const float* film, int film_stride, const float* res0, int RC0, const float* res1,
                 int RC1, float* out, double* out_stats, int tile_cfg, int ksplit, void* scratch,
                 size_t scratch_bytes, void* stream);
int sr3_block_conv_f32(const float* src0, int C0, const float* src1, int C1, int B, int H, int W, int Cout,
                       const float* w_ohwi, const float* bias, const float* ss, int act, const float* film,
                       int film_stride, const float* x2_src0, int x2_C0, const float* x2_src1, int x2_C1,
                       const float* x2_w, const float* x2_bias, float* out, double* out_stats, int tile_cfg,
                       int ksplit, void* scratch, size_t scratch_bytes, void* stream);
int sr3_conv_dropout_f32(const float* src0, int C0, int B, int H, int W, int Cout, const float* w_ohwi,
                         const float* bias, const float* ss, int act, const float* film, int film_stride,
                         const float* res0, int RC0, const float* x2_src0, int x2_C0, const float* x2_src1, int x2_C1,
                         const float* x2_w, const float* x2_bias, float* out, double* out_stats, int tile_cfg,
                         int ksplit, void* scratch, size_t scratch_bytes, unsigned drop_seed, float drop_p,
                         void* stream);
unsigned sr3_dropout_threshold(float drop_p, float* scale_out);
size_t sr3_conv_scratch_bytes(int B, int Ho, int Wo, int Cin, int Cout, int ksize, int tile_cfg, int ksplit);
int sr3_groupnorm_stats_slices(int B, int HW, int C);
int sr3_groupnorm_stats_f32(const float* x_nhwc, int B, int HW, int C, double* stat, void* stream);
int sr3_conv_stats_slices(int B, int Hs, int Ws, int ups, int Cin, int Cout, int tile_cfg, int ksplit);
int sr3_groupnorm_fold_f32(const double* stat0, int C0, int T0, const double* stat1, int C1, int T1, int B, int HW,
                           int groups, const float* gamma, const float* beta, float eps, float* ss, void* stream);
int sr3_attention_f32(const float* qkv, int B, int N, int C, float* out, void* stream);
int sr3_attention_ex_f32(const float* qkv, int B, int N, int C, float* out, int split, void* stream);
int sr3_attention_bwd_f32(const float* qkv, const float* dout, const float* out_fwd, int B, int N, int C, float* dqkv,
                          void* stream);
size_t sr3_attention_bwd_scratch_bytes(int B, int N, int C);
int sr3_attention_bwd_ex_f32(const float* qkv, const float* dout, const float* out_fwd, int B, int N, int C, float* dqkv,
                             void* scratch, size_t scratch_bytes, void* stream);
size_t sr3_conv_wgrad_scratch_bytes(int B, int Hs, int Ws, int ups, int stride, int ksize, int C0, int C1, int Cout, int split);
int sr3_conv_wgrad_f32(const float* src0, int C0, const float* src1, int C1, int B, int Hs, int Ws, int ups, int stride, int ksize,
                       int Cout, const float* ss, int act, const float* dy, float* dw_ohwi, int split, void* scratch,
                       size_t scratch_bytes, void* stream);
int sr3_film_embed_f32(int variant, int B, int inner, const float* level, const int64_t* timestep,
                       const float* freq, const float* w1, const float* b1, const float* w2, const float* b2,
                       const float* wf, const float* bf, int F, float* temb_scratch, float* film_out,
                       void* stream);
int sr3_conv_in_f32(const float* a_nchw, int Ca, const float* b_nchw, int Cb, int B, int H, int W,
                    const float* w_ohwi, const float* bias, int Cout, float* out_nhwc, void* stream);
int sr3_conv_out_f32(const float* x_nhwc, const float* ss, int B, int H, int W, int C, const float* w_ohwi,
                     const float* bias, int Cout, float* out_nchw, void* stream);

#ifdef __cplusplus
}
#endif
#endif
```

Measured before the change: 1.190 images/s.

## Pair GroupNorm fold launches with independent following 1x1 GEMM kernels

Adds a paired kernel in which the first workgroups run the GroupNorm finalize (fold) as a rider and the rest run the 1x1 GEMM, so a small fold launch shares a grid with the next independent 1x1 conv. The planner checks memory-span overlap between the fold and the conv to confirm independence. The goal is to remove one small kernel launch and its serialization gap per pairing in the graph. The cost is extra grid blocks on the GEMM and more complex plan logic.

After: 1.191 images/s (median of 2 runs). No clear change (+0.1%).

```diff
diff --git a/image-super-resolution-via-iterative-refinement_amd/csrc/abi_ops.hip b/image-super-resolution-via-iterative-refinement_amd/csrc/abi_ops.hip
--- a/image-super-resolution-via-iterative-refinement_amd/csrc/abi_ops.hip
+++ b/image-super-resolution-via-iterative-refinement_amd/csrc/abi_ops.hip
@@ -1,4 +1,5 @@
 #include "plan_internal.h"
+#include "rider.h"
 #include "tile_code.h"
 
 namespace {
@@ -187,6 +188,29 @@
   return gn_finalize(stat0, C0, T0, stat1, stat1 ? C1 : 0, stat1 ? T1 : 0, B, HW, groups, gamma, beta, eps, ss,
                      static_cast<hipStream_t>(stream));
 }
+int sr3_gemm1x1_rider_f32(const sr3_rider_desc* rd, int paired, const float* src0, int C0, const float* src1, int C1, int B, int H, int W,
+                          int Cout, const float* w, const float* bias, const float* res0, int RC0, float* out, void* scratch,
+                          size_t scratch_bytes, void* stream) {
+  if (!rd || !src0 || !w || !out || !rd->stat0 || !rd->gamma || !rd->beta || !rd->ss) { set_error("null argument"); return SR3_E_BADARG; }
+  if (rd->B <= 0 || rd->HW <= 0 || rd->groups <= 0) { set_error("rider: sizes must be positive"); return SR3_E_BADARG; }
+  hipStream_t st = static_cast<hipStream_t>(stream);
+  RiderArgs r;
+  if (const int rc = gn_fold_rider(rd->stat0, rd->C0, rd->T0, rd->stat1, rd->stat1 ? rd->C1 : 0, rd->stat1 ? rd->T1 : 0, rd->B, rd->HW, rd->groups,
+                                   rd->gamma, rd->beta, rd->eps, rd->ss, nullptr, &r))
+    return rc;
+  ConvParams c = conv_shape(B, H, W, 0, 1, 1, C0, src1 ? C1 : 0, Cout);
+  c.src0 = src0; c.src1 = src1; c.w = w; c.bias = bias; c.res0 = res0; c.RC0 = res0 ? RC0 : 0; c.out = out;
+  c.igemm_split = 1;
+  if (!gemm1x1_fits(c, 2)) { set_error("conv: the 1x1 GEMM kernel (tile 22) does not fit this problem"); return SR3_E_UNSUPPORTED; }
+  float* q = nullptr;
+  if (const int rc = derive_behind_slabs(c, 22, 1, DERIVE_IGEMM_WSPLIT, scratch, &scratch_bytes, st, &q)) return rc;
+  c.w_split = q;
+  if (!paired) {
+    if (const int rc = rider_launch_alone(r, st)) return rc;
+    return conv_forward(c, 22, 1, static_cast<float*>(scratch), scratch_bytes, st);
+  }
+  return conv_forward(c, 22, 1, static_cast<float*>(scratch), scratch_bytes, st, &r);
+}
 int sr3_attention_f32(const float* qkv, int B, int N, int C, float* out, void* stream) {
   if (!qkv || !out) { set_error("null argument"); return SR3_E_BADARG; }
   return attention_forward(qkv, B, N, C, out, static_cast<hipStream_t>(stream));
diff --git a/image-super-resolution-via-iterative-refinement_amd/csrc/conv_igemm.hip b/image-super-resolution-via-iterative-refinement_amd/csrc/conv_igemm.hip
--- a/image-super-resolution-via-iterative-refinement_amd/csrc/conv_igemm.hip
+++ b/image-super-resolution-via-iterative-refinement_amd/csrc/conv_igemm.hip
@@ -545,7 +545,7 @@
 }
 
 int conv_forward(const ConvParams& pin, int tile_cfg, int ksplit, float* scratch, size_t scratch_bytes,
-                 hipStream_t st) {
+                 hipStream_t st, const RiderArgs* rider) {
   ConvParams p = pin;
   const int Cin = p.C0 + p.C1;
   if ((p.C0 & 3) || (p.C1 & 3) || (p.Cout & 3)) { set_error("conv: channel counts must be multiples of 4 (C0=%d C1=%d Cout=%d)", p.C0, p.C1, p.Cout); return SR3_E_UNSUPPORTED; }
@@ -582,8 +582,9 @@
   const bool k3 = p.ksize == 3;
   if (p.x2_w && (tile_cfg < 5 || tile_cfg == 11 || tile_cfg >= 22 || p.ups)) { set_error("conv: the fused 1x1 segment needs the halo kernel without upsampling"); return SR3_E_UNSUPPORTED; }
   if (p.x2_w && ((p.x2_C0 & 3) || (p.x2_C1 & 3) || !p.x2_src0 || (p.x2_C1 > 0 && !p.x2_src1))) { set_error("conv: bad x2 segment"); return SR3_E_BADARG; }
+  if (rider && tile_cfg != 22) { set_error("conv: only the 1x1 GEMM kernel (tile 22) takes a rider"); return SR3_E_UNSUPPORTED; }
   if (tile_cfg == 22) {
-    rc = gemm1x1_forward(p, 2, st);
+    rc = gemm1x1_forward(p, 2, st, rider);
   } else if (tile_cfg == 11) {
     rc = conv3x3_wino_forward(p, p.wino_u, st);
   } else if (tile_cfg >= 5) {
diff --git a/image-super-resolution-via-iterative-refinement_amd/csrc/gemm1x1.hip b/image-super-resolution-via-iterative-refinement_amd/csrc/gemm1x1.hip
--- a/image-super-resolution-via-iterative-refinement_amd/csrc/gemm1x1.hip
+++ b/image-super-resolution-via-iterative-refinement_amd/csrc/gemm1x1.hip
@@ -1,6 +1,7 @@
 #include <stdlib.h>
 
 #include "sr3_common.h"
+#include "rider.h"
 
 #pragma clang diagnostic ignored "-Wpass-failed"
 
@@ -27,8 +28,8 @@
 
 }
 
-template <int MI, bool ACT, bool S2 = false, int WM = 1>
-__global__ __launch_bounds__(256, 2) void k_gemm1x1_split(const ConvParams p) {
+template <int MI, bool ACT, bool S2, int WM>
+__device__ __forceinline__ void gemm1x1_body(const ConvParams p, const int wg_x, const int nwg_x) {
   static_assert(!(ACT && S2), "the stride-2 form has no GroupNorm affine");
   static_assert(WM == 1 || WM == 2, "waves along M");
   constexpr int NWN = 4 / WM;
@@ -52,7 +53,7 @@
   const int tiles_n = p.Cout / (32 * NWN);
   int tile_m, tile_n;
   {
-    const int nwg = gridDim.x, w = blockIdx.x;
+    const int nwg = nwg_x, w = wg_x;
     const int q = nwg >> 3, r = nwg & 7, xcd = w & 7;
     const int lin = (xcd < r ? xcd * (q + 1) : r * (q + 1) + (xcd - r) * q) + (w >> 3);
     tile_m = lin / tiles_n;
@@ -287,6 +288,22 @@
   }
 }
 
+template <int MI, bool ACT, bool S2 = false, int WM = 1>
+__global__ __launch_bounds__(256, 2) void k_gemm1x1_split(const ConvParams p) {
+  gemm1x1_body<MI, ACT, S2, WM>(p, blockIdx.x, gridDim.x);
+}
+
+template <int MI, int WM>
+__global__ __launch_bounds__(256, 2) void k_gemm1x1_paired(const ConvParams p, const RiderArgs r) {
+  const int nr = r.n_wg;
+  if ((int)blockIdx.x < nr) {
+    const int idx = blockIdx.x * 4 + (threadIdx.x >> 6);
+    if (idx < r.g.B * r.g.groups) gn_fold_body(r.g, idx, threadIdx.x & 63);
+    return;
+  }
+  gemm1x1_body<MI, false, false, WM>(p, blockIdx.x - nr, gridDim.x - nr);
+}
+
 bool gemm1x1_s2(const ConvParams& p) {
   return p.ksize == 3 && p.stride == 2 && p.C1 == 0 && p.act == 0 && !(p.Hs & 1) && !(p.Ws & 1) && p.Ho * 2 == p.Hs && p.Wo * 2 == p.Ws;
 }
@@ -311,7 +328,11 @@
 #endif
 }
 
-int gemm1x1_forward(const ConvParams& p, int mi, hipStream_t st) {
+bool gemm1x1_pairable(const ConvParams& p, int ksplit) {
+  return p.ksize == 1 && p.stride == 1 && p.act == 0 && ksplit == 1 && gemm1x1_fits(p, 2) && p.w_split != nullptr;
+}
+
+int gemm1x1_forward(const ConvParams& p, int mi, hipStream_t st, const RiderArgs* rider) {
   if (!gemm1x1_fits(p, mi) || !p.w_split) { set_error("conv: the 1x1 GEMM kernel (tile 22) does not fit this problem"); return SR3_E_UNSUPPORTED; }
   if (p.act == 1 && !p.ss) { set_error("conv: act needs ss"); return SR3_E_BADARG; }
   const int M = p.B * p.Ho * p.Wo;
@@ -319,6 +340,19 @@
   mi = rows / 32;
   dim3 grid((M / rows) * (p.Cout / cols), p.ksplit);
   const int smem = 2 * 2 * mi * 3 * 1024;
+  if (rider) {
+    if (!gemm1x1_pairable(p, p.ksplit) || rider->n_wg <= 0) { set_error("conv: this 1x1 GEMM launch takes no rider"); return SR3_E_UNSUPPORTED; }
+    dim3 pgrid(grid.x + rider->n_wg, 1);
+    static std::atomic<uint64_t> pdone[3];
+    auto pgo = [&](auto kern, std::atomic<uint64_t>& d) -> int {
+      if (int rc = ensure_max_lds(reinterpret_cast<const void*>(kern), smem, d)) return rc;
+      hipLaunchKernelGGL(kern, pgrid, dim3(256), smem, st, p, *rider);
+      SR3_LAUNCH_CHECK("k_gemm1x1_paired");
+      return SR3_OK;
+    };
+    if (cols == 64) return pgo(k_gemm1x1_paired<1, 2>, pdone[0]);
+    return mi == 2 ? pgo(k_gemm1x1_paired<2, 1>, pdone[1]) : pgo(k_gemm1x1_paired<1, 1>, pdone[2]);
+  }
   static std::atomic<uint64_t> done[9];
   auto go = [&](auto kern, std::atomic<uint64_t>& d) -> int {
     if (int rc = ensure_max_lds(reinterpret_cast<const void*>(kern), smem, d)) return rc;
diff --git a/image-super-resolution-via-iterative-refinement_amd/csrc/plan.hip b/image-super-resolution-via-iterative-refinement_amd/csrc/plan.hip
--- a/image-super-resolution-via-iterative-refinement_amd/csrc/plan.hip
+++ b/image-super-resolution-via-iterative-refinement_amd/csrc/plan.hip
@@ -9,6 +9,7 @@
 #include <vector>
 
 #include "plan_internal.h"
+#include "rider.h"
 #include "tile_code.h"
 #include "train.h"
 
@@ -690,6 +691,62 @@
   return f;
 }
 
+struct Span { size_t lo, hi; };
+struct Access { std::vector<Span> rd, wr; };
+static void add_span(std::vector<Span>& v, size_t off, size_t bytes) { if (off != NO_OFF && bytes) v.push_back(Span{off, off + bytes}); }
+static bool spans_meet(const std::vector<Span>& a, const std::vector<Span>& b) {
+  for (const Span& x : a)
+    for (const Span& y : b)
+      if (x.lo < y.hi && y.lo < x.hi) return true;
+  return false;
+}
+static Access conv_access(const sr3_plan* P, const Op& o, const Regions& R, int B) {
+  Access a;
+  const Op::Conv& v = o.conv;
+  const ConvParams& c = v.cp;
+  const size_t Min = (size_t)B * c.Hs * c.Ws, M = (size_t)B * c.Ho * c.Wo;
+  add_span(a.rd, v.src0, Min * c.C0 * sizeof(float));
+  if (c.C1) add_span(a.rd, v.src1, Min * c.C1 * sizeof(float));
+  add_span(a.rd, v.res0, M * c.RC0 * sizeof(float));
+  add_span(a.rd, v.res1, M * c.RC1 * sizeof(float));
+  if (v.x2_src0 != NO_OFF) { add_span(a.rd, v.x2_src0, M * c.x2_C0 * sizeof(float)); add_span(a.rd, v.x2_src1, M * c.x2_C1 * sizeof(float)); }
+  if (v.film_row >= 0) add_span(a.rd, R.film_off + (size_t)v.film_row * sizeof(float), ((size_t)(B - 1) * c.film_stride + c.Cout) * sizeof(float));
+  if (c.act) add_span(a.rd, R.ss_off + o.ss_rel, (size_t)B * (c.C0 + c.C1) * 2 * sizeof(float));
+  add_span(a.wr, v.out, M * c.Cout * sizeof(float));
+  if (v.ostat != NO_OFF) add_span(a.wr, R.stats_off + v.ostat, (size_t)B * (o.fold_fused ? 1 : c.Ho * c.Wo) * c.Cout * 2 * sizeof(double));
+  if (v.ch.ksplit > 1) { add_span(a.rd, R.scratch_off, R.scratch_bytes); add_span(a.wr, R.scratch_off, R.scratch_bytes); }
+  if (o.fold_fused) {
+    const FoldSpec& t = o.tail;
+    if (t.ostat != NO_OFF) add_span(a.rd, R.stats_off + t.ostat, (size_t)B * t.oT * t.oC * 2 * sizeof(double));
+    add_span(a.wr, R.ss_off + t.ss_rel, (size_t)B * t.Ctot * 2 * sizeof(float));
+    if (t.has_mr) add_span(a.wr, R.mr_off + t.mr_rel, (size_t)B * P->d.norm_groups * 2 * sizeof(float));
+  }
+  return a;
+}
+static Access fold_access(const sr3_plan* P, const Op& o, const Regions& R, int B) {
+  Access a;
+  const Op::Fold& v = o.fold;
+  add_span(a.rd, R.stats_off + v.stat0, (size_t)B * v.T0 * v.C0 * 2 * sizeof(double));
+  if (v.stat1 != NO_OFF) add_span(a.rd, R.stats_off + v.stat1, (size_t)B * v.T1 * v.C1 * 2 * sizeof(double));
+  add_span(a.wr, R.ss_off + o.ss_rel, (size_t)B * (v.C0 + v.C1) * 2 * sizeof(float));
+  if (v.has_mr) add_span(a.wr, R.mr_off + o.mr_rel, (size_t)B * P->d.norm_groups * 2 * sizeof(float));
+  return a;
+}
+static bool pair_fold(const sr3_plan* P, const Op& o, const Op& g, const Regions& R, int B) {
+  if (!P->pair_launch) return false;
+  if (o.kind != OP_FOLD || o.fold.has_mr) return false;
+  if (o.side_id >= 0 || o.wait_id >= 0 || g.side_id >= 0 || g.wait_id >= 0) return false;
+  if (g.kind != OP_CONV || g.fold_fused) return false;
+  const Op::Conv& v = g.conv;
+  const ConvParams& c = v.cp;
+  if (v.ch.tile_cfg != 22 || v.ch.ksplit != 1 || !v.ch.has_wsplit || !c.igemm_split || c.ksize != 1 || c.stride != 1 || c.act != 0 ||
+      v.ostat != NO_OFF || v.x2_src0 != NO_OFF || v.has_drop || !gemm1x1_fits(c, 2))
+    return false;
+  const Access a = fold_access(P, o, R, B);
+  const Access b = conv_access(P, g, R, B);
+  return !(spans_meet(b.wr, a.rd) || spans_meet(b.wr, a.wr) || spans_meet(a.wr, b.rd));
+}
+
 int run_forward(sr3_plan* P, bool train, const float* x, const float* cond, int cond_channels, const float* level,
                 const int64_t* tstep, const float* freq, const float* level_table, const int* step_dev,
                 const float* params, char* ws, float* eps_out, int B, hipStream_t st,
@@ -701,9 +758,19 @@
   char* const stats = ws + R.stats_off;
   const bool forking = !ev && !train;
   hipStream_t const main_st = st;
-  for (const Op& o : train ? P->tops : P->ops) {
+  const std::vector<Op>& list = train ? P->tops : P->ops;
+  const bool pairing = !train && !ev && P->pair_launch != 0;
+  RiderArgs pending;
+  bool have_pending = false;
+  for (size_t oi = 0; oi < list.size(); ++oi) {
+    const Op& o = list[oi];
+    const bool pair = pairing && oi + 1 < list.size() && pair_fold(P, o, list[oi + 1], R, B);
     int rc = SR3_OK;
     st = main_st;
+    if (have_pending && o.kind != OP_CONV) {
+      if (int prc = rider_launch_alone(pending, main_st)) return prc;
+      have_pending = false;
+    }
     if (ev) SR3_HIP(hipEventRecord(ev[op_index], st));
     ++op_index;
     if (forking && o.wait_id >= 0 && o.wait_id < (int)P->join_ev.size())
@@ -757,6 +824,12 @@
       }
       case OP_FOLD: {
         const Op::Fold& v = o.fold;
+        if (pair) {
+          rc = gn_fold_rider(bind<const double>(stats, v.stat0), v.C0, v.T0, bind<const double>(stats, v.stat1), v.C1, v.T1, B, v.pixels,
+                             d.norm_groups, params + v.gamma, params + v.beta, 1e-5f, bind<float>(ws, R.ss_off + o.ss_rel), nullptr, &pending);
+          have_pending = rc == SR3_OK;
+          break;
+        }
         rc = gn_finalize(bind<const double>(stats, v.stat0), v.C0, v.T0, bind<const double>(stats, v.stat1), v.C1, v.T1, B, v.pixels,
                          d.norm_groups, params + v.gamma, params + v.beta, 1e-5f, bind<float>(ws, R.ss_off + o.ss_rel), st,
                          v.has_mr ? bind<float>(ws, R.mr_off + o.mr_rel) : nullptr);
@@ -803,6 +876,15 @@
         if (mid && ch.ksplit > 1) conv_set_mid_event(mid[op_index - 1]);
         FoldTail ft;
         if (o.fold_fused) { ft = make_fold_tail(o.tail, d.norm_groups, params, ws, R); c.fold = &ft; }
+        if (have_pending) {
+          have_pending = false;
+          const RiderArgs rider = pending;
+          if (ch.tile_cfg == 22 && gemm1x1_pairable(c, ch.ksplit)) {
+            rc = conv_forward(c, ch.tile_cfg, ch.ksplit, bind<float>(ws, R.scratch_off), R.scratch_bytes, st, &rider);
+            break;
+          }
+          if ((rc = rider_launch_alone(rider, st))) break;
+        }
         rc = conv_forward(c, ch.tile_cfg, ch.ksplit, bind<float>(ws, R.scratch_off), R.scratch_bytes, st);
         break;
       }
@@ -823,6 +905,7 @@
     if (forking && o.side_id >= 0) SR3_HIP(hipEventRecord(P->join_ev[o.side_id], st));
   }
   st = main_st;
+  if (have_pending) { if (int prc = rider_launch_alone(pending, st)) return prc; }
   if (ev) SR3_HIP(hipEventRecord(ev[op_index], st));
   return SR3_OK;
 }
@@ -924,6 +1007,15 @@
   if (wait_id) *wait_id = plan->ops[index].wait_id;
   return SR3_OK;
 }
+int sr3_plan_op_pair(sr3_plan* plan, int batch, int index, int* rider_kind) {
+  if (!plan || !rider_kind) { set_error("null argument"); return SR3_E_BADARG; }
+  const int cond = plan->built_cond >= 0 ? plan->built_cond : 0;
+  const int rc = build_forward(plan, batch, cond);
+  if (rc) return rc;
+  if (index < 0 || index >= (int)plan->ops.size()) { set_error("op index out of range"); return SR3_E_BADARG; }
+  *rider_kind = index + 1 < (int)plan->ops.size() && pair_fold(plan, plan->ops[index], plan->ops[index + 1], plan->regions, batch) ? 1 : 0;
+  return SR3_OK;
+}
 double sr3_plan_forward_flops(sr3_plan* plan, int batch) {
   if (!plan) return 0;
   const int cond = plan->built_cond >= 0 ? plan->built_cond : 0;
@@ -956,6 +1048,7 @@
   else if (!strcmp(key, "wino2")) slot = &plan->wino2;
   else if (!strcmp(key, "wino_ragged")) slot = &plan->wino_ragged;
   else if (!strcmp(key, "wino_up")) slot = &plan->wino_up;
+  else if (!strcmp(key, "pair_launch")) { const int prev = plan->pair_launch; plan->pair_launch = value; return prev; }
   else if (!strcmp(key, "train_geom")) slot = &plan->train_geom;
   else if (!strcmp(key, "loss_l2")) { const int prev = plan->loss_l2; plan->loss_l2 = value; return prev; }
   if (!slot) { set_error("unknown option %s", key); return SR3_E_BADARG; }
diff --git a/image-super-resolution-via-iterative-refinement_amd/csrc/plan_internal.h b/image-super-resolution-via-iterative-refinement_amd/csrc/plan_internal.h
--- a/image-super-resolution-via-iterative-refinement_amd/csrc/plan_internal.h
+++ b/image-super-resolution-via-iterative-refinement_amd/csrc/plan_internal.h
@@ -170,6 +170,7 @@
   int gemm_n64 = 1;
   int wino_ragged = 1;
   int wino_up = 1;
+  int pair_launch = 1;
   int train_geom = 0;
   int geo_h = 0, geo_w = 0;
   int fork_side = 0;
diff --git a/image-super-resolution-via-iterative-refinement_amd/csrc/rider.h b/image-super-resolution-via-iterative-refinement_amd/csrc/rider.h
--- /dev/null
+++ b/image-super-resolution-via-iterative-refinement_amd/csrc/rider.h
@@ -0,0 +1,66 @@
+#pragma once
+#include "sr3_common.h"
+
+namespace sr3 {
+
+struct GnFoldArgs {
+  const double* st0; int C0, T0;
+  const double* st1; int C1, T1;
+  int B, HW, groups;
+  const float* gamma; const float* beta; float eps;
+  float* ss; float* mr;
+};
+__device__ __forceinline__ void gn_fold_body(const GnFoldArgs& a, int idx, int lane) {
+  const double* __restrict__ st0 = a.st0;
+  const double* __restrict__ st1 = a.st1;
+  const int C0 = a.C0, C1 = a.C1, groups = a.groups;
+  const int C = C0 + C1;
+  const int b = idx / groups, g = idx - b * groups;
+  const int cpg = C / groups;
+  double s = 0.0, s2 = 0.0;
+  const int c_lo = g * cpg, c_hi = c_lo + cpg;
+  const int n0 = max(0, min(c_hi, C0) - c_lo);
+  typedef double d2 __attribute__((ext_vector_type(2)));
+  auto walk = [&](const double* st, int Cs, int T, int c_first, int n) {
+    const int total = n * T;
+    auto at = [&](int i) {
+      const int k = i / T, t = i - k * T;
+      return *reinterpret_cast<const d2*>(st + (((size_t)b * T + t) * Cs + (c_first + k)) * 2);
+    };
+    int i = lane;
+    for (; i + 192 < total; i += 256) {
+      const d2 q0 = at(i), q1 = at(i + 64), q2 = at(i + 128), q3 = at(i + 192);
+      s += q0[0]; s2 += q0[1]; s += q1[0]; s2 += q1[1]; s += q2[0]; s2 += q2[1]; s += q3[0]; s2 += q3[1];
+    }
+    for (; i < total; i += 64) { const d2 q = at(i); s += q[0]; s2 += q[1]; }
+  };
+  walk(st0, C0, a.T0, c_lo, n0);
+  const int n1 = cpg - n0;
+  const int c1_lo = max(c_lo, C0) - C0;
+  if (n1 > 0) walk(st1, C1, a.T1, c1_lo, n1);
+#pragma unroll
+  for (int m = 32; m >= 1; m >>= 1) { s += __shfl_xor(s, m); s2 += __shfl_xor(s2, m); }
+  const double cnt = (double)a.HW * cpg;
+  const double mean = s / cnt;
+  double var = s2 / cnt - mean * mean;
+  if (var < 0.0) var = 0.0;
+  const float rstd = (float)(1.0 / sqrt(var + (double)a.eps));
+  if (a.mr && lane == 0) { a.mr[((size_t)b * groups + g) * 2] = (float)mean; a.mr[((size_t)b * groups + g) * 2 + 1] = rstd; }
+  for (int k = lane; k < cpg; k += 64) {
+    const int c = g * cpg + k;
+    const float sc = rstd * a.gamma[c];
+    float* o = a.ss + ((size_t)b * C + c) * 2;
+    o[0] = sc;
+    o[1] = a.beta[c] - (float)mean * sc;
+  }
+}
+
+struct RiderArgs {
+  int n_wg = 0;
+  GnFoldArgs g = {};
+};
+int rider_launch_alone(const RiderArgs& r, hipStream_t st);
+int gn_fold_rider(const double* stat0, int C0, int T0, const double* stat1, int C1, int T1, int B, int HW, int groups, const float* gamma,
+                  const float* beta, float eps, float* ss, float* mr, RiderArgs* out);
+
+}
diff --git a/image-super-resolution-via-iterative-refinement_amd/csrc/small_kernels.hip b/image-super-resolution-via-iterative-refinement_amd/csrc/small_kernels.hip
--- a/image-super-resolution-via-iterative-refinement_amd/csrc/small_kernels.hip
+++ b/image-super-resolution-via-iterative-refinement_amd/csrc/small_kernels.hip
@@ -1,6 +1,7 @@
 #include <string.h>
 
 #include "sr3_common.h"
+#include "rider.h"
 
 namespace sr3 {
 
@@ -72,59 +73,24 @@
   return SR3_OK;
 }
 
-__global__ __launch_bounds__(64) void k_gn_finalize(const double* __restrict__ st0, int C0, int T0,
-                                                     const double* __restrict__ st1, int C1, int T1, int HW,
-                                                     int groups, const float* __restrict__ gamma,
-                                                     const float* __restrict__ beta, float eps,
-                                                     float* __restrict__ ss, float* __restrict__ mr) {
+__global__ __launch_bounds__(64) void k_gn_finalize(const GnFoldArgs a) { gn_fold_body(a, blockIdx.x, threadIdx.x); }
+
+int gn_fold_rider(const double* stat0, int C0, int T0, const double* stat1, int C1, int T1, int B, int HW, int groups, const float* gamma,
+                  const float* beta, float eps, float* ss, float* mr, RiderArgs* out) {
   const int C = C0 + C1;
-  const int b = blockIdx.x / groups, g = blockIdx.x - b * groups;
-  const int cpg = C / groups;
-  const int lane = threadIdx.x;
-  double s = 0.0, s2 = 0.0;
-  const int c_lo = g * cpg, c_hi = c_lo + cpg;
-  const int n0 = max(0, min(c_hi, C0) - c_lo);
-  typedef double d2 __attribute__((ext_vector_type(2)));
-  auto walk = [&](const double* st, int Cs, int T, int c_first, int n) {
-    const int total = n * T;
-    auto at = [&](int idx) {
-      const int k = idx / T, t = idx - k * T;
-      return *reinterpret_cast<const d2*>(st + (((size_t)b * T + t) * Cs + (c_first + k)) * 2);
-    };
-    int idx = lane;
-    for (; idx + 192 < total; idx += 256) {
-      const d2 q0 = at(idx), q1 = at(idx + 64), q2 = at(idx + 128), q3 = at(idx + 192);
-      s += q0[0]; s2 += q0[1]; s += q1[0]; s2 += q1[1]; s += q2[0]; s2 += q2[1]; s += q3[0]; s2 += q3[1];
-    }
-    for (; idx < total; idx += 64) { const d2 q = at(idx); s += q[0]; s2 += q[1]; }
-  };
-  walk(st0, C0, T0, c_lo, n0);
-  const int n1 = cpg - n0;
-  const int c1_lo = max(c_lo, C0) - C0;
-  if (n1 > 0) walk(st1, C1, T1, c1_lo, n1);
-#pragma unroll
-  for (int m = 32; m >= 1; m >>= 1) { s += __shfl_xor(s, m); s2 += __shfl_xor(s2, m); }
-  const double cnt = (double)HW * cpg;
-  const double mean = s / cnt;
-  double var = s2 / cnt - mean * mean;
-  if (var < 0.0) var = 0.0;
-  const float rstd = (float)(1.0 / sqrt(var + (double)eps));
-  if (mr && lane == 0) { mr[((size_t)b * groups + g) * 2] = (float)mean; mr[((size_t)b * groups + g) * 2 + 1] = rstd; }
-  for (int k = lane; k < cpg; k += 64) {
-    const int c = g * cpg + k;
-    const float sc = rstd * gamma[c];
-    float* o = ss + ((size_t)b * C + c) * 2;
-    o[0] = sc;
-    o[1] = beta[c] - (float)mean * sc;
-  }
+  if (groups <= 0 || C % groups) { set_error("gn_finalize: C=%d not divisible by groups=%d", C, groups); return SR3_E_BADARG; }
+  RiderArgs r;
+  r.n_wg = (B * groups + 3) / 4;
+  r.g = GnFoldArgs{stat0, C0, T0, stat1, C1, T1, B, HW, groups, gamma, beta, eps, ss, mr};
+  *out = r;
+  return SR3_OK;
 }
 
 int gn_finalize(const double* stat0, int C0, int T0, const double* stat1, int C1, int T1, int B, int HW, int groups,
                 const float* gamma, const float* beta, float eps, float* ss, hipStream_t st, float* mr) {
-  const int C = C0 + C1;
-  if (groups <= 0 || C % groups) { set_error("gn_finalize: C=%d not divisible by groups=%d", C, groups); return SR3_E_BADARG; }
-  hipLaunchKernelGGL(k_gn_finalize, dim3(B * groups), dim3(64), 0, st, stat0, C0, T0, stat1, C1, T1, HW, groups,
-                     gamma, beta, eps, ss, mr);
+  RiderArgs r;
+  if (int rc = gn_fold_rider(stat0, C0, T0, stat1, C1, T1, B, HW, groups, gamma, beta, eps, ss, mr, &r)) return rc;
+  hipLaunchKernelGGL(k_gn_finalize, dim3(B * groups), dim3(64), 0, st, r.g);
   SR3_LAUNCH_CHECK("k_gn_finalize");
   return SR3_OK;
 }
@@ -264,6 +230,11 @@
                      p.Ho * p.Wo, p.ostat);
   SR3_LAUNCH_CHECK("k_rows_fold");
   return SR3_OK;
+}
+
+int rider_launch_alone(const RiderArgs& r, hipStream_t st) {
+  const GnFoldArgs& g = r.g;
+  return gn_finalize(g.st0, g.C0, g.T0, g.st1, g.C1, g.T1, g.B, g.HW, g.groups, g.gamma, g.beta, g.eps, g.ss, st, g.mr);
 }
 
 __global__ __launch_bounds__(256) void k_split3_selftest(int n, unsigned seed, int* __restrict__ bad) {
diff --git a/image-super-resolution-via-iterative-refinement_amd/csrc/sr3_common.h b/image-super-resolution-via-iterative-refinement_amd/csrc/sr3_common.h
--- a/image-super-resolution-via-iterative-refinement_amd/csrc/sr3_common.h
+++ b/image-super-resolution-via-iterative-refinement_amd/csrc/sr3_common.h
@@ -162,8 +162,9 @@
   return hash32(idx * 0x9E3779B9U + seed) >= thresh ? scale : 0.f;
 }
 
+struct RiderArgs;
 int conv_forward(const ConvParams& p, int tile_cfg, int ksplit, float* splitk_scratch,
-                 size_t splitk_scratch_bytes, hipStream_t st);
+                 size_t splitk_scratch_bytes, hipStream_t st, const RiderArgs* rider = nullptr);
 size_t conv_splitk_bytes(const ConvParams& p, int tile_cfg, int ksplit);
 void conv_pick(const ConvParams& p, int& tile_cfg, int& ksplit);
 int splitk_rows_per_block(const ConvParams& p, bool stats);
@@ -171,7 +172,8 @@
 int igemm_split_weights(const float* w, int Cout, int taps, int Cin, float* out, hipStream_t st);
 bool gemm1x1_fits(const ConvParams& p, int mi);
 int gemm1x1_cols(const ConvParams& p);
-int gemm1x1_forward(const ConvParams& p, int mi, hipStream_t st);
+int gemm1x1_forward(const ConvParams& p, int mi, hipStream_t st, const RiderArgs* rider = nullptr);
+bool gemm1x1_pairable(const ConvParams& p, int ksplit);
 int gemm1x1_rows(const ConvParams& p);
 void conv_set_mid_event(hipEvent_t ev);
 struct HaloGeom {
diff --git a/image-super-resolution-via-iterative-refinement_amd/sr3_hip/engine.py b/image-super-resolution-via-iterative-refinement_amd/sr3_hip/engine.py
--- a/image-super-resolution-via-iterative-refinement_amd/sr3_hip/engine.py
+++ b/image-super-resolution-via-iterative-refinement_amd/sr3_hip/engine.py
@@ -118,6 +118,15 @@
             if side.value >= 0 or wait.value >= 0:
                 o['side_id'], o['wait_id'] = side.value, wait.value
             out.append(o)
+        return out
+
+    def pair_list(self, batch):
+        kind = C.c_int()
+        out = []
+        for i in range(self.num_ops(batch)):
+            L.check(self.lib.sr3_plan_op_pair(self.handle, int(batch), i, C.byref(kind)))
+            if kind.value:
+                out.append(i)
         return out
 
     def taps(self):
diff --git a/image-super-resolution-via-iterative-refinement_amd/sr3_hip/lib.py b/image-super-resolution-via-iterative-refinement_amd/sr3_hip/lib.py
--- a/image-super-resolution-via-iterative-refinement_amd/sr3_hip/lib.py
+++ b/image-super-resolution-via-iterative-refinement_amd/sr3_hip/lib.py
@@ -25,6 +25,13 @@
     _fields_ = [('kind', C.c_int), ('tile_cfg', C.c_int), ('ksplit', C.c_int), ('ksize', C.c_int), ('stride', C.c_int),
                 ('upsample', C.c_int), ('cin', C.c_int), ('cout', C.c_int), ('h_out', C.c_int), ('w_out', C.c_int),
                 ('fused_res_conv_cin', C.c_int), ('fused_output_stats', C.c_int), ('flops', C.c_double)]
+
+
+class RiderDesc(C.Structure):
+    _fields_ = [('B', C.c_int), ('HW', C.c_int), ('groups', C.c_int),
+                ('stat0', C.c_void_p), ('C0', C.c_int), ('T0', C.c_int),
+                ('stat1', C.c_void_p), ('C1', C.c_int), ('T1', C.c_int),
+                ('gamma', C.c_void_p), ('beta', C.c_void_p), ('eps', C.c_float), ('ss', C.c_void_p)]
 
 
 _P = C.c_void_p
@@ -60,6 +67,7 @@
     'sr3_plan_param_floats': (_Z, [_P]),
     'sr3_plan_op_info': (C.c_int, [C.c_void_p, C.c_int, C.c_int, C.POINTER(OpInfo)]),
     'sr3_plan_op_side': (C.c_int, [C.c_void_p, C.c_int, C.c_int, C.POINTER(C.c_int), C.POINTER(C.c_int)]),
+    'sr3_plan_op_pair': (_I, [_P, _I, _I, _PI]),
     'sr3_plan_num_ops': (_I, [_P, _I]),
     'sr3_plan_forward_flops': (C.c_double, [_P, _I]),
     'sr3_plan_set_option': (_I, [_P, C.c_char_p, _I]),
@@ -122,6 +130,7 @@
     'sr3_groupnorm_stats_slices': (_I, [_I, _I, _I]),
     'sr3_conv_stats_slices': (_I, [_I, _I, _I, _I, _I, _I, _I, _I]),
     'sr3_groupnorm_fold_f32': (_I, [_P, _I, _I, _P, _I, _I, _I, _I, _I, _P, _P, C.c_float, _P, _P]),
+    'sr3_gemm1x1_rider_f32': (_I, [C.POINTER(RiderDesc), _I, _P, _I, _P, _I, _I, _I, _I, _I, _P, _P, _P, _I, _P, _P, _Z, _P]),
     'sr3_attention_f32': (_I, [_P, _I, _I, _I, _P, _P]),
     'sr3_attention_ex_f32': (_I, [_P, _I, _I, _I, _P, _I, _P]),
     'sr3_film_embed_f32': (_I, [_I, _I, _I, _P, _P, _P, _P, _P, _P, _P, _P, _P, _I, _P, _P, _P]),
diff --git a/include/sr3_mi355x.h b/include/sr3_mi355x.h
--- a/include/sr3_mi355x.h
+++ b/include/sr3_mi355x.h
@@ -61,6 +61,7 @@
 } sr3_op_info;
 int sr3_plan_op_info(sr3_plan* plan, int batch, int index, sr3_op_info* out);
 int sr3_plan_op_side(sr3_plan* plan, int batch, int index, int* side_id, int* wait_id);
+int sr3_plan_op_pair(sr3_plan* plan, int batch, int index, int* rider_kind);
 double sr3_plan_forward_flops(sr3_plan* plan, int batch);
 int sr3_plan_set_option(sr3_plan* plan, const char* key, int value);
 
@@ -245,6 +246,16 @@
 int sr3_conv_stats_slices(int B, int Hs, int Ws, int ups, int Cin, int Cout, int tile_cfg, int ksplit);
 int sr3_groupnorm_fold_f32(const double* stat0, int C0, int T0, const double* stat1, int C1, int T1, int B, int HW,
                            int groups, const float* gamma, const float* beta, float eps, float* ss, void* stream);
+typedef struct sr3_rider_desc {
+  int B, HW, groups;
+  const double* stat0; int C0, T0;
+  const double* stat1; int C1, T1;
+  const float* gamma; const float* beta; float eps;
+  float* ss;
+} sr3_rider_desc;
+int sr3_gemm1x1_rider_f32(const sr3_rider_desc* rider, int paired, const float* src0, int C0, const float* src1, int C1, int B, int H, int W,
+                          int Cout, const float* w, const float* bias, const float* res0, int RC0, float* out, void* scratch,
+                          size_t scratch_bytes, void* stream);
 int sr3_attention_f32(const float* qkv, int B, int N, int C, float* out, void* stream);
 int sr3_attention_ex_f32(const float* qkv, int B, int N, int C, float* out, int split, void* stream);
 int sr3_attention_bwd_f32(const float* qkv, const float* dout, const float* out_fwd, int B, int N, int C, float* dqkv,
```
